# deadskull7/One-Stop-for-COVID-19-Infection-and-Lung-Segmentation-plus-Classification

Measured on AMD Instinct MI355X. Metric: CT images/sec (fwd+bwd) U-Net 512x512x1 bs16, higher is better.
Workload: dtype f32 storage / accumulate / parameters; conv products as a two-term fp16 split (3 fp16 MFMAs per multiply, ~2^-22 per product; --algo 2 = strict fp32); 1 GPU; U-Net infection seg (task1 graph T1:853-916), 512x512x1, batch 16/GPU, fp32, fwd+loss+bwd+Keras-Adam; BASELINE.json configs[1]; storage=fp32, global_batch=16, parallelism=dp1, deterministic=False, bn_fold=2

## Files before the change

include/unet_hip.h:

```cpp
#ifndef UNET_HIP_H
#define UNET_HIP_H
#include <stddef.h>
#include <stdint.h>

#ifdef __cplusplus
extern "C" {
#endif

#define UNET_ABI_VERSION 16

typedef struct unet_ctx unet_ctx;
typedef struct unet_model unet_model;
typedef uint16_t unet_bf16;
enum { UNET_DTYPE_F32 = 0, UNET_DTYPE_BF16 = 1 };

enum { UNET_OK = 0, UNET_E_ARG = -1, UNET_E_HIP = -2, UNET_E_SHAPE = -3, UNET_E_STATE = -4, UNET_E_NODEV = -5 };

enum { UNET_ALGO_AUTO = 0, UNET_ALGO_NAIVE = 1, UNET_ALGO_MFMA = 2 };

int32_t unet_abi_version(void);
int32_t unet_ctx_create(int32_t device_id, unet_ctx** out);
void unet_ctx_destroy(unet_ctx* ctx);
const char* unet_last_error(const unet_ctx* ctx);
int32_t unet_ctx_set_profiling(unet_ctx* ctx, int32_t on);
enum { UNET_OPT_RELU_BITS = 1, UNET_OPT_BN_FOLD = 2, UNET_OPT_ENC_BN_FUSED = 3, UNET_OPT_BN_CONCAT_ANALYTIC = 4, UNET_OPT_BN_FUSE_STATS = 5, UNET_OPT_DETERMINISTIC = 6,
       UNET_OPT_HEAD_FUSED = 7, UNET_OPT_SKIP_RAW = 8, UNET_OPT_POOL_SUMS_FUSED = 9, UNET_OPT_HEAD_BWD_FUSED = 10, UNET_OPT_CONV_PP = 13, UNET_OPT_ENC_TAIL_DGRAD = 14,
       UNET_OPT_WGRAD_EARLY_SPLIT = 15 };
int32_t unet_ctx_set_option(unet_ctx* ctx, int32_t option, int32_t value);
int32_t unet_ctx_get_option(unet_ctx* ctx, int32_t option);

enum { UNET_ACT_NONE = 0, UNET_ACT_RELU = 1, UNET_ACT_ELU = 2 };
enum { UNET_MASK_NONE = 0, UNET_MASK_RELU = 1, UNET_MASK_ELU = 2, UNET_MASK_ELU_DROP = 3, UNET_MASK_RELU_BITS = 9  };

size_t unet_conv3x3_w_ws_floats(int32_t cin, int32_t cout);
int32_t unet_conv3x3_pick_algo(int32_t algo, int32_t wd, int32_t cin, int32_t cout);
double unet_conv3x3_exec_ratio(int32_t algo, int32_t h, int32_t wd, int32_t cin, int32_t cout);
double unet_conv3x3_wgrad_exec_ratio(int32_t algo, int32_t h, int32_t wd, int32_t cin, int32_t cout);
int32_t unet_request_bn_stats(unet_ctx*, int32_t c);
int32_t unet_relu_bits_supported(int32_t algo, int32_t h, int32_t wd, int32_t cin, int32_t cout);
size_t unet_relu_bits_bytes(int32_t n, int32_t h, int32_t wd, int32_t c);
int32_t unet_request_relu_bits(unet_ctx*, void* bits);
int32_t unet_allow_k_slices(unet_ctx*);
int32_t unet_ctx_max_kernel_scratch_bytes(unet_ctx*);
int32_t unet_conv3x3_fwd(unet_ctx*, const float* x, const float* w, const float* bias, float* y,
                         int32_t n, int32_t h, int32_t wd, int32_t cin, int32_t cout,
                         int32_t act, float drop_rate, uint64_t drop_seed, int32_t algo, float* w_ws, void* stream);
int32_t unet_conv3x3_fwd_ld(unet_ctx*, const float* x, const float* w, const float* bias, float* y, int32_t ldy,
                            int32_t n, int32_t h, int32_t wd, int32_t cin, int32_t cout, int32_t act, int32_t algo, float* w_ws, void* stream);
int32_t unet_conv3x3_bwd_data(unet_ctx*, const float* dy, const float* w, const float* mask_src,
                              int32_t mask_mode, float mask_rate, uint64_t mask_seed,
                              float* dx, float* wt_ws, int32_t n, int32_t h, int32_t wd,
                              int32_t cin, int32_t cout, int32_t algo, void* stream);
int32_t unet_conv3x3_bnfold_supported(int32_t algo, int32_t h, int32_t wd, int32_t cin, int32_t cout);
size_t unet_conv3x3_bnfold_ws_floats(int32_t n, int32_t cin, int32_t cout);
int32_t unet_conv3x3_bnfold_fwd(unet_ctx*, const float* x, const float* bnp, const float* w, const float* bias, float* y, int32_t n, int32_t h,
                                int32_t wd, int32_t cin, int32_t cout, int32_t act, int32_t algo, float* ws, void* stream);
int32_t unet_conv3x3_bnfold_bwd_weights(unet_ctx*, const float* x, const float* bnp, const float* dy, const float* w, float* dw, float* db,
                                        double* bn_bwd_sums, void* gws, size_t gws_bytes, float* ws, int32_t n, int32_t h, int32_t wd,
                                        int32_t cin, int32_t cout, int32_t algo, void* stream);
int32_t unet_conv3x3_bnfold_bwd_data(unet_ctx*, const float* dy, const float* w, const float* bnp, const double* bn_bwd_sums, double count, const float* x,
                                     int32_t x_channels, int32_t mask_mode, float mask_rate, uint64_t mask_seed, float* dx, float* wt_ws, float* coef,
                                     int32_t n, int32_t h, int32_t wd, int32_t cin, int32_t cout, int32_t algo, void* stream);
int32_t unet_conv3x3_bnfold_bwd_data_enc_tail(unet_ctx*, const float* dy, const float* w, const float* bnp, const double* bn_bwd_sums, double count, const float* x, int32_t ldx,
                                              const float* enc_bnp, const double* enc_sums, double enc_count, const float* skip_k1, const float* dy_pooled, float rate,
                                              uint64_t seed, float* dx, float* wt_ws, float* coef, int32_t n, int32_t h, int32_t wd, int32_t c, int32_t algo, void* stream);
size_t unet_conv3x3_bwd_weights_ws_bytes(int32_t n, int32_t h, int32_t wd, int32_t cin, int32_t cout);
int32_t unet_conv3x3_bwd_weights(unet_ctx*, const float* x, const float* dy, float* dw, float* db,
                                 void* ws, size_t ws_bytes, int32_t n, int32_t h, int32_t wd,
                                 int32_t cin, int32_t cout, int32_t algo, void* stream);

int32_t unet_convT2x2_fwd(unet_ctx*, const float* x, const float* w, const float* bias, float* y,
                          int32_t ldy, int32_t n, int32_t h, int32_t wd, int32_t cin, int32_t cout,
                          int32_t algo, void* stream);
int32_t unet_convT2x2_bwd_data(unet_ctx*, const float* dy, int32_t lddy, const float* w,
                               const float* relu_src, float* dx, int32_t n, int32_t h, int32_t wd,
                               int32_t cin, int32_t cout, int32_t algo, void* stream);
size_t unet_convT2x2_bwd_weights_ws_bytes(int32_t n, int32_t h, int32_t wd, int32_t cin, int32_t cout);
int32_t unet_convT2x2_bwd_weights(unet_ctx*, const float* x, const float* dy, int32_t lddy,
                                  float* dw, float* db, void* ws, size_t ws_bytes, int32_t n,
                                  int32_t h, int32_t wd, int32_t cin, int32_t cout, int32_t algo,
                                  void* stream);

int32_t unet_bn_stats(unet_ctx*, const float* x, int32_t ldx, double* sums, int64_t pixels,
                      int32_t c, void* stream);
int32_t unet_bn_stats_concat(unet_ctx*, const float* x_up, int32_t ldx, const double* src_sums, double src_count, const float* src_gamma,
                             const float* src_beta, double* sums, int64_t pixels, int32_t c_up, int32_t c_skip, void* stream);
int32_t unet_bn_finalize_train(unet_ctx*, const double* sums, double count, const float* gamma,
                               const float* beta, float* moving_mean, float* moving_var,
                               float* bnp, int32_t c, void* stream);
int32_t unet_bn_finalize_infer(unet_ctx*, const float* gamma, const float* beta,
                               const float* moving_mean, const float* moving_var, float* bnp,
                               int32_t c, void* stream);
int32_t unet_bn_apply(unet_ctx*, const float* x, int32_t ldx, const float* bnp, float* y,
                      int32_t ldy, int64_t pixels, int32_t c, void* stream);
int32_t unet_bn_bwd_stats(unet_ctx*, const float* dy, int32_t lddy, const float* x, int32_t ldx,
                          const float* bnp, double* sums, int64_t pixels, int32_t c, void* stream);
int32_t unet_bn_bwd_param_grads(unet_ctx*, const double* sums, float* dgamma, float* dbeta,
                                int32_t c, void* stream);
int32_t unet_bn_bwd_apply(unet_ctx*, const float* dy, int32_t lddy, const float* x, int32_t ldx,
                          const float* bnp, const double* sums, double count, int32_t mask_mode,
                          float mask_rate, uint64_t mask_seed, float* dx, int32_t lddx, int64_t pixels,
                          int32_t c, void* stream);

int32_t unet_maxpool2x2_dropout_fwd(unet_ctx*, const float* x, int32_t ldx, float* y, int32_t n,
                                    int32_t h, int32_t wd, int32_t c, float rate, uint64_t seed,
                                    void* stream);
int32_t unet_maxpool2x2_dropout_bwd(unet_ctx*, const float* x, int32_t ldx, const float* dy,
                                    float* dx, int32_t lddx, int32_t n, int32_t h, int32_t wd,
                                    int32_t c, float rate, uint64_t seed, int32_t accumulate,
                                    void* stream);

int32_t unet_bn_apply_maxpool_dropout_fwd(unet_ctx*, const float* x, int32_t ldx, const float* bnp, float* y,
                                          int32_t ldy, float* pooled, int32_t n, int32_t h, int32_t wd,
                                          int32_t c, float rate, uint64_t seed, void* stream);
int32_t unet_maxpool2x2_dropout_bwd_bnstats(unet_ctx*, const float* y, int32_t ldy, const float* dy, float* dx,
                                            int32_t lddx, const float* gamma, const float* beta, double* sums,
                                            int32_t n, int32_t h, int32_t wd, int32_t c, float rate,
                                            uint64_t seed, void* stream);
int32_t unet_maxpool2x2_dropout_bwd_sums(unet_ctx*, const float* pooled, const float* dy_pooled, const float* gamma, const float* beta, double* sums,
                                         int32_t n, int32_t h, int32_t wd, int32_t c, float rate, uint64_t seed, void* stream);
int32_t unet_bn_bwd_skip_term(unet_ctx*, double* sums, const double* dec_sum_dyxhat, const float* dec_invstd, const float* dec_gamma,
                              const float* gamma, int32_t c, double frac, void* stream);
int32_t unet_bn_maxpool_bwd_apply(unet_ctx*, const float* x, int32_t ldx, const float* bnp, const double* sums, double count, const float* g_skip,
                                  int32_t ldg, const float* dy_pooled, float* dx, int32_t lddx, int32_t n, int32_t h, int32_t wd, int32_t c,
                                  float rate, uint64_t seed, void* stream);

enum { UNET_LOSS_BCE_DICE = 0, UNET_LOSS_BCE = 1, UNET_LOSS_DICE = 2, UNET_LOSS_TVERSKY = 3, UNET_LOSS_WEIGHTED_BCE_DICE = 4 };
int32_t unet_loss_weight_map(unet_ctx*, const float* y_true, float* weight, int32_t n, int32_t h, int32_t wd, void* stream);
int32_t unet_head_fwd_ex(unet_ctx*, const float* x, const float* w, const float* bias, float* p, const float* y_true, const float* weight_map, double* loss_sums,
                         int64_t pixels, int32_t cin, void* stream);
int32_t unet_head_fwd_bf16_ex(unet_ctx*, const unet_bf16* x, const float* w, const float* bias, float* p, const float* y_true, const float* weight_map,
                              double* loss_sums, int64_t pixels, int32_t cin, void* stream);

int32_t unet_head_fwd(unet_ctx*, const float* x, const float* w, const float* bias, float* p,
                      const float* y_true, double* loss_sums, int64_t pixels, int32_t cin,
                      void* stream);
int32_t unet_loss_finalize(unet_ctx*, const double* loss_sums, double count, float* loss_out,
                           void* stream);
int32_t unet_head_bwd(unet_ctx*, const float* x, const float* w, const float* p, const float* y_true,
                      const double* loss_sums, double count, float* dx, float* dw, float* db,
                      int64_t pixels, int32_t cin, int32_t relu_mask, void* stream);
int32_t unet_loss_finalize_ex(unet_ctx*, const double* loss_sums, double count, int32_t loss, float alpha, float beta, float* loss_out, void* stream);
int32_t unet_head_bwd_ex(unet_ctx*, const float* x, const float* w, const float* p, const float* y_true, const double* loss_sums, double count,
                         int32_t loss, float alpha, float beta, const float* weight_map, float* dx, float* dw, float* db, int64_t pixels, int32_t cin, int32_t relu_mask,
                         void* stream);

int32_t unet_conv3x3_bwd_data_pool_sums_supported(unet_ctx*, int32_t algo, int32_t wd, int32_t cin, int32_t cout);
int32_t unet_conv3x3_bwd_data_pool_sums(unet_ctx*, const float* dy, const float* w, const float* pooled, const float* gamma, const float* beta, float rate,
// ... 355 lines not shown
```

one-stop-for-covid-19-infection-and-lung-segmentation-plus-classification_amd/_lib.py:

```python
from __future__ import annotations

import ctypes as C
import os

_HERE = os.path.dirname(os.path.abspath(__file__))
LIB_PATH = os.environ.get("COVIDSEG_AMD_LIB") or os.path.join(_HERE, "libunet_hip.so")
ABI_VERSION = 16
COMM_HANDLE_BYTES, COMM_MAX_WORLD, COMM_MAX_DOUBLES = 64, 8, 2048

ALGO_AUTO, ALGO_NAIVE, ALGO_MFMA = 0, 1, 2
OPTIONS = {"relu_bits": 1, "bn_fold": 2, "enc_bn_fused": 3, "bn_concat_analytic": 4, "bn_fuse_stats": 5, "deterministic": 6, "head_fused": 7, "skip_raw": 8, "pool_sums_fused": 9, "head_bwd_fused": 10, "conv_pp": 13, "enc_tail_dgrad": 14, "wgrad_early_split": 15}
ARCH_UNET, ARCH_UNETPP, ARCH_CLASSIFIER = 0, 1, 2
LOSSES = {"bce_dice_loss": 0, "binary_crossentropy": 1, "dice_loss": 2, "tversky_loss": 3, "weighted_bce_dice_loss": 4}
DTYPE_F32, DTYPE_BF16 = 0, 1
ACT_NONE, ACT_RELU, ACT_ELU = 0, 1, 2
MORPH_OPS = {"dilate": 0, "erode": 1, "open": 2, "close": 3}
MORPH_MAX_ITERATIONS = 64
INTENSITY_MAX_EDGES = 63
JOINT_HIST_MAX_K, JOINT_HIST_MAX_BINS = 16, 64
SMOOTH_MAX_RADIUS = 32
PAIRS_CHUNK, PAIRS_LDS_SLOTS = 4096, 1024
PAIRS_MIN_CAPACITY, PAIRS_MAX_CAPACITY = 16, 2 ** 30
TRACK_CLS_NONE, TRACK_CLS_RESOLVED, TRACK_CLS_SHRINKAGE, TRACK_CLS_BOTH, TRACK_CLS_GROWTH, TRACK_CLS_NEW = 0, 1, 2, 3, 4, 5
TEXTURE_MAX_LEVELS, TEXTURE_MAX_DISTANCE, TEXTURE_LDS_COUNTERS = 64, 4, 8192
TEXTURE_MAX_RUN = 2 ** 15
ZONE_MAX_PARTS, ZONE_MAX_SHELLS, ZONE_MAX_BINS = 8, 4, 1024
RANK_MAX_RADIUS = 2
FILTER_MODES = {"nearest": 0, "constant": 1, "reflect": 2}
GEODESIC_MAX_STEP = 65534
MASK_NONE, MASK_RELU, MASK_ELU, MASK_ELU_DROP = 0, 1, 2, 3
PROG_FWD_TRAIN, PROG_BWD, PROG_FWD_INFER = 0, 1, 2
SYNC_BN_FWD, SYNC_LOSS, SYNC_BN_BWD, SYNC_GRAD_BUCKET = 0, 1, 2, 3

f32p = C.POINTER(C.c_float)
f64p = C.POINTER(C.c_double)
vp = C.c_void_p
i32, i64, u64, f32, f64, sz = C.c_int32, C.c_int64, C.c_uint64, C.c_float, C.c_double, C.c_size_t


class SyncPoint(C.Structure):
    _fields_ = [("after_op", i32), ("kind", i32), ("ptr", vp), ("count", i64), ("use_op", i32), ("reserved", i32)]


RENDER_MAX_TILES, RENDER_MAX_LAYERS = 64, 4


class RenderTile(C.Structure):
    _fields_ = [("axis", i32), ("index", i32), ("x0", i32), ("y0", i32), ("w", i32), ("h", i32)]


class RenderLayer(C.Structure):
    _fields_ = [("labels", vp), ("palette", vp), ("dtype", i32), ("palette_size", i32), ("fill_alpha", i32), ("outline_alpha", i32)]


class ZoneSpec(C.Structure):
    _fields_ = [("parts", i32 * 3), ("flip", i32 * 3), ("lo", (i32 * 3) * 2), ("extent", (i32 * 3) * 2), ("shells", i32), ("reserved", i32), ("r2", (f64 * 3) * 2)]


_PROTOS = {
    "unet_abi_version": (i32, []),
    "unet_ctx_create": (i32, [i32, C.POINTER(vp)]),
    "unet_ctx_destroy": (None, [vp]),
    "unet_last_error": (C.c_char_p, [vp]),
    "unet_ctx_set_profiling": (i32, [vp, i32]),
    "unet_ctx_set_option": (i32, [vp, i32, i32]),
    "unet_ctx_get_option": (i32, [vp, i32]),
    "unet_conv3x3_w_ws_floats": (sz, [i32, i32]),
    "unet_conv3x3_pick_algo": (i32, [i32, i32, i32, i32]),
    "unet_conv3x3_exec_ratio": (f64, [i32, i32, i32, i32, i32]),
    "unet_conv3x3_wgrad_exec_ratio": (f64, [i32, i32, i32, i32, i32]),
    "unet_request_bn_stats": (i32, [vp, i32]),
    "unet_relu_bits_supported": (i32, [i32, i32, i32, i32, i32]),
    "unet_relu_bits_bytes": (sz, [i32, i32, i32, i32]),
    "unet_request_relu_bits": (i32, [vp, vp]),
    "unet_allow_k_slices": (i32, [vp]),
    "unet_ctx_max_kernel_scratch_bytes": (i32, [vp]),
    "unet_conv3x3_fwd": (i32, [vp, vp, vp, vp, vp, i32, i32, i32, i32, i32, i32, f32, u64, i32, vp, vp]),
    "unet_conv3x3_fwd_ld": (i32, [vp, vp, vp, vp, vp, i32, i32, i32, i32, i32, i32, i32, i32, vp, vp]),
    "unet_conv3x3_bwd_data": (i32, [vp, vp, vp, vp, i32, f32, u64, vp, vp, i32, i32, i32, i32, i32, i32, vp]),
    "unet_conv3x3_bwd_weights_ws_bytes": (sz, [i32, i32, i32, i32, i32]),
    "unet_conv3x3_bwd_weights": (i32, [vp, vp, vp, vp, vp, vp, sz, i32, i32, i32, i32, i32, i32, vp]),
    "unet_convT2x2_fwd": (i32, [vp, vp, vp, vp, vp, i32, i32, i32, i32, i32, i32, i32, vp]),
    "unet_convT2x2_bwd_data": (i32, [vp, vp, i32, vp, vp, vp, i32, i32, i32, i32, i32, i32, vp]),
    "unet_convT2x2_bwd_weights_ws_bytes": (sz, [i32, i32, i32, i32, i32]),
    "unet_convT2x2_bwd_weights": (i32, [vp, vp, vp, i32, vp, vp, vp, sz, i32, i32, i32, i32, i32, i32, vp]),
    "unet_cast_f32_to_bf16": (i32, [vp, vp, vp, i64, vp]),
    "unet_cast_bf16_to_f32": (i32, [vp, vp, vp, i64, vp]),
    "unet_conv3x3_fwd_bf16": (i32, [vp, vp, vp, vp, vp, i32, i32, i32, i32, i32, i32, f32, u64, vp, vp]),
    "unet_conv3x3_first_fwd_bf16": (i32, [vp, vp, vp, vp, vp, i32, i32, i32, i32, i32, f32, u64, vp]),
    "unet_conv3x3_bwd_data_bf16": (i32, [vp, vp, vp, vp, i32, f32, u64, vp, vp, i32, i32, i32, i32, i32, vp]),
    "unet_conv3x3_bwd_weights_ws_bytes_bf16": (sz, [i32, i32, i32, i32, i32]),
    "unet_conv3x3_bwd_weights_bf16": (i32, [vp, vp, vp, vp, vp, vp, sz, i32, i32, i32, i32, i32, vp]),
    "unet_conv3x3_first_bwd_weights_bf16": (i32, [vp, vp, vp, vp, vp, vp, sz, i32, i32, i32, i32, vp]),
    "unet_convT2x2_fwd_bf16": (i32, [vp, vp, vp, vp, vp, i32, i32, i32, i32, i32, i32, vp, vp]),
    "unet_convT2x2_bwd_data_bf16": (i32, [vp, vp, i32, vp, vp, vp, i32, i32, i32, i32, i32, vp, vp]),
    "unet_convT2x2_bwd_weights_ws_bytes_bf16": (sz, [i32, i32, i32, i32, i32]),
    "unet_convT2x2_bwd_weights_bf16": (i32, [vp, vp, vp, i32, vp, vp, vp, sz, i32, i32, i32, i32, i32, vp]),
    "unet_bn_stats": (i32, [vp, vp, i32, vp, i64, i32, vp]),
    "unet_bn_stats_bf16": (i32, [vp, vp, i32, vp, i64, i32, vp]),
    "unet_conv3x3_bnfold_supported": (i32, [i32, i32, i32, i32, i32]),
    "unet_conv3x3_bnfold_ws_floats": (sz, [i32, i32, i32]),
    "unet_conv3x3_bnfold_fwd": (i32, [vp, vp, vp, vp, vp, vp, i32, i32, i32, i32, i32, i32, i32, vp, vp]),
    "unet_conv3x3_bnfold_bwd_weights": (i32, [vp, vp, vp, vp, vp, vp, vp, vp, vp, sz, vp, i32, i32, i32, i32, i32, i32, vp]),
    "unet_conv3x3_bnfold_bwd_data": (i32, [vp, vp, vp, vp, vp, f64, vp, i32, i32, f32, u64, vp, vp, vp, i32, i32, i32, i32, i32, i32, vp]),
    "unet_conv3x3_bnfold_bwd_data_enc_tail": (i32, [vp, vp, vp, vp, vp, f64, vp, i32, vp, vp, f64, vp, vp, f32, u64, vp, vp, vp, i32, i32, i32, i32, i32, vp]),
    "unet_bn_stats_concat": (i32, [vp, vp, i32, vp, f64, vp, vp, vp, i64, i32, i32, vp]),
    "unet_bn_stats_concat_bf16": (i32, [vp, vp, i32, vp, f64, vp, vp, vp, i64, i32, i32, vp]),
    "unet_bn_finalize_train": (i32, [vp, vp, f64, vp, vp, vp, vp, vp, i32, vp]),
    "unet_bn_finalize_infer": (i32, [vp, vp, vp, vp, vp, vp, i32, vp]),
    "unet_bn_apply": (i32, [vp, vp, i32, vp, vp, i32, i64, i32, vp]),
    "unet_bn_apply_bf16": (i32, [vp, vp, i32, vp, vp, i32, i64, i32, vp]),
    "unet_bn_bwd_stats": (i32, [vp, vp, i32, vp, i32, vp, vp, i64, i32, vp]),
    "unet_bn_bwd_stats_bf16": (i32, [vp, vp, i32, vp, i32, vp, vp, i64, i32, vp]),
    "unet_bn_bwd_param_grads": (i32, [vp, vp, vp, vp, i32, vp]),
    "unet_bn_bwd_apply": (i32, [vp, vp, i32, vp, i32, vp, vp, f64, i32, f32, u64, vp, i32, i64, i32, vp]),
    "unet_bn_bwd_apply_bf16": (i32, [vp, vp, i32, vp, i32, vp, vp, f64, i32, f32, u64, vp, i32, i64, i32, vp]),
    "unet_maxpool2x2_dropout_fwd": (i32, [vp, vp, i32, vp, i32, i32, i32, i32, f32, u64, vp]),
    "unet_maxpool2x2_dropout_fwd_bf16": (i32, [vp, vp, i32, vp, i32, i32, i32, i32, f32, u64, vp]),
    "unet_maxpool2x2_dropout_bwd": (i32, [vp, vp, i32, vp, vp, i32, i32, i32, i32, i32, f32, u64, i32, vp]),
    "unet_maxpool2x2_dropout_bwd_bf16": (i32, [vp, vp, i32, vp, vp, i32, i32, i32, i32, i32, f32, u64, i32, vp]),
    "unet_bn_apply_maxpool_dropout_fwd": (i32, [vp, vp, i32, vp, vp, i32, vp, i32, i32, i32, i32, f32, u64, vp]),
    "unet_bn_apply_maxpool_dropout_fwd_bf16": (i32, [vp, vp, i32, vp, vp, i32, vp, i32, i32, i32, i32, f32, u64, vp]),
    "unet_maxpool2x2_dropout_bwd_bnstats": (i32, [vp, vp, i32, vp, vp, i32, vp, vp, vp, i32, i32, i32, i32, f32, u64, vp]),
    "unet_maxpool2x2_dropout_bwd_sums": (i32, [vp, vp, vp, vp, vp, vp, i32, i32, i32, i32, f32, u64, vp]),
    "unet_maxpool2x2_dropout_bwd_sums_bf16": (i32, [vp, vp, vp, vp, vp, vp, i32, i32, i32, i32, f32, u64, vp]),
    "unet_bn_maxpool_bwd_apply_bf16": (i32, [vp, vp, i32, vp, vp, f64, vp, i32, vp, vp, i32, i32, i32, i32, i32, f32, u64, vp]),
    "unet_bn_bwd_skip_term": (i32, [vp, vp, vp, vp, vp, vp, i32, f64, vp]),
    "unet_bn_maxpool_bwd_apply": (i32, [vp, vp, i32, vp, vp, f64, vp, i32, vp, vp, i32, i32, i32, i32, i32, f32, u64, vp]),
    "unet_maxpool2x2_dropout_bwd_bnstats_bf16": (i32, [vp, vp, i32, vp, vp, i32, vp, vp, vp, i32, i32, i32, i32, f32, u64, vp]),
    "unet_head_fwd": (i32, [vp, vp, vp, vp, vp, vp, vp, i64, i32, vp]),
    "unet_head_fwd_bf16": (i32, [vp, vp, vp, vp, vp, vp, vp, i64, i32, vp]),
    "unet_loss_finalize": (i32, [vp, vp, f64, vp, vp]),
    "unet_head_bwd": (i32, [vp, vp, vp, vp, vp, vp, f64, vp, vp, vp, i64, i32, i32, vp]),
    "unet_head_bwd_bf16": (i32, [vp, vp, vp, vp, vp, vp, f64, vp, vp, vp, i64, i32, i32, vp]),
    "unet_loss_finalize_ex": (i32, [vp, vp, f64, i32, f32, f32, vp, vp]),
    "unet_head_bwd_ex": (i32, [vp, vp, vp, vp, vp, vp, f64, i32, f32, f32, vp, vp, vp, vp, i64, i32, i32, vp]),
    "unet_head_bwd_bf16_ex": (i32, [vp, vp, vp, vp, vp, vp, f64, i32, f32, f32, vp, vp, vp, vp, i64, i32, i32, vp]),
    "unet_head_fwd_ex": (i32, [vp, vp, vp, vp, vp, vp, vp, vp, i64, i32, vp]),
    "unet_head_fwd_bf16_ex": (i32, [vp, vp, vp, vp, vp, vp, vp, vp, i64, i32, vp]),
    "unet_loss_weight_map": (i32, [vp, vp, vp, i32, i32, i32, vp]),
    "unet_conv3x3_head_fwd_ex": (i32, [vp, vp, vp, vp, vp, vp, vp, vp, vp, vp, vp, vp, i32, i32, i32, i32, vp, vp]),
    "unet_adam_keras": (i32, [vp, vp, vp, vp, vp, i64, f32, f32, f32, f32, f32, vp]),
    "unet_seg_metrics_sweep": (i32, [vp, vp, vp, vp, i32, vp, i64, vp]),
    "unet_gather_samples": (i32, [vp, vp, vp, vp, i64, i64, vp]),
    "unet_augment_samples": (i32, [vp, vp, vp, vp, vp, vp, vp, i64, i32, i32, i32, vp]),
    "unet_feat_col_mean": (i32, [vp, vp, i64, i64, i64, vp, vp]),
    "unet_feat_gemm_nt_workspace": (sz, [i64, i64, i64, i32]),
    "unet_feat_gemm_nt": (i32, [vp, vp, i64, vp, vp, i64, vp, i64, i64, i64, i32, vp, i64, i32, vp, sz, vp]),
    "unet_feat_gemm_tn_workspace": (sz, [i64, i64, i64]),
    "unet_feat_gemm_tn": (i32, [vp, vp, i64, vp, i64, vp, i64, i64, i64, vp, i64, i32, vp, sz, vp]),
    "unet_kmeans_step": (i32, [vp, vp, i64, i64, i64, vp, i32, vp, vp, vp, vp, vp, vp]),
    "unet_cluster_route_workspace": (sz, [i64, i64, i32]),
    "unet_cluster_route": (i32, [vp, vp, i32, i64, i32, i32, i32, i64, vp, vp, i32, vp, i32, vp, vp, vp, vp, sz, vp]),
    "unet_conv3x3_head_supported": (i32, [vp, i32, i32, i32, i32]),
    "unet_conv3x3_head_fwd": (i32, [vp, vp, vp, vp, vp, vp, vp, vp, vp, vp, vp, i32, i32, i32, i32, vp, vp]),
    "unet_conv3x3_bwd_data_pool_sums_supported": (i32, [vp, i32, i32, i32, i32]),
    "unet_conv3x3_bwd_data_pool_sums": (i32, [vp, vp, vp, vp, vp, vp, f32, vp, vp, vp, i32, i32, i32, i32, i32, vp]),
    "unet_head_dy": (i32, [vp, vp, vp, vp, f64, vp, vp, vp, vp, vp, vp, vp, i32, i32, i32, vp]),
    "unet_head_bwd_stream_supported": (i32, [vp, i32, i32, i32]),
    "unet_head_dzm": (i32, [vp, vp, vp, vp, f64, vp, vp, vp, vp, vp, i32, i32, i32, vp]),
    "unet_head_dy_ex": (i32, [vp, vp, vp, vp, f64, vp, i32, f32, f32, vp, vp, vp, vp, vp, vp, vp, i32, i32, i32, vp]),
    "unet_head_dzm_ex": (i32, [vp, vp, vp, vp, f64, vp, i32, f32, f32, vp, vp, vp, vp, vp, i32, i32, i32, vp]),
    "unet_conv3x3_bwd_data_dzm": (i32, [vp, vp, vp, vp, vp, vp, vp, i32, i32, i32, i32, vp]),
    "unet_conv3x3_bwd_weights_dzm": (i32, [vp, vp, vp, vp, vp, vp, vp, sz, i32, i32, i32, i32, vp]),
    "unet_zero": (i32, [vp, vp, sz, vp]),
    "unet_comm_create": (i32, [vp, i32, i32, vp, vp]),
    "unet_comm_connect": (i32, [vp, vp]),
    "unet_comm_set_timeout_ms": (i32, [vp, i32]),
    "unet_comm_allreduce_f64": (i32, [vp, vp, i32, vp]),
    "unet_comm_status": (i32, [vp, vp, vp]),
    "unet_comm_destroy": (None, [vp]),
    "unet_copy_slice": (i32, [vp, vp, i32, vp, i32, i64, i32, vp]),
    "unet_copy_slice_bf16": (i32, [vp, vp, i32, vp, i32, i64, i32, vp]),
    "unet_accum_slices": (i32, [vp, C.POINTER(vp), C.POINTER(i32), i32, vp, i32, i64, i32, i32, vp]),
    "unet_accum_slices_bf16": (i32, [vp, C.POINTER(vp), C.POINTER(i32), i32, vp, i32, i64, i32, i32, vp]),
    "unet_dense_ws_bytes": (sz, [i32, i32, i32]),
    "unet_dense_fwd": (i32, [vp, vp, vp, vp, vp, i32, i32, i32, i32, f32, u64, vp, sz, vp]),
    "unet_dense_fwd_bf16": (i32, [vp, vp, vp, vp, vp, i32, i32, i32, i32, f32, u64, vp, sz, vp]),
    "unet_dense_bwd": (i32, [vp, vp, vp, vp, vp, vp, i32, i32, i32, vp]),
    "unet_dense_bwd_bf16": (i32, [vp, vp, vp, vp, vp, vp, i32, i32, i32, vp]),
    "unet_cls_head_fwd": (i32, [vp, vp, vp, vp, vp, vp, f32, f32, vp, i32, i32, vp]),
    "unet_cls_loss_finalize": (i32, [vp, vp, f64, vp, vp]),
    "unet_cls_head_bwd": (i32, [vp, vp, vp, vp, vp, f32, f32, f64, f32, vp, vp, vp, vp, i32, i32, vp]),
    "unet_pre_minmax_ws_bytes": (sz, [i32]),
    "unet_pre_minmax_to_u8": (i32, [vp, vp, vp, i32, i64, vp, sz, vp]),
    "unet_pre_unit_to_u8": (i32, [vp, vp, vp, i64, vp]),
    "unet_pre_u8_to_unit": (i32, [vp, vp, vp, i64, vp]),
    "unet_pre_clahe_ws_bytes": (sz, [i32, i32, i32]),
    "unet_pre_clahe_u8": (i32, [vp, vp, vp, i32, i32, i32, f32, i32, i32, vp, sz, vp]),
    "unet_pre_resize_u8": (i32, [vp, vp, i32, i32, i32, vp, vp, i32, i32, i32, i32, i32, vp]),
    "unet_pre_contours_u8": (i32, [vp, vp, i32, i32, i32, i32, vp, vp, vp, i32]),
    "unet_vol_slices_ws_bytes": (sz, [i32, i32]),
    "unet_vol_slices_f64": (i32, [vp, vp, i32, i32, i32, i32, i32, f64, f64, i32, i32, i32, vp, vp, vp, vp, vp, vp, sz, vp]),
    "unet_vol_paste_back": (i32, [vp, vp, i32, i32, vp, vp, i32, vp]),
    "unet_vol_unslice": (i32, [vp, vp, i32, f32, i32, i32, i32, i32, i32, vp, vp, vp]),
    "unet_vol_label_ws_bytes": (sz, [i32, i32, i32]),
    "unet_vol_label": (i32, [vp, vp, i32, i32, i32, i32, vp, vp, vp, sz, vp]),
    "unet_vol_component_stats": (i32, [vp, vp, i32, i32, i32, i32, vp, vp]),
    "unet_vol_filter_components": (i32, [vp, vp, vp, i32, i32, i32, i32, i32, i32, vp, vp, vp]),
    "unet_vol_confusion": (i32, [vp, vp, vp, i32, i32, i32, vp, vp]),
    "unet_vol_surface": (i32, [vp, vp, i32, i32, i32, i32, vp, vp, vp]),
    "unet_vol_edt_ws_bytes": (sz, [i32, i32, i32]),
    "unet_vol_edt_sq": (i32, [vp, vp, i32, i32, i32, i32, vp, vp, vp, sz, vp]),
    "unet_vol_sqrt_f64": (i32, [vp, vp, i64, vp]),
    "unet_vol_surface_distances": (i32, [vp, vp, vp, i32, i32, i32, vp, vp, i64, vp, sz, vp]),
    "unet_vol_lesion_overlap": (i32, [vp, vp, i32, vp, i32, i32, i32, i32, vp, vp, vp]),
    "unet_vol_label_planar": (i32, [vp, vp, i32, i32, i32, i32, vp, vp, vp, sz, vp]),
    "unet_vol_morph_ws_bytes": (sz, [i32, i32, i32]),
    "unet_vol_morph": (i32, [vp, vp, i32, i32, i32, i32, i32, i32, i32, i32, vp, vp, vp, sz, vp]),
    "unet_vol_ball": (i32, [vp, vp, i32, i32, i32, f64, i32, vp, vp, vp]),
    "unet_vol_fill_holes_ws_bytes": (sz, [i32, i32, i32]),
    "unet_vol_fill_holes": (i32, [vp, vp, i32, i32, i32, i32, i32, vp, vp, vp, sz, vp]),
    "unet_vol_dihedral": (i32, [vp, vp, i32, i32, i32, vp, vp]),
    "unet_vol_canvas_axpy": (i32, [vp, vp, f32, vp, i64, i32, vp]),
    "unet_vol_canvas_div": (i32, [vp, vp, f32, i64, vp]),
    "unet_vol_unslice_prob": (i32, [vp, vp, i32, i32, i32, i32, i32, i32, vp, vp]),
    "unet_vol_vote_pack": (i32, [vp, vp, i32, i32, vp, i64, vp]),
    "unet_vol_vote_reduce": (i32, [vp, vp, i32, i32, i32, i32, i32, vp, vp, vp, vp, vp, vp, vp]),
    "unet_vol_intensity_bands": (i32, [vp, vp, i32, i32, i32, i32, i32, f64, f64, vp, vp, i32, vp, vp, i32, vp, vp, vp, vp]),
    "unet_vol_intensity_gather": (i32, [vp, vp, i32, i32, i32, i32, i32, f64, f64, vp, vp, i32, vp, vp, vp, i64, vp, vp]),
    "unet_vol_group_moments_ws_bytes": (sz, [i64, i32]),
    "unet_vol_group_moments": (i32, [vp, vp, vp, i32, vp, vp, sz, vp]),
    "unet_vol_side_assign": (i32, [vp, vp, vp, vp, i32, i32, i32, i32, i32, vp, vp, vp]),
    "unet_vol_side_table": (i32, [vp, vp, vp, vp, i32, i32, i32, i32, vp, vp, vp, vp]),
    "unet_vol_project": (i32, [vp, vp, i32, i32, i32, i32, i32, f64, f64, i32, i32, i32, i32, vp, vp, vp, i32, vp, vp]),
    "unet_vol_render": (i32, [vp, vp, i32, i32, i32, i32, i32, f64, f64, vp, f64, f64, vp, i32, i32, i32, vp, i32, vp, i32, vp, i32, i32, vp]),
    "unet_vol_resample_nearest": (i32, [vp, vp, i32, i32, i32, i32, vp, i32, u64, vp, i32, i32, i32, vp]),
    "unet_vol_resample_linear": (i32, [vp, vp, i32, i32, i32, i32, i32, f64, f64, vp, i32, f64, vp, i32, i32, i32, i32, vp]),
    "unet_vol_joint_hist": (i32, [vp, vp, i32, i32, i32, i32, i32, f64, f64, vp, vp, i32, i32, i32, i32, i32, f64, f64, vp, i32, i32, f64, f64, f64, f64, vp, vp]),
    "unet_vol_smooth_axis": (i32, [vp, vp, i32, i32, i32, i32, i32, i32, vp, vp, vp]),
    "unet_vol_demons_step": (i32, [vp, vp, i32, i32, i32, i32, i32, f64, f64, vp, vp, i32, i32, i32, i32, i32, f64, f64, vp, vp, vp, f64, vp, vp, vp]),
    "unet_vol_warp_field": (i32, [vp, vp, i32, i32, i32, i32, i32, f64, f64, vp, vp, vp, i32, i32, i32, vp, i32, i32, f64, u64, vp, i32, i32, i32, i32, vp]),
    "unet_vol_jacobian": (i32, [vp, vp, i32, i32, i32, vp, vp, vp, vp]),
    "unet_vol_mesh_ws_bytes": (sz, [i32, i32, i32, i32]),
    "unet_vol_mesh_count": (i32, [vp, vp, i32, i32, i32, i32, i32, i32, f64, f64, f64, i32, i32, f64, vp, sz, vp, vp]),
    "unet_vol_mesh_emit": (i32, [vp, vp, i32, i32, i32, i32, i32, i32, f64, f64, f64, i32, i32, f64, vp, vp, sz, vp, i64, vp, vp, i64, vp]),
    "unet_vol_mesh_measure": (i32, [vp, vp, i64, vp, i64, vp, vp, vp]),
    "unet_vol_label_pairs": (i32, [vp, vp, i32, vp, i32, i32, i32, i32, vp, vp, i64, vp, vp]),
# ... 120 lines not shown
```

one-stop-for-covid-19-infection-and-lung-segmentation-plus-classification_amd/csrc/common.h:

```cpp
#pragma once
#include <hip/hip_runtime.h>
#include <stdint.h>
#include <stdio.h>
#include <set>
#include <string>

#include "../../include/unet_hip.h"

constexpr int UNET_BN_SLOTS = 64, UNET_BN_SLOTS_DET = 1024, UNET_BN_SLOT_DOUBLES = 2048;
struct unet_loss_sel { int32_t kind = UNET_LOSS_BCE_DICE; float alpha = 0.5f, beta = 0.5f; };
inline bool unet_loss_sel_ok(const unet_loss_sel& ls, const float* wm = nullptr, bool need_map = true) {
  if (ls.kind < UNET_LOSS_BCE_DICE || ls.kind > UNET_LOSS_WEIGHTED_BCE_DICE) return false;
  if (ls.kind == UNET_LOSS_TVERSKY && !(ls.alpha > 0.0f && ls.beta > 0.0f && ls.alpha < 1e30f && ls.beta < 1e30f)) return false;
  return !need_map || (ls.kind == UNET_LOSS_WEIGHTED_BCE_DICE) == (wm != nullptr);
}
constexpr int UNET_HEAD_SUMS = 100;
struct unet_ctx {
  int device = 0;
  int num_cu = 256;
  int profiling = 0;
  int opt_relu_bits = 1;
  int opt_bn_fold = 2;
  int opt_enc_bn_fused = 1;
  int opt_bn_concat_analytic = 1;
  int opt_bn_fuse_stats = 1;
  int opt_pool_sums_fused = 1;
  int opt_skip_raw = 1;
  int opt_head_fused = 1;
  int opt_head_bwd_fused = 1;
  int opt_enc_tail_dgrad = 1;
  int opt_wgrad_early_split = 0;
  int opt_conv_pp = 1;
  int opt_deterministic = 0;
  double* bn_slots = nullptr;
  int bn_nslots() const { return opt_deterministic ? UNET_BN_SLOTS_DET : UNET_BN_SLOTS; }
  void* convt_img = nullptr;
  size_t convt_img_bytes = 0;
  int k_slices_ok = 0;
  void* splitk_ws = nullptr;
  size_t splitk_ws_bytes = 0;
  int stats_req_c = 0;
  const void* stats_in_slots = nullptr;
  int stats_in_slots_c = 0;
  bool stats_in_slots_xs = false;
  unsigned long long* signs_req = nullptr;
  const void* signs_done = nullptr;
  std::set<const void*> big_lds_kernels;
  std::set<const void*> noted_kernels;
  int max_scratch_bytes = 0;
  std::string err;
};

#define UNET_FAIL(ctx, code, ...)                         \
  do {                                                    \
    char _b[512];                                         \
    snprintf(_b, sizeof(_b), __VA_ARGS__);                \
    if (ctx) (ctx)->err = _b;                             \
    return (code);                                        \
  } while (0)

#define UNET_CHECK_LAUNCH(ctx, what)                                              \
  do {                                                                            \
    hipError_t _e = hipGetLastError();                                            \
    if (_e != hipSuccess) UNET_FAIL(ctx, UNET_E_HIP, "%s: %s", what, hipGetErrorString(_e)); \
  } while (0)

#define UNET_HIP(ctx, expr)                                                       \
  do {                                                                            \
    hipError_t _e = (expr);                                                       \
    if (_e != hipSuccess) UNET_FAIL(ctx, UNET_E_HIP, "%s: %s", #expr, hipGetErrorString(_e)); \
  } while (0)

static inline int32_t unet_big_lds(unet_ctx* ctx, const void* kernel, size_t bytes, const char* what) {
  if (ctx->big_lds_kernels.count(kernel)) return UNET_OK;
  if (hipFuncSetAttribute(kernel, hipFuncAttributeMaxDynamicSharedMemorySize, (int)bytes) != hipSuccess) UNET_FAIL(ctx, UNET_E_HIP, "%s: cannot reserve %zu bytes of LDS", what, bytes);
  ctx->big_lds_kernels.insert(kernel);
  return UNET_OK;
}
static inline void unet_note_kernel(unet_ctx* ctx, const void* kernel) {
  if (ctx->noted_kernels.count(kernel)) return;
  ctx->noted_kernels.insert(kernel);
  hipFuncAttributes at;
  if (hipFuncGetAttributes(&at, kernel) == hipSuccess && (int)at.localSizeBytes > ctx->max_scratch_bytes) ctx->max_scratch_bytes = (int)at.localSizeBytes;
}
#define UNET_BIG_LDS(ctx, kern, bytes, what) do { int32_t _r = unet_big_lds(ctx, reinterpret_cast<const void*>(kern), bytes, what); if (_r) return _r; } while (0)

static inline hipStream_t as_stream(void* s) { return reinterpret_cast<hipStream_t>(s); }
static inline int64_t cdiv64(int64_t a, int64_t b) { return (a + b - 1) / b; }

__device__ __forceinline__ float wave_sum(float v) {
#pragma unroll
  for (int o = 32; o > 0; o >>= 1) v += __shfl_xor(v, o, 64);
  return v;
}

constexpr int UNET_XW = 4;
__device__ __forceinline__ void xsum_add(double* row, int idx, float t) {
  unsigned long long* acc = reinterpret_cast<unsigned long long*>(row) + (size_t)UNET_XW * idx;
  const int eb = (int)((__float_as_uint(t) >> 23) & 0xFF);
  if (eb == 0) return;
  const int e = eb - 127;
  if (e >= 60) { atomicMax(reinterpret_cast<long long*>(acc + 3), 1LL << 62); return; }
  if (e >= 39) {
    atomicAdd(acc + 3, (unsigned long long)__double2ll_rd((double)t * (1.0 / 65536.0)));
    return;
  }
  const int w = min(max((e - 23 + 80) >> 5, 0), 2);
  const double sc = __longlong_as_double((long long)(1023 + 80 - 32 * w) << 52);
  const long long q = __double2ll_rd((double)t * sc);
  atomicAdd(acc + w, (unsigned long long)(q & 0xFFFFFFFFll));
  atomicAdd(acc + w + 1, (unsigned long long)(q >> 32));
}
__device__ __forceinline__ double xsum_take(double* slots, int idx, int nslots) {
// ... 68 lines not shown
typedef float unet_f32x16 __attribute__((ext_vector_type(16)));
__device__ __forceinline__ unsigned pack_bf16x2(float lo, float hi) {
  return __builtin_bit_cast(unsigned, __builtin_convertvector((unet_f32x2){lo, hi}, unet_bf16x2));
}
__device__ __forceinline__ float bf16_lo(unsigned u) { return __uint_as_float(u << 16); }
__device__ __forceinline__ float bf16_hi(unsigned u) { return __uint_as_float(u & 0xFFFF0000u); }
__device__ __forceinline__ float4 ld4(const float* p) { return *reinterpret_cast<const float4*>(p); }
__device__ __forceinline__ void st4(float* p, float4 v) { *reinterpret_cast<float4*>(p) = v; }
__device__ __forceinline__ float4 ld4(const unet_bf16* p) {
  const uint2 u = *reinterpret_cast<const uint2*>(p);
  return make_float4(bf16_lo(u.x), bf16_hi(u.x), bf16_lo(u.y), bf16_hi(u.y));
}
__device__ __forceinline__ void st4(unet_bf16* p, float4 v) { *reinterpret_cast<uint2*>(p) = make_uint2(pack_bf16x2(v.x, v.y), pack_bf16x2(v.z, v.w)); }
__device__ __forceinline__ float ld1(const float* p) { return *p; }
__device__ __forceinline__ float ld1(const unet_bf16* p) { return __uint_as_float((unsigned)*p << 16); }
__device__ __forceinline__ void st1(float* p, float v) { *p = v; }
__device__ __forceinline__ void st1(unet_bf16* p, float v) { *p = (unet_bf16)(pack_bf16x2(v, 0.f) & 0xFFFFu); }

__device__ __forceinline__ uint4 philox4x32(uint64_t ctr, uint64_t seed) {
  uint32_t c0 = (uint32_t)ctr, c1 = (uint32_t)(ctr >> 32), c2 = 0x243F6A88u, c3 = 0x85A308D3u;
  uint32_t k0 = (uint32_t)seed, k1 = (uint32_t)(seed >> 32);
#pragma unroll
  for (int r = 0; r < 10; ++r) {
    uint32_t hi0 = __umulhi(0xD2511F53u, c0), lo0 = 0xD2511F53u * c0;
    uint32_t hi1 = __umulhi(0xCD9E8D57u, c2), lo1 = 0xCD9E8D57u * c2;
    uint32_t n0 = hi1 ^ c1 ^ k0, n1 = lo1, n2 = hi0 ^ c3 ^ k1, n3 = lo0;
    c0 = n0; c1 = n1; c2 = n2; c3 = n3;
    k0 += 0x9E3779B9u; k1 += 0xBB67AE85u;
  }
  return make_uint4(c0, c1, c2, c3);
}
__device__ __forceinline__ float u32_to_unit(uint32_t u) { return (float)(u >> 8) * (1.0f / 16777216.0f); }

__device__ __forceinline__ float4 keep_scale(long long quad_idx, float rate, uint64_t seed) {
  uint4 r = philox4x32((uint64_t)quad_idx, seed);
  float s = 1.0f / (1.0f - rate);
  return make_float4(u32_to_unit(r.x) >= rate ? s : 0.f, u32_to_unit(r.y) >= rate ? s : 0.f,
                     u32_to_unit(r.z) >= rate ? s : 0.f, u32_to_unit(r.w) >= rate ? s : 0.f);
}

__device__ __forceinline__ int argmax4(float a, float b, float c, float d) {
  int k = 0; float m = a;
  if (b > m) { m = b; k = 1; }
  if (c > m) { m = c; k = 2; }
  if (d > m) { m = d; k = 3; }
  return k;
}

enum { ACT_NONE = 0, ACT_RELU = 1, ACT_ELU = 2 };
__device__ __forceinline__ float apply_act(float v, int act) {
  if (act == ACT_RELU) return fmaxf(v, 0.0f);
  if (act == ACT_ELU) return v > 0.0f ? v : expm1f(v);
  return v;
}
enum { MASK_NONE = 0, MASK_RELU = 1, MASK_ELU = 2, MASK_ELU_DROP = 3 };
enum { MASK_BIAS_TAB = 4 };
enum { MASK_BN_BWD = 5 };
enum { MASK_BN_BWD_ELU = 6, MASK_BN_BWD_ELU_DROP = 7 };
enum { MASK_BN_BWD_RELU = 8 };
enum { MASK_RELU_BITS = 9 };
enum { MASK_POOL_SUMS = 10 };
int32_t k_bn_bwd_coef(unet_ctx*, const float* bnp, const double* sums, double count, float* coef, int c, hipStream_t s);
__device__ __forceinline__ float mask_factor(float m, int mode, float ks , float rate) {
  if (mode == MASK_RELU) return m > 0.0f ? 1.0f : 0.0f;
  if (mode == MASK_ELU) return m > 0.0f ? 1.0f : m + 1.0f;
  if (mode == MASK_ELU_DROP) { const float a = m * (1.0f - rate); return ks * (a > 0.0f ? 1.0f : a + 1.0f); }
  return 1.0f;
}

size_t bn_fold_scratch_floats(int cin, int cout);
int32_t k_bn_fold_prepare(unet_ctx*, const float* w, const float* bias, const float* scale, const float* shift, int cin, int cout, float* scratch, hipStream_t s, bool want_scaled = true);
size_t wgrad_bn_fold_scratch_floats(int n, int cout);
bool wgrad_bn_fold_supported(int cout);
int32_t k_wgrad_bn_fold_fix(unet_ctx*, const float* dy, int n, int h, int wd, int cin, int cout, const float* scale, const float* shift, float* dw, const float* db, float* scratch,
                            hipStream_t s, const float* w = nullptr, const float* mean = nullptr, const float* istd = nullptr, double* bn_bwd_sums = nullptr,
                            const float* pre_s = nullptr, const float* pre_t = nullptr,
                            float* dgamma = nullptr, float* dbeta = nullptr);
int32_t k_wgrad_bn_fold_fix_bf16(unet_ctx*, const unet_bf16* dy, int n, int h, int wd, int cin, int cout, const float* scale, const float* shift, float* dw, const float* db,
                                 float* scratch, hipStream_t s, const float* w = nullptr, const float* mean = nullptr, const float* istd = nullptr, double* bn_bwd_sums = nullptr);
constexpr int UNET_PREP_MAX = 36;
bool h2_conv3x3_selected(int algo, int K, int M);
bool pp_conv3x3_selected(const unet_ctx* ctx, int K, int M, int n, int h, int wd, const float* mask, int mask_mode, int act, float rate, int ldy);
int32_t k_conv3x3_pp_fwd(unet_ctx*, const float* x, const void* wimg, const float* bias, const float* mask, int mask_mode, float* y, int ldy, int n, int h, int wd, int K, int M,
                         int act, hipStream_t s, bool vdy = false);
size_t h2_wimg_bytes(int K, int M);
int32_t k_h2_weights(unet_ctx*, const float* w, void* img, int cin, int cout, int flip, hipStream_t s, const float* cs = nullptr);
int32_t k_h2_weights_multi(unet_ctx*, const float* const* w, void* const* img, const int* cin, const int* cout, const int* flip, int count, hipStream_t s);
int32_t k_h2_weights_bound(unet_ctx*, const float* w, const float* cs, void* img, int cin, int cout, hipStream_t s);
int32_t k_h2_prep_multi(unet_ctx*, const float* const* w, const float* const* cs, void* const* img, const int* cin, const int* cout, const int* kind, int count, hipStream_t s);
size_t h2_convT_img_bytes(int cin, int cout);
int32_t k_conv3x3_h2_fwd(unet_ctx*, const float* x, const void* wimg, const float* bias, const float* mask, int mask_mode, float* y, int n, int h, int wd, int K, int M,
                         int act, float rate, uint64_t seed, hipStream_t s, int mask_climit = 1 << 30, int ldy = 0);
int32_t k_slot_fold(unet_ctx*, double* sums, int count, hipStream_t s, bool xs = false);
int32_t k_enc_tail_finish(unet_ctx*, double* sums, const double* dec_sum_dyxhat, const float* dec_invstd, const float* dec_gamma, const float* gamma, float* dgamma, float* dbeta, int c,
                          double frac, hipStream_t s);
bool h2_enc_tail_dgrad_selected(const unet_ctx* ctx, int algo, int n, int h, int wd, int C, bool force);
int32_t k_conv3x3_h2_dgrad_bn_bwd_up(unet_ctx*, const float* dy, const void* wimg, const float* coef, const float* x, float* dx, int n, int h, int wd, int C, hipStream_t s);
int32_t k_conv3x3_h2_dgrad_enc_tail(unet_ctx*, const float* dy, const void* wimg, const float* coef, const float* x, int ldx, const float* enc_bnp, const double* enc_sums, double count,
                                    const float* skip_k1, const float* dy_pooled, float* dx, int n, int h, int wd, int C, float rate, uint64_t seed, hipStream_t s);
bool h2_pool_sums_selected(const unet_ctx* ctx, int algo, int wd, int K, int M);
int32_t k_conv3x3_h2_dgrad_pool_sums(unet_ctx*, const float* dy, const void* wimg, const float* pooled, const float* gamma, const float* beta, float rate, float* dx, double* sums,
                                     int n, int h, int wd, int K, int M, hipStream_t s);
int32_t k_bn_finalize_compose(unet_ctx*, int training, const double* sums, double count, const float* gamma, const float* beta, float* mm, float* mv, float* bnp, int c,
                              const float* enc_bnp, float* comp, hipStream_t s);
int32_t k_loss_finalize(unet_ctx*, const double* loss_sums, double count, float* loss_out, float* loss_out2, hipStream_t s, unet_loss_sel ls = {});
int32_t k_cls_loss_finalize(unet_ctx*, const double* sums, double count, float* out, float* out2, hipStream_t s);
int32_t k_bn_compose(unet_ctx*, const float* bnp_dec, const float* bnp_enc, float* comp, int c, hipStream_t s);
struct h2_head_args { const float* w = nullptr; const float* b = nullptr; float* p = nullptr; const float* t = nullptr; double* slots = nullptr; float aux = 0.0f; const float* wm = nullptr; double inv_count = 0.0; };
bool h2_conv3x3_head_selected(const unet_ctx* ctx, int algo, int wd, int K, int M);
int32_t k_conv3x3_h2_head_fwd(unet_ctx*, const float* x, const void* wimg, const float* bias, float* y, const float* wh, const float* bh, float* p, const float* t,
                              int n, int h, int wd, int K, hipStream_t s, const float* wm = nullptr);
int32_t k_head_fold(unet_ctx*, double* loss_sums, double* head_sums, hipStream_t s, bool weighted = false);
int32_t k_loss_weight_map(unet_ctx*, const float* y_true, float* weight, int n, int h, int wd, hipStream_t s);
int32_t k_head_dy(unet_ctx*, const float* p, const float* t, const double* loss_sums, double count, const double* head_sums, const float* w, const unsigned long long* bits,
                  const float* y, float* dy, float* dw, float* db, int n, int h, int wd, hipStream_t s, unet_loss_sel ls = {}, const float* wm = nullptr);
int32_t k_bn_maxpool_bwd_apply_k1(unet_ctx*, const float* x, int ldx, const float* bnp, const double* sums, double count, const float* g_skip, int ldg, const float* skip_k1,
                                  const float* dy_pooled, float* dx, int lddx, int n, int h, int wd, int c, float rate, uint64_t seed, hipStream_t s);
bool h2_convT_selected(const unet_ctx* ctx, int algo, int cin, int cout);
int32_t k_convT_h2_fwd(unet_ctx*, const float* x, const float* w, const float* bias, float* y, int ldy, int n, int h, int wd, int cin, int cout, hipStream_t s, const void* prepared = nullptr);
int32_t k_convT_h2_dgrad(unet_ctx*, const float* dy, int lddy, const float* w, const float* mask, float* dx, int n, int h, int wd, int cin, int cout, hipStream_t s, int mask_bits = 0,
                         const void* prepared = nullptr);
bool h2_wgrad_selected(int algo, int cin, int cout);
bool h2_wgrad_c16_selected(int algo, int wd, int cin, int cout);
size_t h2_wgrad_c16_ws_bytes(int n, int h, int wd);
int32_t k_wgrad_c16_gather(unet_ctx*, const float* G, float* dw, float* db, hipStream_t s);
int32_t k_conv3x3_h2_wgrad_c16(unet_ctx*, const float* x, const float* dy, float* dw, float* db, void* ws, size_t ws_bytes, int n, int h, int wd, hipStream_t s);
size_t h2_wgrad_ws_bytes(int n, int h, int wd, int cin, int cout);
int32_t k_conv3x3_h2_wgrad(unet_ctx*, const float* x, const float* dy, float* dw, float* db, void* ws, size_t ws_bytes, int n, int h, int wd, int cin, int cout, hipStream_t s);
int32_t k_head_dzm(unet_ctx*, const float* p, const float* t, const double* loss_sums, double count, const double* head_sums, const unsigned long long* bits, void* dzm, float* dw,
                   float* db, int n, int h, int wd, hipStream_t s, unet_loss_sel ls = {}, const float* wm = nullptr);
bool h2_head_bwd_selected(const unet_ctx* ctx, int algo, int wd, int cin);
int32_t k_conv3x3_h2_dgrad_dzm(unet_ctx*, const void* dzm, const void* wimg, const float* mask, int mask_mode, float* dx, int n, int h, int wd, int M, hipStream_t s);
int32_t k_conv3x3_h2_wgrad_dzm(unet_ctx*, const float* x, const void* dzm, const float* w_head, float* dw, float* db, void* ws, size_t ws_bytes, int n, int h, int wd, int cin,
                               hipStream_t s);
int32_t k_conv3x3_naive_fwd(unet_ctx*, const float* x, const float* w, const float* bias, const float* mask, int mask_mode,
                            float* y, int n, int h, int wd, int cin, int cout, int act, float rate, uint64_t seed, hipStream_t s);
bool c1_relu_bits_supported(int wd, int cout);
int32_t k_conv3x3_c1_fwd_bits(unet_ctx*, const float* x, const float* w, const float* bias, float* y, unsigned long long* signs, int n, int h, int wd, int cout, hipStream_t s);
int32_t k_conv3x3_c1_fwd(unet_ctx*, const float* x, const float* w, const float* bias, float* y, int n, int h,
                         int wd, int cout, int act, float rate, uint64_t seed, hipStream_t s);
size_t c1_wgrad_ws_bytes(int cout);
int32_t k_conv3x3_c1_wgrad(unet_ctx*, const float* x, const float* dy, float* dw, float* db, void* ws, size_t ws_bytes, int n, int h,
                           int wd, int cout, hipStream_t s);
int32_t k_flip_transpose_w3x3(unet_ctx*, const float* w, float* wt, int cin, int cout, hipStream_t s);
int32_t k_conv3x3_naive_wgrad(unet_ctx*, const float* x, const float* dy, float* dw, float* db, int n, int h,
                              int wd, int cin, int cout, hipStream_t s);
int32_t k_convT_naive_fwd(unet_ctx*, const float* x, const float* w, const float* bias, float* y, int ldy, int n,
                          int h, int wd, int cin, int cout, hipStream_t s);
int32_t k_convT_naive_dgrad(unet_ctx*, const float* dy, int lddy, const float* w, const float* mask, float* dx,
                            int n, int h, int wd, int cin, int cout, hipStream_t s);
int32_t k_convT_naive_wgrad(unet_ctx*, const float* x, const float* dy, int lddy, float* dw, float* db, int n,
                            int h, int wd, int cin, int cout, hipStream_t s);
bool mfma_conv3x3_supported(int cin, int cout);
int32_t k_conv3x3_mfma_fwd(unet_ctx*, const float* x, const float* w, const float* bias, const float* mask, int mask_mode,
                           float* y, int n, int h, int wd, int cin, int cout, int act, float rate, uint64_t seed, hipStream_t s);
bool mfma_wgrad_supported(int ca, int cb);
bool mfma_convT_supported(int cin, int cout);
int32_t k_convT_mfma_fwd(unet_ctx*, const float* x, const float* w, const float* bias, float* y, int ldy, int n, int h, int wd,
                         int cin, int cout, hipStream_t s);
int32_t k_convT_mfma_dgrad(unet_ctx*, const float* dy, int lddy, const float* w, const float* mask, float* dx, int n, int h, int wd,
                           int cin, int cout, hipStream_t s);
size_t mfma_convT_wgrad_ws_bytes(int n, int h, int wd, int cin, int cout);
bool h2_convT_wgrad_selected(int algo, int cin, int cout);
size_t h2_convT_wgrad_ws_bytes(int n, int h, int wd, int cin, int cout);
int32_t k_convT_h2_wgrad(unet_ctx*, const float* x, const float* dy, int lddy, float* dw, float* db, void* ws, size_t ws_bytes, int n, int h, int wd, int cin, int cout,
                         hipStream_t s);
int32_t k_convT_mfma_wgrad(unet_ctx*, const float* x, const float* dy, int lddy, float* dw, float* db, void* ws, size_t ws_bytes, int n,
// ... 32 lines not shown
```

one-stop-for-covid-19-infection-and-lung-segmentation-plus-classification_amd/csrc/kernels_conv_naive.hip:

```cpp
#include "common.h"

namespace {
constexpr int TPB = 256;

__global__ __launch_bounds__(TPB) void conv3x3_naive_kernel(const float* __restrict__ x, const float* __restrict__ w,
                                                            const float* __restrict__ bias, const float* __restrict__ mask, int mask_mode,
                                                            float* __restrict__ y, int N, int H, int W, int Cin, int Cout, int act,
                                                            float rate, unsigned long long seed) {
  const long long total = (long long)N * H * W * Cout;
  for (long long idx = (long long)blockIdx.x * TPB + threadIdx.x; idx < total; idx += (long long)gridDim.x * TPB) {
    int co = (int)(idx % Cout); long long pix = idx / Cout;
    int j = (int)(pix % W); long long t = pix / W; int i = (int)(t % H); long long n = t / H;
    float acc = bias ? bias[co] : 0.0f;
    for (int a = 0; a < 3; ++a) {
      int ii = i + a - 1; if (ii < 0 || ii >= H) continue;
      for (int b = 0; b < 3; ++b) {
        int jj = j + b - 1; if (jj < 0 || jj >= W) continue;
        const float* xp = x + ((n * H + ii) * W + jj) * (long long)Cin;
        const float* wp = w + (long long)((a * 3 + b) * Cin) * Cout + co;
        for (int ci = 0; ci < Cin; ++ci) acc = fmaf(xp[ci], wp[(long long)ci * Cout], acc);
      }
    }
    acc = apply_act(acc, act);
    float ks = 1.0f;
// ... 344 lines not shown
  long long threads = (long long)n * h * wd * (cout / 4);
  if ((wd & 3) == 0) {
    hipLaunchKernelGGL(conv3x3_c1x4_kernel<T>, dim3(grid_for(threads / 4, 4096)), dim3(TPB), 0, s, x, w, bias, y, n, h, wd, cout, act, rate, (unsigned long long)seed);
    UNET_CHECK_LAUNCH(ctx, "conv3x3_c1x4_fwd"); return UNET_OK;
  }
  hipLaunchKernelGGL(conv3x3_c1_kernel<T>, dim3(grid_for(threads / 2 + 1, 2048)), dim3(TPB), 0, s, x, w, bias, y, n, h, wd, cout, act, rate,
                     (unsigned long long)seed);
  UNET_CHECK_LAUNCH(ctx, "conv3x3_c1_fwd"); return UNET_OK;
}
int32_t k_conv3x3_c1_fwd(unet_ctx* ctx, const float* x, const float* w, const float* bias, float* y, int n, int h, int wd, int cout, int act, float rate,
                         uint64_t seed, hipStream_t s) { return c1_fwd_impl(ctx, x, w, bias, y, n, h, wd, cout, act, rate, seed, s); }
bool c1_relu_bits_supported(int wd, int cout) { return cout == 32 && wd >= 8 && (wd & 7) == 0; }
int32_t k_conv3x3_c1_fwd_bits(unet_ctx* ctx, const float* x, const float* w, const float* bias, float* y, unsigned long long* signs, int n, int h, int wd, int cout, hipStream_t s) {
  if (!c1_relu_bits_supported(wd, cout) || !signs || (long long)n * h * wd >= (1LL << 31)) UNET_FAIL(ctx, UNET_E_SHAPE, "conv3x3_c1 + sign bits: cout=%d W=%d unsupported", cout, wd);
  const long long items = (long long)n * ((h + 3) / 4) * (wd / 8);
  hipLaunchKernelGGL(conv3x3_c1_bits_kernel, dim3(grid_for(items * 64, 4096)), dim3(TPB), 0, s, x, w, bias, y, signs, n, h, wd);
  UNET_CHECK_LAUNCH(ctx, "conv3x3_c1_bits_fwd"); return UNET_OK;
}
int32_t k_conv3x3_c1_fwd_bf16(unet_ctx* ctx, const float* x, const float* w, const float* bias, unet_bf16* y, int n, int h, int wd, int cout, int act,
                              float rate, uint64_t seed, hipStream_t s) { return c1_fwd_impl(ctx, x, w, bias, y, n, h, wd, cout, act, rate, seed, s); }

int32_t k_flip_transpose_w3x3(unet_ctx* ctx, const float* w, float* wt, int cin, int cout, hipStream_t s) {
  hipLaunchKernelGGL(flip_transpose_kernel, dim3(grid_for(9LL * cin * cout, 2048)), dim3(TPB), 0, s, w, wt, cin, cout);
  UNET_CHECK_LAUNCH(ctx, "flip_transpose"); return UNET_OK;
}

int32_t k_conv3x3_naive_wgrad(unet_ctx* ctx, const float* x, const float* dy, float* dw, float* db, int n, int h, int wd,
                              int cin, int cout, hipStream_t s) {
  UNET_HIP(ctx, hipMemsetAsync(dw, 0, sizeof(float) * 9 * cin * cout, s));
  UNET_HIP(ctx, hipMemsetAsync(db, 0, sizeof(float) * cout, s));
  long long outs = (long long)(9 * cin + 1) * cout, pixels = (long long)n * h * wd;
  int gx = (int)cdiv64(outs, TPB);
  long long want = (1 << 18) / (outs < 1 ? 1 : outs) + 1;
  int gy = (int)std::min<long long>(std::max<long long>(want, 1), std::max<long long>(pixels / 64, 1));
  hipLaunchKernelGGL(conv3x3_naive_wgrad_kernel, dim3(gx, gy), dim3(TPB), 0, s, x, dy, dw, db, n, h, wd, cin, cout);
  UNET_CHECK_LAUNCH(ctx, "conv3x3_naive_wgrad"); return UNET_OK;
}

int32_t k_convT_naive_fwd(unet_ctx* ctx, const float* x, const float* w, const float* bias, float* y, int ldy, int n, int h,
                          int wd, int cin, int cout, hipStream_t s) {
  long long total = (long long)n * 4 * h * wd * cout;
  hipLaunchKernelGGL(convT_naive_fwd_kernel, dim3(grid_for(total, 1 << 20)), dim3(TPB), 0, s, x, w, bias, y, ldy, n, h, wd, cin, cout);
  UNET_CHECK_LAUNCH(ctx, "convT_naive_fwd"); return UNET_OK;
}

int32_t k_convT_naive_dgrad(unet_ctx* ctx, const float* dy, int lddy, const float* w, const float* mask, float* dx, int n,
                            int h, int wd, int cin, int cout, hipStream_t s) {
  long long total = (long long)n * h * wd * cin;
  dim3 g(grid_for(total, 1 << 20)), b(TPB);
  if (mask) hipLaunchKernelGGL(convT_naive_dgrad_kernel<true>, g, b, 0, s, dy, lddy, w, mask, dx, n, h, wd, cin, cout);
  else hipLaunchKernelGGL(convT_naive_dgrad_kernel<false>, g, b, 0, s, dy, lddy, w, mask, dx, n, h, wd, cin, cout);
  UNET_CHECK_LAUNCH(ctx, "convT_naive_dgrad"); return UNET_OK;
}

int32_t k_convT_naive_wgrad(unet_ctx* ctx, const float* x, const float* dy, int lddy, float* dw, float* db, int n, int h,
                            int wd, int cin, int cout, hipStream_t s) {
  UNET_HIP(ctx, hipMemsetAsync(dw, 0, sizeof(float) * 4 * cin * cout, s));
  UNET_HIP(ctx, hipMemsetAsync(db, 0, sizeof(float) * cout, s));
  long long outs = 4LL * cout * (cin + 1), pixels = (long long)n * h * wd;
  int gx = (int)cdiv64(outs, TPB);
  long long want = (1 << 18) / outs + 1;
  int gy = (int)std::min<long long>(std::max<long long>(want, 1), std::max<long long>(pixels / 64, 1));
  hipLaunchKernelGGL(convT_naive_wgrad_kernel, dim3(gx, gy), dim3(TPB), 0, s, x, dy, lddy, dw, db, n, h, wd, cin, cout);
  UNET_CHECK_LAUNCH(ctx, "convT_naive_wgrad"); return UNET_OK;
}

size_t c1_wgrad_ws_bytes(int cout) { return (size_t)(C1_BLOCKS + 32) * 10 * cout * sizeof(float); }

template <typename T>
static int32_t c1_wgrad_impl(unet_ctx* ctx, const float* x, const T* dy, float* dw, float* db, void* ws, size_t ws_bytes, int n, int h,
                           int wd, int cout, hipStream_t s) {
  if ((cout & 3) || TPB % (cout / 4) || (cout / 4) > 64 || (long long)n * h * wd >= (1LL << 31)) UNET_FAIL(ctx, UNET_E_SHAPE, "conv3x3_c1_wgrad: cout=%d unsupported", cout);
  if (!ws || ws_bytes < c1_wgrad_ws_bytes(cout)) UNET_FAIL(ctx, UNET_E_ARG, "conv3x3_c1_wgrad: workspace too small");
  long long groups = ((long long)n * h * wd * (cout / 4) + TPB - 1) / TPB;
  int blocks = (int)std::min<long long>(C1_BLOCKS, std::max<long long>(groups, 1));
  if ((wd & 3) == 0) hipLaunchKernelGGL((conv3x3_c1_wgrad_kernel<T, true>), dim3(blocks), dim3(TPB), 0, s, x, dy, static_cast<float*>(ws), n, h, wd, cout);
  else hipLaunchKernelGGL((conv3x3_c1_wgrad_kernel<T, false>), dim3(blocks), dim3(TPB), 0, s, x, dy, static_cast<float*>(ws), n, h, wd, cout);
  float* part = static_cast<float*>(ws); float* part2 = part + (size_t)C1_BLOCKS * 10 * cout;
  const int ngroups = (blocks + 31) / 32;
  hipLaunchKernelGGL(reduce_c1_kernel, dim3((10 * cout + 127) / 128, ngroups), dim3(128), 0, s, part, part2, nullptr, blocks, 32, cout, 0);
  hipLaunchKernelGGL(reduce_c1_kernel, dim3((10 * cout + 127) / 128, 1), dim3(128), 0, s, part2, dw, db, ngroups, ngroups, cout, 1);
  UNET_CHECK_LAUNCH(ctx, "conv3x3_c1_wgrad"); return UNET_OK;
}
int32_t k_conv3x3_c1_wgrad(unet_ctx* ctx, const float* x, const float* dy, float* dw, float* db, void* ws, size_t ws_bytes, int n, int h, int wd, int cout,
                           hipStream_t s) { return c1_wgrad_impl(ctx, x, dy, dw, db, ws, ws_bytes, n, h, wd, cout, s); }
int32_t k_conv3x3_c1_wgrad_bf16(unet_ctx* ctx, const float* x, const unet_bf16* dy, float* dw, float* db, void* ws, size_t ws_bytes, int n, int h, int wd,
                                int cout, hipStream_t s) { return c1_wgrad_impl(ctx, x, dy, dw, db, ws, ws_bytes, n, h, wd, cout, s); }
```

one-stop-for-covid-19-infection-and-lung-segmentation-plus-classification_amd/csrc/kernels_conv_pp.hip:

```cpp
#include <type_traits>

#include "common.h"

#ifndef PP_TRACE
#define PP_TRACE 0
#endif
#ifndef PP_MID
#define PP_MID 2
#endif
#ifndef PP_STORE_AUX
#define PP_STORE_AUX 2
#endif
#ifndef PP_EXP
#define PP_EXP 0
#endif
#if PP_TRACE
__device__ unsigned long long pp_trace[256 * 2 * 40 * 12];
#define PP_STAMP(i) do { if (lane == 0 && wave == 0 && it < 40 && blockIdx.x < 256) pp_trace[((blockIdx.x * 2 + half) * 40 + it) * 12 + (i)] = __builtin_readcyclecounter(); } while (0)
extern "C" int32_t unet_debug_pp_trace(unsigned long long* host, int n) { return hipMemcpyFromSymbol(host, HIP_SYMBOL(pp_trace), (size_t)n * 8) == hipSuccess ? 0 : 1; }
#else
#define PP_STAMP(i) do { } while (0)
#endif

namespace {

typedef _Float16 f16x8 __attribute__((ext_vector_type(8)));
typedef unet_f32x16 f32x16;
constexpr int PP_HEADER = 256;

__device__ __forceinline__ float pp_pow2f(int e) { return __uint_as_float((unsigned)(e + 127) << 23); }
__device__ __forceinline__ f16x8 pp_frag(const char* p) { return *reinterpret_cast<const f16x8*>(p); }
__device__ __forceinline__ int pp_cell(int p, int c) { return p * 128 + ((c ^ (p & 7)) << 4); }

template <int KC, bool BITS, bool VDY>
__global__ __launch_bounds__(512, 2) void conv_pp_kernel(const float* __restrict__ x, const unet_bf16* __restrict__ wimg_hdr, const float* __restrict__ bias,
                                                         const float* __restrict__ mask, float* __restrict__ y, int ldy, int N, int H, int W, int act, int mask_mode,
                                                         int tiles_x, int tiles_y, int total_tiles, double* __restrict__ stats, int stats_c,
                                                         unsigned long long* __restrict__ signs, int xs) {
  constexpr int RW = 2, TH = 8, PWD = 34, NPIX = (TH + 2) * PWD, K = 16 * KC, M = 32;
  constexpr int HS = NPIX * 16;
  constexpr int PLANE = 2 * HS, CHUNK = 2 * PLANE + 32;
  constexpr int IN_HALF = KC * CHUNK;
  constexpr int W_BYTES = 9 * 2048, W_ALL = KC * W_BYTES;
  constexpr int PPC = 4 * KC, PPIECES = NPIX * PPC, PL = (PPIECES + 255) / 256;
  static_assert(256 % PPC == 0, "a thread's pieces are the same 16 bytes of 256 / PPC pixels apart");
  extern __shared__ __attribute__((aligned(16))) char smem[];
  const int tid = threadIdx.x & 255, lane = threadIdx.x & 63, l31 = lane & 31, hi = lane >> 5;
  const int wave8 = __builtin_amdgcn_readfirstlane(threadIdx.x >> 6);
  const int half = wave8 >> 2, wave = wave8 & 3;
  char* const s_w = smem;
  char* const s_in = smem + W_ALL + half * IN_HALF;
  char* const s_out = smem + W_ALL + 2 * IN_HALF + wave * 4096;
  float* const s_amax = reinterpret_cast<float*>(smem + W_ALL + 2 * IN_HALF + 4 * 4096) + half * 4;
  float* const s_bias = reinterpret_cast<float*>(smem + W_ALL + 2 * IN_HALF + 4 * 4096) + 8;
  float* const s_stat = s_bias + 32;
  float* const s_tab = s_stat + 8 * 2 * 32;

  const int per = gridDim.x >> 3, xcd = blockIdx.x & 7, j = blockIdx.x >> 3;
  const int tpx = (total_tiles + 7) >> 3;
  const int t_beg = xcd * tpx, t_end = min(t_beg + tpx, total_tiles);
  const int slots = 2 * per, iters = (tpx + slots - 1) / slots;
  const int t0 = t_beg + j * 2 + half;

  const int pc = tid % PPC, pix0 = tid / PPC;
  const int dst0 = (pc >> 2) * CHUNK + ((pc & 3) >> 1) * HS + pix0 * 16 + (pc & 1) * 8;
  int rel[PL];
#pragma unroll
  for (int k = 0; k < PL; ++k) {
    const int pix = pix0 + k * (256 / PPC), r = pix / PWD, col = pix - r * PWD;
    rel[k] = pix < NPIX ? (VDY ? (r * W + col) * 8 : ((r * W + col) * K + pc * 4) * 4) : UNET_OOB;
  }
  constexpr int XPP = VDY ? 2 : K;
  const long long lead = (long long)(W + 1) * XPP;
  const __amdgpu_buffer_rsrc_t rs_x = make_rsrc(x - lead, ((long long)N * H * W * XPP + lead) * 4);
  const __amdgpu_buffer_rsrc_t rs_y = make_rsrc(y, (((long long)N * H * W - 1) * ldy + M) * 4);
  const int st_lane = ((lane >> 3) * ldy + (lane & 7) * 4) * 4;

  unet_u32x4 pregA[PL];
  struct pos { int n, y0, x0; };
  auto tile_pos = [&](int t) __attribute__((always_inline)) {
    pos p; const int tx = t % tiles_x; const int t2 = t / tiles_x;
    const int ty = t2 % tiles_y; p.n = t2 / tiles_y; p.x0 = tx * 32; p.y0 = ty * TH;
    return p;
  };
  const int d_x = (slots % tiles_x) * 32, d_y = ((slots / tiles_x) % tiles_y) * TH, d_n = slots / (tiles_x * tiles_y);
  auto advance = [&](pos p) __attribute__((always_inline)) {
    p.x0 += d_x; if (p.x0 >= tiles_x * 32) { p.x0 -= tiles_x * 32; p.y0 += TH; }
    p.y0 += d_y; if (p.y0 >= tiles_y * TH) { p.y0 -= tiles_y * TH; p.n += 1; }
    p.n += d_n;
    return p;
  };
  auto issue_loads = [&](pos p, unet_u32x4 (&preg)[PL]) __attribute__((always_inline)) {
    const int soff = (((p.n * H + p.y0) * W + p.x0) * XPP) * 4;
    int off[PL];
    if (p.y0 > 0 && p.y0 + TH < H && p.x0 > 0 && p.x0 + 32 < W) {
#pragma unroll
      for (int k = 0; k < PL; ++k) off[k] = rel[k];
    } else {
#pragma unroll
      for (int k = 0; k < PL; ++k) {
        const int pix = pix0 + k * (256 / PPC), r = pix / PWD, col = pix - r * PWD;
        const bool ok = (unsigned)(p.y0 - 1 + r) < (unsigned)H && (unsigned)(p.x0 - 1 + col) < (unsigned)W;
        off[k] = ok ? rel[k] : UNET_OOB;
      }
    }
#pragma unroll
    for (int k = 0; k < PL; ++k) {
      asm volatile("" : "+v"(off[k]));
      if (VDY) { const unet_u32x2 v = __builtin_amdgcn_raw_buffer_load_b64(rs_x, off[k], soff, 0); preg[k][0] = v[0]; preg[k][1] = v[1]; }
      else preg[k] = __builtin_amdgcn_raw_buffer_load_b128(rs_x, off[k], soff, 0);
    }
  };

  {
    const __amdgpu_buffer_rsrc_t rs_w = __builtin_amdgcn_make_buffer_rsrc(const_cast<unet_bf16*>(wimg_hdr), 0, PP_HEADER + W_ALL, 0x00020000);
    constexpr int WP = W_ALL / 16;
#pragma unroll
    for (int k = 0; k < (WP + 511) / 512; ++k) {
      const int idx = (int)threadIdx.x + k * 512;
      const unet_u32x4 v = __builtin_amdgcn_raw_buffer_load_b128(rs_w, idx < WP ? PP_HEADER + idx * 16 : UNET_OOB, 0, 0);
      if (idx < WP) *reinterpret_cast<unet_u32x4*>(s_w + idx * 16) = v;
    }
    if (threadIdx.x < 32) s_bias[threadIdx.x] = bias ? bias[threadIdx.x] : 0.f;
    if (!BITS && mask_mode == MASK_BIAS_TAB) s_tab[threadIdx.x] = mask[threadIdx.x];
  }
  const float w_unscale = *reinterpret_cast<const float*>(wimg_hdr);
  pos p_prev = {0, 0, 0}, p_cur = tile_pos(t0), p_next = advance(p_cur);
  if (t0 < t_end) issue_loads(p_cur, pregA);
  __syncthreads();
  if (half) { __builtin_amdgcn_s_barrier(); __builtin_amdgcn_s_barrier(); }

  f32x16 acc[RW];
#pragma unroll
  for (int r = 0; r < RW; ++r)
#pragma unroll
    for (int i = 0; i < 16; ++i) acc[r][i] = 0.f;
  float vprev[RW][16];
  float4 st1 = make_float4(0.f, 0.f, 0.f, 0.f), st2 = st1;
  int e_prev = 0, e_cur = 0;
  constexpr bool bits_mask = BITS;
  const bool tab_mask = !BITS && mask_mode == MASK_BIAS_TAB;
  unsigned mpre[BITS ? RW : 1][4];
  const __amdgpu_buffer_rsrc_t rs_m = make_rsrc(mask, BITS ? (long long)N * H * (W >> 3) * 32 : 0);
  float4 t4s[4];
  int sg_lo = 0, sg_hi = 0;

  auto eslice = [&](const int sl) __attribute__((always_inline)) {
    const int pn = p_prev.n, py0 = p_prev.y0, px0 = p_prev.x0;
    const int r = sl < 9 ? 0 : 1, q = sl - r * 9;
    const int py = py0 + wave * RW + r;
    if (py >= H) return;
    if (q == 0) {
#pragma unroll
      for (int qq = 0; qq < 4; ++qq)
        *reinterpret_cast<float4*>(s_out + pp_cell(l31, hi * 4 + qq)) = make_float4(vprev[r][qq * 4], vprev[r][qq * 4 + 1], vprev[r][qq * 4 + 2], vprev[r][qq * 4 + 3]);
    } else if (q == 1) {
#pragma unroll
      for (int jj = 0; jj < 4; ++jj) t4s[jj] = *reinterpret_cast<const float4*>(s_out + pp_cell(jj * 8 + (lane >> 3), lane & 7));
    }
    if (q >= 2 && (q & 1) == 0) {
      const int jj = (q - 2) >> 1;
      const int pxj = px0 + jj * 8 + (lane >> 3);
      const float4 t4 = t4s[jj];
      if (signs) {
        const unsigned long long b[4] = {__builtin_amdgcn_ballot_w64(t4.x > 0.f), __builtin_amdgcn_ballot_w64(t4.y > 0.f), __builtin_amdgcn_ballot_w64(t4.z > 0.f), __builtin_amdgcn_ballot_w64(t4.w > 0.f)};
#pragma unroll
        for (int k = 0; k < 4; ++k) {
          unet_writelane(sg_lo, (unsigned)b[k], jj * 4 + k);
          unet_writelane(sg_hi, (unsigned)(b[k] >> 32), jj * 4 + k);
        }
        if (jj == 3) {
          const int cells = min(4, (W - px0) >> 3);
          if (lane < 4 * cells)
            signs[(((long long)pn * H + py) * (W >> 3) + (px0 >> 3)) * 4 + lane] = ((unsigned long long)(unsigned)sg_hi << 32) | (unsigned)sg_lo;
        }
      }
      const bool ok = pxj < W;
      const int row_off = (((pn * H + py) * W + px0 + jj * 8) * ldy) * 4;
      __builtin_amdgcn_raw_buffer_store_b128(__builtin_bit_cast(unet_u32x4, t4), rs_y, ok ? st_lane : UNET_OOB, row_off, PP_STORE_AUX);
      if (stats) {
        const float kf = ok ? 1.f : 0.f;
        st1.x = fmaf(kf, t4.x, st1.x); st1.y = fmaf(kf, t4.y, st1.y); st1.z = fmaf(kf, t4.z, st1.z); st1.w = fmaf(kf, t4.w, st1.w);
        const float ux = kf * t4.x, uy = kf * t4.y, uz = kf * t4.z, uw = kf * t4.w;
        st2.x = fmaf(ux, t4.x, st2.x); st2.y = fmaf(uy, t4.y, st2.y); st2.z = fmaf(uz, t4.z, st2.z); st2.w = fmaf(uw, t4.w, st2.w);
      }
    }
  };

  auto mphase = [&](auto HC_, auto HP_, const int it) __attribute__((always_inline)) {
    constexpr bool HC = decltype(HC_)::value, HP = decltype(HP_)::value;
    f16x8 px[2][RW + 2], wf[2][2];
    auto ld_row = [&](int ch, int kx, int rr) __attribute__((always_inline)) {
#pragma unroll
      for (int p = 0; p < 2; ++p) px[p][rr] = pp_frag(s_in + ch * CHUNK + p * PLANE + hi * HS + ((wave * RW + rr) * PWD + l31 + kx) * 16);
    };
    auto ld_w = [&](int s_) __attribute__((always_inline)) {
      const int ch = s_ / 9, kx = (s_ / 3) % 3, ky = s_ % 3;
#pragma unroll
      for (int p = 0; p < 2; ++p) wf[s_ & 1][p] = pp_frag(s_w + ch * W_BYTES + (((ky * 3 + kx) * 2 + p) * 2 + hi) * 512 + l31 * 16);
    };
    if (HC) {
#pragma unroll
      for (int r = 0; r < RW; ++r)
#pragma unroll
        for (int i = 0; i < 16; ++i) acc[r][i] = 0.f;
      ld_row(0, 0, 0); ld_row(0, 0, 1); ld_w(0);
    }
#pragma unroll
    for (int s_ = 0; s_ < 9 * KC; ++s_) {
      if (HC) {
        const int ky = s_ % 3;
        if (s_ + 1 < 9 * KC) {
          const int s1 = s_ + 1, ch1 = s1 / 9, kx1 = (s1 / 3) % 3, ky1 = s1 % 3;
          ld_w(s1);
          if (ky1 == 0) { ld_row(ch1, kx1, 0); ld_row(ch1, kx1, 1); }
          else ld_row(ch1, kx1, ky1 + 1);
        }
#pragma unroll
        for (int pr = 0; pr < 3; ++pr) {
          constexpr int PW[3] = {0, 1, 0}, PX[3] = {1, 0, 0};
#pragma unroll
          for (int r = 0; r < RW; ++r) acc[r] = __builtin_amdgcn_mfma_f32_32x32x16_f16(wf[s_ & 1][PW[pr]], px[PX[pr]][r + ky], acc[r], 0, 0, 0);
        }
      }
      if (HP) eslice(s_ * 18 / (9 * KC));
      __builtin_amdgcn_sched_barrier(0);
      if (s_ == PP_MID) {
        PP_STAMP(7);
        __builtin_amdgcn_s_barrier();
        PP_STAMP(8);
        __builtin_amdgcn_sched_barrier(0);
      }
    }
  };

  auto body = [&](const int it, unet_u32x4 (&preg)[PL]) __attribute__((always_inline)) {
    const int t_cur = t0 + it * slots, t_next = t_cur + slots, t_prev = t_cur - slots;
    const bool have_cur = it < iters && t_cur < t_end, have_next = it + 1 < iters && t_next < t_end, have_prev = it >= 1 && t_prev < t_end;
    auto output_values = [&]() __attribute__((always_inline)) {
    {
        const int py0 = p_prev.y0, px0 = p_prev.x0;
        const float unscale = pp_pow2f(-e_prev) * w_unscale;
        const int px_ = px0 + l31;
        const bool border = tab_mask && (py0 == 0 || py0 + TH >= H || px0 == 0 || px0 + 32 >= W);
        float bv[16];
#pragma unroll
        for (int q = 0; q < 4; ++q) {
          const float4 b4 = *reinterpret_cast<const float4*>(s_bias + hi * 16 + q * 4);
          bv[q * 4] = b4.x; bv[q * 4 + 1] = b4.y; bv[q * 4 + 2] = b4.z; bv[q * 4 + 3] = b4.w;
        }
#pragma unroll
        for (int r = 0; r < RW; ++r) {
          const int py = py0 + wave * RW + r;
          if (border && (py == 0 || py == H - 1 || px_ == 0 || px_ == W - 1)) {
            const int cls = (((py == 0) | ((py == H - 1) << 1)) << 2) | ((px_ == 0) | ((px_ == W - 1) << 1));
            const float* tb = s_tab + cls * M + hi * 16;
#pragma unroll
            for (int q = 0; q < 4; ++q) {
              const float4 b4 = *reinterpret_cast<const float4*>(tb + q * 4);
              vprev[r][q * 4] = fmaf(acc[r][q * 4], unscale, b4.x); vprev[r][q * 4 + 1] = fmaf(acc[r][q * 4 + 1], unscale, b4.y);
              vprev[r][q * 4 + 2] = fmaf(acc[r][q * 4 + 2], unscale, b4.z); vprev[r][q * 4 + 3] = fmaf(acc[r][q * 4 + 3], unscale, b4.w);
            }
          } else {
#pragma unroll
            for (int i = 0; i < 16; ++i) vprev[r][i] = fmaf(acc[r][i], unscale, bv[i]);
          }
          if (act == ACT_RELU) {
#pragma unroll
            for (int i = 0; i < 16; ++i) vprev[r][i] = fmaxf(vprev[r][i], 0.f);
          }
          if (bits_mask) {
            const unsigned sh = (l31 & 3) * 8 + hi * 4;
#pragma unroll
            for (int qq = 0; qq < 4; ++qq)
#pragma unroll
              for (int k = 0; k < 4; ++k) vprev[r][qq * 4 + k] = __uint_as_float(__float_as_uint(vprev[r][qq * 4 + k]) & (unsigned)__builtin_amdgcn_sbfe((int)mpre[BITS ? r : 0][k], sh + qq, 1u));
          }
        }
      }
    };
    PP_STAMP(0);
    if (have_cur) {
      float mx = 0.f;
#pragma unroll
      for (int k = 0; k < PL; ++k) {
        if (VDY) { mx = fmaxf(mx, preg[k][1] ? fabsf(__uint_as_float(preg[k][0])) : 0.f); continue; }
        asm("v_max3_f32 %0, |%1|, |%2|, %0" : "+v"(mx) : "v"(preg[k][0]), "v"(preg[k][1]));
        asm("v_max3_f32 %0, |%1|, |%2|, %0" : "+v"(mx) : "v"(preg[k][2]), "v"(preg[k][3]));
      }
      mx = wave_max_nonneg(mx);
      if (lane == 0) s_amax[wave] = mx;
    }
    asm volatile("s_waitcnt lgkmcnt(0)" ::: "memory");
    PP_STAMP(1);
    __builtin_amdgcn_s_barrier();
    PP_STAMP(2);
    if (BITS && have_prev) output_values();
    if (have_cur) {
      const float4 m4 = *reinterpret_cast<const float4*>(s_amax);
      const float mx = fmaxf(fmaxf(m4.x, m4.y), fmaxf(m4.z, m4.w));
      const int eb = __builtin_amdgcn_readfirstlane((int)((__float_as_uint(mx) >> 23) & 0xFF));
      e_cur = min(138 - eb, 120);
      const float sc = pp_pow2f(e_cur);
#pragma unroll
      for (int k = 0; k < PL; ++k) {
        if (pix0 + k * (256 / PPC) < NPIX) {
          unsigned h0, m0, h1, m1;
          if (VDY) {
            unsigned hh, mm;
            split2_scaled(__uint_as_float(preg[k][0]), __uint_as_float(preg[k][0]), sc, hh, mm);
            const unsigned nib = preg[k][1] >> (pc * 4);
            const unsigned k01 = h2_pair_mask(nib, 0), k23 = h2_pair_mask(nib, 2);
            h0 = hh & k01; h1 = hh & k23; m0 = mm & k01; m1 = mm & k23;
          } else {
          split2_scaled(__uint_as_float(preg[k][0]), __uint_as_float(preg[k][1]), sc, h0, m0);
          split2_scaled(__uint_as_float(preg[k][2]), __uint_as_float(preg[k][3]), sc, h1, m1);
          }
          *reinterpret_cast<uint2*>(s_in + dst0 + k * (256 / PPC) * 16) = make_uint2(h0, h1);
          *reinterpret_cast<uint2*>(s_in + dst0 + k * (256 / PPC) * 16 + PLANE) = make_uint2(m0, m1);
        }
      }
    }
    PP_STAMP(3);
    if (bits_mask && have_cur) {
#pragma unroll
      for (int r = 0; r < RW; ++r) {
        const int py = p_cur.y0 + wave * RW + r;
        const bool ok = py < H && p_cur.x0 + (l31 & ~7) < W;
        const int mo = ok ? (((p_cur.n * H + py) * (W >> 3) + (p_cur.x0 >> 3) + (l31 >> 3)) * 32 + ((l31 >> 2) & 1) * 4) : UNET_OOB;
#pragma unroll
        for (int k = 0; k < 4; ++k) mpre[BITS ? r : 0][k] = __builtin_amdgcn_raw_buffer_load_b32(rs_m, mo, k * 8, 0);
      }
    }
    __builtin_amdgcn_sched_barrier(0);
    if (have_next && (PP_EXP & 2) == 0) issue_loads(p_next, preg);
    __builtin_amdgcn_sched_barrier(0);
    PP_STAMP(4);
    if (!BITS && have_prev) output_values();
    asm volatile("s_waitcnt lgkmcnt(0)" ::: "memory");
    PP_STAMP(5);
    __builtin_amdgcn_s_barrier();
    PP_STAMP(6);
    __builtin_amdgcn_sched_barrier(0);
    if (have_cur && have_prev) mphase(std::true_type{}, std::true_type{}, it);
    else if (have_cur) mphase(std::true_type{}, std::false_type{}, it);
    else if (have_prev) mphase(std::false_type{}, std::true_type{}, it);
    else { PP_STAMP(7); __builtin_amdgcn_s_barrier(); PP_STAMP(8); }
    asm volatile("s_waitcnt lgkmcnt(0)" ::: "memory");
    __builtin_amdgcn_sched_barrier(0);
    PP_STAMP(9);
    __builtin_amdgcn_s_barrier();
    PP_STAMP(10);
    e_prev = e_cur; p_prev = p_cur; p_cur = p_next; p_next = advance(p_next);
  };
  for (int it = 0; it <= iters; ++it) body(it, pregA);
  if (!half) { __builtin_amdgcn_s_barrier(); __builtin_amdgcn_s_barrier(); }

  if (stats) {
    float sv[8] = {st1.x, st1.y, st1.z, st1.w, st2.x, st2.y, st2.z, st2.w};
#pragma unroll
    for (int i = 0; i < 8; ++i) { sv[i] += __shfl_xor(sv[i], 8); sv[i] += __shfl_xor(sv[i], 16); sv[i] += __shfl_xor(sv[i], 32); }
    if (lane < 8) {
#pragma unroll
      for (int i = 0; i < 4; ++i) { s_stat[(wave8 * 2 + 0) * 32 + lane * 4 + i] = sv[i]; s_stat[(wave8 * 2 + 1) * 32 + lane * 4 + i] = sv[4 + i]; }
    }
    __syncthreads();
    if (threadIdx.x < 64) {
      const int kind = threadIdx.x >> 5, c32 = threadIdx.x & 31;
      float t = 0.f;
#pragma unroll
      for (int wv = 0; wv < 8; ++wv) t += s_stat[(wv * 2 + kind) * 32 + c32];
      double* const row = stats + (size_t)(blockIdx.x % UNET_BN_SLOTS) * UNET_BN_SLOT_DOUBLES;
      if (xs) xsum_add(row, (kind ? stats_c : 0) + c32, t); else atomicAdd(row + (kind ? stats_c : 0) + c32, (double)t);
    }
  }
}

}

bool pp_conv3x3_selected(const unet_ctx* ctx, int K, int M, int n, int h, int wd, const float* mask, int mask_mode, int act, float rate, int ldy) {
  if (!ctx || !ctx->opt_conv_pp) return false;
  if (K != 32 || M != 32 || rate != 0.0f || (act != ACT_NONE && act != ACT_RELU)) return false;
  if (mask && mask_mode != MASK_BIAS_TAB && mask_mode != MASK_RELU_BITS) return false;
  if (mask && mask_mode == MASK_RELU_BITS && (wd & 7)) return false;
  if (ldy < M || (ldy & 3)) return false;
  const long long tiles = (long long)((wd + 31) / 32) * ((h + 7) / 8) * n;
  if (tiles < 4LL * 2 * ctx->num_cu && ctx->opt_conv_pp < 2) return false;
  if ((long long)n * h * wd * K * 4 + (long long)(wd + 1) * K * 4 >= (1LL << 31)) return false;
  if ((long long)n * h * wd * ldy * 4 >= (1LL << 31)) return false;
  return true;
}

int32_t k_conv3x3_pp_fwd(unet_ctx* ctx, const float* x, const void* wimg, const float* bias, const float* mask, int mask_mode, float* y, int ldy, int n, int h, int wd, int K, int M,
                         int act, hipStream_t s, bool vdy) {
  if (K != 32 || M != 32) UNET_FAIL(ctx, UNET_E_SHAPE, "conv pp: K=%d M=%d", K, M);
  constexpr int KC = 2;
  ctx->k_slices_ok = 0;
  if (!mask) mask_mode = MASK_NONE;
  const int tiles_x = (wd + 31) / 32, tiles_y = (h + 7) / 8;
  const long long total = (long long)tiles_x * tiles_y * n;
  double* stats = nullptr; int stats_c = 0;
  if (ctx->stats_req_c > 0) {
    const int c = ctx->stats_req_c; ctx->stats_req_c = 0;
    const int xw = ctx->opt_deterministic ? UNET_XW : 1;
    if ((mask_mode == MASK_NONE || mask_mode == MASK_BIAS_TAB) && 2 * c * xw <= UNET_BN_SLOT_DOUBLES && c == M && ctx->bn_slots) {
      stats = ctx->bn_slots; stats_c = c; ctx->stats_in_slots = y; ctx->stats_in_slots_c = c; ctx->stats_in_slots_xs = ctx->opt_deterministic != 0;
    }
  }
  unsigned long long* signs = nullptr;
  if (ctx->signs_req) {
    unsigned long long* q = ctx->signs_req; ctx->signs_req = nullptr;
    if (act == ACT_RELU && (mask_mode == MASK_NONE || mask_mode == MASK_BIAS_TAB) && !(wd & 7)) { signs = q; ctx->signs_done = q; }
  }
  constexpr int NPIX = 340, CHUNK = 4 * NPIX * 16 + 32;
  constexpr size_t smem = (size_t)KC * 9 * 2048 + 2 * (size_t)KC * CHUNK + 4 * 4096 + 32 + 128 + 8 * 2 * 32 * 4 + 16 * 32 * 4;
  if (vdy && (stats || signs || bias || act != ACT_NONE || mask_mode == MASK_BIAS_TAB)) UNET_FAIL(ctx, UNET_E_ARG, "conv pp behind the head's {dz, mask} stream: a plain data-gradient launch only");
  auto kern = vdy ? (mask_mode == MASK_RELU_BITS ? conv_pp_kernel<KC, true, true> : conv_pp_kernel<KC, false, true>)
                  : (mask_mode == MASK_RELU_BITS ? conv_pp_kernel<KC, true, false> : conv_pp_kernel<KC, false, false>);
  UNET_BIG_LDS(ctx, kern, smem, "conv_pp");
  unet_note_kernel(ctx, reinterpret_cast<const void*>(kern));
  const unsigned grid = (unsigned)(ctx->num_cu & ~7);
  hipLaunchKernelGGL(kern, dim3(grid), dim3(512), smem, s, x, static_cast<const unet_bf16*>(wimg), bias, mask, y, ldy, n, h, wd, act, mask_mode, tiles_x, tiles_y, (int)total, stats,
                     stats_c, signs, ctx->opt_deterministic ? 1 : 0);
  UNET_CHECK_LAUNCH(ctx, "conv_pp");
  return UNET_OK;
}
```

one-stop-for-covid-19-infection-and-lung-segmentation-plus-classification_amd/csrc/model.hip:

```cpp
#include <algorithm>
#include <functional>
#include <map>
#include <set>
#include <string>
#include <vector>

#include "common.h"

extern "C" {

int32_t unet_abi_version(void) { return UNET_ABI_VERSION; }

int32_t unet_ctx_create(int32_t device_id, unet_ctx** out) {
  if (!out) return UNET_E_ARG;
  *out = nullptr;
  int ndev = 0;
  if (hipGetDeviceCount(&ndev) != hipSuccess || ndev <= 0 || device_id < 0 || device_id >= ndev) return UNET_E_NODEV;
  hipDeviceProp_t prop;
  if (hipGetDeviceProperties(&prop, device_id) != hipSuccess) return UNET_E_NODEV;
  if (std::string(prop.gcnArchName).rfind("gfx950", 0) != 0) return UNET_E_NODEV;
  unet_ctx* c = new unet_ctx();
  c->device = device_id;
  c->num_cu = prop.multiProcessorCount;
  const size_t sb = sizeof(double) * UNET_BN_SLOTS_DET * UNET_BN_SLOT_DOUBLES;
  int prev = 0;
  (void)hipGetDevice(&prev);
  if (hipSetDevice(device_id) != hipSuccess || hipMalloc(reinterpret_cast<void**>(&c->bn_slots), sb) != hipSuccess ||
      hipMemset(c->bn_slots, 0, sb) != hipSuccess) { (void)hipSetDevice(prev); delete c; return UNET_E_HIP; }
  c->convt_img_bytes = (size_t)8 << 20;
  if (hipMalloc(&c->convt_img, c->convt_img_bytes) != hipSuccess) { c->convt_img = nullptr; c->convt_img_bytes = 0; }
  c->splitk_ws_bytes = (size_t)32 << 20;
  if (hipMalloc(&c->splitk_ws, c->splitk_ws_bytes) != hipSuccess) { c->splitk_ws = nullptr; c->splitk_ws_bytes = 0; }
  (void)hipSetDevice(prev);
  *out = c;
  return UNET_OK;
}

void unet_ctx_destroy(unet_ctx* ctx) {
  if (ctx && ctx->bn_slots) (void)hipFree(ctx->bn_slots);
  if (ctx && ctx->convt_img) (void)hipFree(ctx->convt_img);
  if (ctx && ctx->splitk_ws) (void)hipFree(ctx->splitk_ws);
  delete ctx;
}
const char* unet_last_error(const unet_ctx* ctx) { return ctx ? ctx->err.c_str() : "null ctx"; }
int32_t unet_ctx_set_profiling(unet_ctx* ctx, int32_t on) { if (!ctx) return UNET_E_ARG; ctx->profiling = on; return UNET_OK; }

static int* ctx_option(unet_ctx* ctx, int32_t option) {
  switch (option) {
    case UNET_OPT_RELU_BITS: return &ctx->opt_relu_bits;
    case UNET_OPT_BN_FOLD: return &ctx->opt_bn_fold;
    case UNET_OPT_ENC_BN_FUSED: return &ctx->opt_enc_bn_fused;
    case UNET_OPT_BN_CONCAT_ANALYTIC: return &ctx->opt_bn_concat_analytic;
    case UNET_OPT_BN_FUSE_STATS: return &ctx->opt_bn_fuse_stats;
    case UNET_OPT_DETERMINISTIC: return &ctx->opt_deterministic;
    case UNET_OPT_HEAD_FUSED: return &ctx->opt_head_fused;
    case UNET_OPT_SKIP_RAW: return &ctx->opt_skip_raw;
    case UNET_OPT_POOL_SUMS_FUSED: return &ctx->opt_pool_sums_fused;
    case UNET_OPT_HEAD_BWD_FUSED: return &ctx->opt_head_bwd_fused;
    case UNET_OPT_CONV_PP: return &ctx->opt_conv_pp;
    case UNET_OPT_ENC_TAIL_DGRAD: return &ctx->opt_enc_tail_dgrad;
    case UNET_OPT_WGRAD_EARLY_SPLIT: return &ctx->opt_wgrad_early_split;
    default: return nullptr;
  }
}
int32_t unet_ctx_set_option(unet_ctx* ctx, int32_t option, int32_t value) {
  if (!ctx) return UNET_E_ARG;
  int* p = ctx_option(ctx, option);
  const int hi = option == UNET_OPT_BN_FOLD ? 3 : (option == UNET_OPT_CONV_PP || option == UNET_OPT_ENC_TAIL_DGRAD) ? 2 : 1;
  if (!p || value < 0 || value > hi) UNET_FAIL(ctx, UNET_E_ARG, "ctx_set_option: option %d value %d", option, value);
  *p = value;
  return UNET_OK;
}
int32_t unet_ctx_get_option(unet_ctx* ctx, int32_t option) {
  if (!ctx) return UNET_E_ARG;
  const int* p = ctx_option(ctx, option);
  if (!p) UNET_FAIL(ctx, UNET_E_ARG, "ctx_get_option: unknown option %d", option);
  return *p;
}

}

static bool use_mfma(int algo, int cin, int cout) {
  if (algo == UNET_ALGO_NAIVE) return false;
  return mfma_conv3x3_supported(cin, cout);
}
static bool use_h2(int algo, int cin, int cout, const void* uws) { return uws && h2_conv3x3_selected(algo, cin, cout); }

static int32_t conv3x3_fwd_dispatch(unet_ctx* ctx, const float* x, const float* w, const float* bias, const float* mask, int mask_mode,
                                    float* y, int n, int h, int wd, int cin, int cout, int act, float rate, uint64_t seed, int algo,
                                    hipStream_t s, float* uws = nullptr, int flip = 0, const float* prepared = nullptr, int ldy = 0) {
  if (ldy && ldy != cout && !(use_h2(algo, cin, cout, uws) && prepared)) UNET_FAIL(ctx, UNET_E_STATE, "conv3x3: a strided output (ldy %d) exists on the h2 kernels with a prepared image only", ldy);
  if (use_h2(algo, cin, cout, uws)) {
    if (prepared) return k_conv3x3_h2_fwd(ctx, x, prepared, bias, mask, mask_mode, y, n, h, wd, cin, cout, act, rate, seed, s, 1 << 30, ldy);
    int32_t r = flip ? k_h2_weights(ctx, w, uws, cout, cin, 1, s) : k_h2_weights(ctx, w, uws, cin, cout, 0, s);
    if (r) return r;
    return k_conv3x3_h2_fwd(ctx, x, uws, bias, mask, mask_mode, y, n, h, wd, cin, cout, act, rate, seed, s);
  }
  if (mask_mode >= MASK_BIAS_TAB) UNET_FAIL(ctx, UNET_E_STATE, "conv3x3: the folded-BatchNorm / bit-mask epilogues exist on the h2 kernels only (cin=%d cout=%d algo=%d)", cin, cout, algo);
  if (flip) {
    if (!uws) UNET_FAIL(ctx, UNET_E_ARG, "conv3x3 data gradient: needs the weight scratch");
    int32_t r = k_flip_transpose_w3x3(ctx, w, uws, cout, cin, s);
    if (r) return r;
    w = uws;
  }
  if (use_mfma(algo, cin, cout)) return k_conv3x3_mfma_fwd(ctx, x, w, bias, mask, mask_mode, y, n, h, wd, cin, cout, act, rate, seed, s);
  if (cin == 1 && !mask && algo != UNET_ALGO_NAIVE && (cout % 4) == 0 && 256 % (cout / 4) == 0) {
    if (ctx->signs_req && act == ACT_RELU && rate == 0.0f && c1_relu_bits_supported(wd, cout)) {
      unsigned long long* q = ctx->signs_req; ctx->signs_req = nullptr;
      int32_t r = k_conv3x3_c1_fwd_bits(ctx, x, w, bias, y, q, n, h, wd, cout, s);
      if (!r) ctx->signs_done = q;
      return r;
    }
    return k_conv3x3_c1_fwd(ctx, x, w, bias, y, n, h, wd, cout, act, rate, seed, s);
  }
  return k_conv3x3_naive_fwd(ctx, x, w, bias, mask, mask_mode, y, n, h, wd, cin, cout, act, rate, seed, s);
}

static int32_t conv3x3_wgrad_dispatch(unet_ctx* ctx, const float* x, const float* dy, float* dw, float* db, void* ws,
                                      size_t ws_bytes, int n, int h, int wd, int cin, int cout, int algo, hipStream_t s) {
  if (algo != UNET_ALGO_NAIVE && mfma_wgrad_supported(cin, cout) && ws && ws_bytes >= mfma_wgrad_ws_bytes(n, h, wd, cin, cout)) {
    if (h2_wgrad_c16_selected(algo, wd, cin, cout) && ws_bytes >= h2_wgrad_c16_ws_bytes(n, h, wd))
      return k_conv3x3_h2_wgrad_c16(ctx, x, dy, dw, db, ws, ws_bytes, n, h, wd, s);
    if (h2_wgrad_selected(algo, cin, cout) && ws_bytes >= h2_wgrad_ws_bytes(n, h, wd, cin, cout))
      return k_conv3x3_h2_wgrad(ctx, x, dy, dw, db, ws, ws_bytes, n, h, wd, cin, cout, s);
    return k_conv3x3_mfma_wgrad(ctx, x, dy, dw, db, ws, ws_bytes, n, h, wd, cin, cout, s);
  }
  if (cin == 1 && algo != UNET_ALGO_NAIVE && (cout % 4) == 0 && 256 % (cout / 4) == 0 && cout <= 256 && ws && ws_bytes >= c1_wgrad_ws_bytes(cout))
    return k_conv3x3_c1_wgrad(ctx, x, dy, dw, db, ws, ws_bytes, n, h, wd, cout, s);
  return k_conv3x3_naive_wgrad(ctx, x, dy, dw, db, n, h, wd, cin, cout, s);
}

extern "C" {

int32_t unet_request_bn_stats(unet_ctx* ctx, int32_t c) {
  if (!ctx || c < 0) UNET_FAIL(ctx, UNET_E_ARG, "request_bn_stats: bad args");
  ctx->stats_req_c = ctx->opt_bn_fuse_stats ? c : 0;
  return UNET_OK;
}

int32_t unet_relu_bits_supported(int32_t algo, int32_t h, int32_t wd, int32_t cin, int32_t cout) {
  if (cin < 1 || cout < 1 || (cout & 31) || (wd & 7) || h < 1) return 0;
  if (cin == 1) return algo == UNET_ALGO_AUTO && c1_relu_bits_supported(wd, cout) ? 1 : 0;
  return h2_conv3x3_selected(algo, cin, cout) ? 1 : 0;
}
// ... 50 lines not shown
  ctx->signs_req = nullptr;
  if (!r && armed && ctx->signs_done != armed) UNET_FAIL(ctx, UNET_E_SHAPE, "conv3x3_head_fwd: armed with unet_request_relu_bits but the launch did not write them");
  if (!r && y_true) r = k_head_fold(ctx, loss_sums, head_sums, as_stream(stream), weight_map != nullptr);
  return r;
}
int32_t unet_conv3x3_head_fwd(unet_ctx* ctx, const float* x, const float* w, const float* bias, float* y, const float* w_head, const float* b_head, float* p, const float* y_true,
                              double* loss_sums, double* head_sums, int32_t n, int32_t h, int32_t wd, int32_t cin, float* w_ws, void* stream) {
  return unet_conv3x3_head_fwd_ex(ctx, x, w, bias, y, w_head, b_head, p, y_true, nullptr, loss_sums, head_sums, n, h, wd, cin, w_ws, stream);
}
int32_t unet_head_bwd_stream_supported(unet_ctx* ctx, int32_t algo, int32_t wd, int32_t cin) {
  return ctx && cin == 32 && h2_head_bwd_selected(ctx, algo, wd, cin) && h2_wgrad_selected(algo, cin, 32) ? 1 : 0;
}
int32_t unet_head_dzm(unet_ctx* ctx, const float* p, const float* y_true, const double* loss_sums, double count, const double* head_sums, const void* relu_bits, void* dzm,
                      float* dw_head, float* db_head, int32_t n, int32_t h, int32_t wd, void* stream) {
  if (!ctx) return UNET_E_ARG;
  return k_head_dzm(ctx, p, y_true, loss_sums, count, head_sums, static_cast<const unsigned long long*>(relu_bits), dzm, dw_head, db_head, n, h, wd, as_stream(stream));
}
int32_t unet_head_dzm_ex(unet_ctx* ctx, const float* p, const float* y_true, const double* loss_sums, double count, const double* head_sums, int32_t loss, float alpha,
                         float beta, const float* weight_map, const void* relu_bits, void* dzm, float* dw_head, float* db_head, int32_t n, int32_t h, int32_t wd, void* stream) {
  if (!ctx) return UNET_E_ARG;
  return k_head_dzm(ctx, p, y_true, loss_sums, count, head_sums, static_cast<const unsigned long long*>(relu_bits), dzm, dw_head, db_head, n, h, wd, as_stream(stream),
                    unet_loss_sel{loss, alpha, beta}, weight_map);
}
int32_t unet_conv3x3_bwd_data_dzm(unet_ctx* ctx, const void* dzm, const float* w, const float* w_head, const void* relu_bits_in, float* dx, float* wt_ws, int32_t n, int32_t h,
                                  int32_t wd, int32_t cin, void* stream) {
  if (!ctx || !dzm || !w || !w_head || !dx || !wt_ws || n < 1 || h < 1 || wd < 1) UNET_FAIL(ctx, UNET_E_ARG, "conv3x3_bwd_data_dzm: bad args");
  if (!unet_head_bwd_stream_supported(ctx, UNET_ALGO_AUTO, wd, cin)) UNET_FAIL(ctx, UNET_E_SHAPE, "conv3x3_bwd_data_dzm: not supported here (unet_head_bwd_stream_supported)");
  int32_t r = k_h2_weights(ctx, w, wt_ws, cin, 32, 1, as_stream(stream), w_head);
  if (!r) r = k_conv3x3_h2_dgrad_dzm(ctx, dzm, wt_ws, static_cast<const float*>(relu_bits_in), relu_bits_in ? MASK_RELU_BITS : MASK_NONE, dx, n, h, wd, cin, as_stream(stream));
  ctx->k_slices_ok = 0;
  return r;
}
int32_t unet_conv3x3_bwd_weights_dzm(unet_ctx* ctx, const float* x, const void* dzm, const float* w_head, float* dw, float* db, void* ws, size_t ws_bytes, int32_t n, int32_t h,
                                     int32_t wd, int32_t cin, void* stream) {
  if (!ctx || !x || !dzm || !w_head || !dw || !db || n < 1 || h < 1 || wd < 1) UNET_FAIL(ctx, UNET_E_ARG, "conv3x3_bwd_weights_dzm: bad args");
  if (!unet_head_bwd_stream_supported(ctx, UNET_ALGO_AUTO, wd, cin)) UNET_FAIL(ctx, UNET_E_SHAPE, "conv3x3_bwd_weights_dzm: not supported here (unet_head_bwd_stream_supported)");
  return k_conv3x3_h2_wgrad_dzm(ctx, x, dzm, w_head, dw, db, ws, ws_bytes, n, h, wd, cin, as_stream(stream));
}
int32_t unet_head_dy(unet_ctx* ctx, const float* p, const float* y_true, const double* loss_sums, double count, const double* head_sums, const float* w_head, const void* relu_bits,
                     const float* y, float* dy, float* dw_head, float* db_head, int32_t n, int32_t h, int32_t wd, void* stream) {
  if (!ctx) return UNET_E_ARG;
  return k_head_dy(ctx, p, y_true, loss_sums, count, head_sums, w_head, static_cast<const unsigned long long*>(relu_bits), y, dy, dw_head, db_head, n, h, wd, as_stream(stream));
}
int32_t unet_head_dy_ex(unet_ctx* ctx, const float* p, const float* y_true, const double* loss_sums, double count, const double* head_sums, int32_t loss, float alpha,
                        float beta, const float* weight_map, const float* w_head, const void* relu_bits, const float* y, float* dy, float* dw_head, float* db_head,
                        int32_t n, int32_t h, int32_t wd, void* stream) {
  if (!ctx) return UNET_E_ARG;
  return k_head_dy(ctx, p, y_true, loss_sums, count, head_sums, w_head, static_cast<const unsigned long long*>(relu_bits), y, dy, dw_head, db_head, n, h, wd, as_stream(stream),
                   unet_loss_sel{loss, alpha, beta}, weight_map);
}

int32_t unet_conv3x3_pick_algo(int32_t algo, int32_t wd, int32_t cin, int32_t cout) {
  (void)wd;
  if (h2_conv3x3_selected(algo, cin, cout)) return UNET_ALGO_AUTO;
  if (algo != UNET_ALGO_NAIVE && mfma_conv3x3_supported(cin, cout)) return UNET_ALGO_MFMA;
  return UNET_ALGO_NAIVE;
}

double unet_conv3x3_exec_ratio(int32_t algo, int32_t h, int32_t wd, int32_t cin, int32_t cout) {
  (void)h; (void)wd;
  return h2_conv3x3_selected(algo, cin, cout) ? 3.0 * 157.3 / 2500.0 : 1.0;
}

double unet_conv3x3_wgrad_exec_ratio(int32_t algo, int32_t h, int32_t wd, int32_t cin, int32_t cout) {
  (void)h; (void)wd;
  if (algo == UNET_ALGO_NAIVE || !mfma_wgrad_supported(cin, cout)) return 1.0;
  return h2_wgrad_selected(algo, cin, cout) ? 3.0 * 157.3 / 2500.0 : 1.0;
}

size_t unet_conv3x3_w_ws_floats(int32_t cin, int32_t cout) { return cin > 0 && cout > 0 ? (size_t)16 * std::max(cin, 32) * std::max(cout, 32) + 64 : 0; }

int32_t unet_conv3x3_bwd_data(unet_ctx* ctx, const float* dy, const float* w, const float* mask_src, int32_t mask_mode, float mask_rate,
                              uint64_t mask_seed, float* dx, float* wt_ws, int32_t n, int32_t h, int32_t wd, int32_t cin, int32_t cout,
                              int32_t algo, void* stream) {
  if (!ctx || !dy || !w || !dx || !wt_ws || n < 1 || h < 1 || wd < 1 || cin < 1 || cout < 1 || mask_mode < 0 || (mask_mode > 3 && mask_mode != MASK_RELU_BITS) ||
      (mask_mode != MASK_NONE && !mask_src) || mask_rate < 0 || mask_rate >= 1)
    UNET_FAIL(ctx, UNET_E_ARG, "conv3x3_bwd_data: bad args");
  if (mask_mode == MASK_RELU_BITS && !unet_relu_bits_supported(algo, h, wd, cout, cin))
    UNET_FAIL(ctx, UNET_E_SHAPE, "conv3x3_bwd_data: no bit-mask form for h=%d w=%d cin=%d cout=%d algo=%d (unet_relu_bits_supported(algo, h, w, cout, cin))", h, wd, cin, cout, algo);
  const int32_t r = conv3x3_fwd_dispatch(ctx, dy, w, nullptr, mask_src, mask_mode, dx, n, h, wd, cout, cin, ACT_NONE, mask_rate, mask_seed, algo,
                                         as_stream(stream), wt_ws, 1);
  ctx->k_slices_ok = 0;
  return r;
}

int32_t unet_conv3x3_bwd_data_pool_sums_supported(unet_ctx* ctx, int32_t algo, int32_t wd, int32_t cin, int32_t cout) { return ctx && h2_pool_sums_selected(ctx, algo, wd, cout, cin) ? 1 : 0; }
int32_t unet_conv3x3_bwd_data_pool_sums(unet_ctx* ctx, const float* dy, const float* w, const float* pooled, const float* gamma, const float* beta, float rate, float* dx, double* sums,
                                        float* wt_ws, int32_t n, int32_t h, int32_t wd, int32_t cin, int32_t cout, void* stream) {
  if (!ctx || !dy || !w || !pooled || !gamma || !beta || !dx || !sums || !wt_ws || n < 1 || h < 1 || wd < 1) UNET_FAIL(ctx, UNET_E_ARG, "conv3x3_bwd_data_pool_sums: bad args");
  if (!h2_pool_sums_selected(ctx, UNET_ALGO_AUTO, wd, cout, cin)) UNET_FAIL(ctx, UNET_E_SHAPE, "conv3x3_bwd_data_pool_sums: not supported here (unet_conv3x3_bwd_data_pool_sums_supported)");
  int32_t r = k_h2_weights(ctx, w, wt_ws, cin, cout, 1, as_stream(stream));
  if (r) return r;
  return k_conv3x3_h2_dgrad_pool_sums(ctx, dy, wt_ws, pooled, gamma, beta, rate, dx, sums, n, h, wd, cout, cin, as_stream(stream));
}

int32_t unet_conv3x3_bnfold_supported(int32_t algo, int32_t h, int32_t wd, int32_t cin, int32_t cout) {
  return (h >= 1 && wd >= 1 && cin >= 1 && cout >= 1 && h2_conv3x3_selected(algo, cin, cout) && (cout % 16) == 0 && wgrad_bn_fold_supported(cout)) ? 1 : 0;
}
size_t unet_conv3x3_bnfold_ws_floats(int32_t n, int32_t cin, int32_t cout) {
  if (n < 1 || cin < 1 || cout < 1) return 0;
  return bn_fold_scratch_floats(cin, cout) + unet_conv3x3_w_ws_floats(cin, cout) + wgrad_bn_fold_scratch_floats(n, cout);
}
int32_t unet_conv3x3_bnfold_fwd(unet_ctx* ctx, const float* x, const float* bnp, const float* w, const float* bias, float* y, int32_t n, int32_t h, int32_t wd,
                                int32_t cin, int32_t cout, int32_t act, int32_t algo, float* ws, void* stream) {
  if (!ctx || !x || !bnp || !w || !y || !ws || n < 1 || act < 0 || act > ACT_RELU) UNET_FAIL(ctx, UNET_E_ARG, "conv3x3_bnfold_fwd: bad args");
  if (!unet_conv3x3_bnfold_supported(algo, h, wd, cin, cout)) UNET_FAIL(ctx, UNET_E_SHAPE, "conv3x3_bnfold_fwd: no folded form for h=%d w=%d cin=%d cout=%d (unet_conv3x3_bnfold_supported)", h, wd, cin, cout);
  hipStream_t s = as_stream(stream);
  float* u = ws + bn_fold_scratch_floats(cin, cout);
  int32_t r = k_bn_fold_prepare(ctx, w, bias, bnp, bnp + cin, cin, cout, ws, s, false);
  if (r) return r;
  r = k_h2_weights(ctx, w, u, cin, cout, 0, s, bnp);
  if (r) return r;
  const float* tab = ws + (size_t)9 * cin * cout;
  r = k_conv3x3_h2_fwd(ctx, x, u, tab, tab, MASK_BIAS_TAB, y, n, h, wd, cin, cout, act, 0.0f, 0, s);
  ctx->k_slices_ok = 0;
  return r;
}
int32_t unet_conv3x3_bnfold_bwd_weights(unet_ctx* ctx, const float* x, const float* bnp, const float* dy, const float* w, float* dw, float* db, double* bn_bwd_sums, void* gws,
                                        size_t gws_bytes, float* ws, int32_t n, int32_t h, int32_t wd, int32_t cin, int32_t cout, int32_t algo, void* stream) {
  if (!ctx || !x || !bnp || !dy || !dw || !db || !ws || n < 1 || h < 1 || wd < 1 || cin < 1) UNET_FAIL(ctx, UNET_E_ARG, "conv3x3_bnfold_bwd_weights: bad args");
  if (!wgrad_bn_fold_supported(cout)) UNET_FAIL(ctx, UNET_E_SHAPE, "conv3x3_bnfold_bwd_weights: cout=%d (needs a divisor of 256)", cout);
  hipStream_t s = as_stream(stream);
  int32_t r = conv3x3_wgrad_dispatch(ctx, x, dy, dw, db, gws, gws_bytes, n, h, wd, cin, cout, algo, s);
  if (r) return r;
  if (bn_bwd_sums && !w) UNET_FAIL(ctx, UNET_E_ARG, "conv3x3_bnfold_bwd_weights: bn_bwd_sums needs the kernel w");
  return k_wgrad_bn_fold_fix(ctx, dy, n, h, wd, cin, cout, bnp, bnp + cin, dw, db, ws + bn_fold_scratch_floats(cin, cout) + unet_conv3x3_w_ws_floats(cin, cout), s,
                             bn_bwd_sums ? w : nullptr, bn_bwd_sums ? bnp + 2 * cin : nullptr, bn_bwd_sums ? bnp + 3 * cin : nullptr, bn_bwd_sums);
}
int32_t unet_conv3x3_bnfold_bwd_data(unet_ctx* ctx, const float* dy, const float* w, const float* bnp, const double* bn_bwd_sums, double count, const float* x, int32_t x_channels,
                                     int32_t mask_mode, float mask_rate, uint64_t mask_seed, float* dx, float* wt_ws, float* coef, int32_t n, int32_t h, int32_t wd, int32_t cin,
                                     int32_t cout, int32_t algo, void* stream) {
  if (!ctx || !dy || !w || !bnp || !bn_bwd_sums || !x || !dx || !wt_ws || !coef || n < 1 || !(count >= 1) || mask_mode < MASK_NONE || mask_mode > MASK_ELU_DROP || !(mask_rate >= 0) ||
      mask_rate >= 1)
    UNET_FAIL(ctx, UNET_E_ARG, "conv3x3_bnfold_bwd_data: bad args");
  if (!unet_conv3x3_bnfold_supported(algo, h, wd, cin, cout))
    UNET_FAIL(ctx, UNET_E_SHAPE, "conv3x3_bnfold_bwd_data: no folded form for h=%d w=%d cin=%d cout=%d (unet_conv3x3_bnfold_supported)", h, wd, cin, cout);
  if (x_channels != cin && (x_channels < 32 || x_channels > cin || (x_channels % 32) || mask_mode != MASK_NONE))
    UNET_FAIL(ctx, UNET_E_ARG, "conv3x3_bnfold_bwd_data: x_channels %d (cin = %d, or a multiple of 32 below it with UNET_MASK_NONE)", x_channels, cin);
  static const int modes[4] = {MASK_BN_BWD, MASK_BN_BWD_RELU, MASK_BN_BWD_ELU, MASK_BN_BWD_ELU_DROP};
  hipStream_t s = as_stream(stream);
  int32_t r = k_bn_bwd_coef(ctx, bnp, bn_bwd_sums, count, coef, cin, s);
  if (!r) r = k_h2_weights(ctx, w, wt_ws, cin, cout, 1, s);
  const bool drop = mask_mode == MASK_ELU_DROP;
  if (!r) r = k_conv3x3_h2_fwd(ctx, dy, wt_ws, coef, x, modes[mask_mode], dx, n, h, wd, cout, cin, ACT_NONE, drop ? mask_rate : 0.0f, drop ? mask_seed : 0, s, x_channels < cin ? x_channels : 1 << 30);
  ctx->k_slices_ok = 0;
  return r;
}
int32_t unet_conv3x3_bnfold_bwd_data_enc_tail(unet_ctx* ctx, const float* dy, const float* w, const float* bnp, const double* bn_bwd_sums, double count, const float* x, int32_t ldx,
                                              const float* enc_bnp, const double* enc_sums, double enc_count, const float* skip_k1, const float* dy_pooled, float rate, uint64_t seed,
                                              float* dx, float* wt_ws, float* coef, int32_t n, int32_t h, int32_t wd, int32_t c, int32_t algo, void* stream) {
  if (!ctx || !dy || !w || !bnp || !bn_bwd_sums || !x || !enc_bnp || !enc_sums || !dy_pooled || !dx || !wt_ws || !coef || n < 1 || !(count >= 1) || !(enc_count >= 1) || !(rate >= 0) || rate >= 1)
    UNET_FAIL(ctx, UNET_E_ARG, "conv3x3_bnfold_bwd_data_enc_tail: bad args");
  if (c < 32 || (c % 32) || (h & 1) || (wd & 1) || !unet_conv3x3_bnfold_supported(algo, h, wd, 2 * c, c) || !h2_enc_tail_dgrad_selected(ctx, algo, n, h, wd, c, true))
    UNET_FAIL(ctx, UNET_E_SHAPE, "conv3x3_bnfold_bwd_data_enc_tail: h=%d w=%d c=%d (even h and w, c a multiple of 32, unet_conv3x3_bnfold_supported(2 c -> c))", h, wd, c);
  hipStream_t s = as_stream(stream);
  int32_t r = k_bn_bwd_coef(ctx, bnp, bn_bwd_sums, count, coef, 2 * c, s);
  if (!r) r = k_h2_weights(ctx, w, wt_ws, 2 * c, c, 1, s);
  if (!r) r = k_conv3x3_h2_dgrad_enc_tail(ctx, dy, wt_ws, coef, x, ldx, enc_bnp, enc_sums, enc_count, skip_k1, dy_pooled, dx, n, h, wd, c, rate, seed, s);
  return r;
}

size_t unet_conv3x3_bwd_weights_ws_bytes(int32_t n, int32_t h, int32_t wd, int32_t cin, int32_t cout) {
  if (cin == 1 && (cout % 4) == 0 && 256 % (cout / 4) == 0 && cout <= 256) return c1_wgrad_ws_bytes(cout);
  return mfma_wgrad_supported(cin, cout) ? mfma_wgrad_ws_bytes(n, h, wd, cin, cout) : 0;
}

// ... 61 lines not shown
  return k_conv3x3_bf16_wgrad(ctx, x, dy, dw, db, ws, ws_bytes, n, h, wd, cin, cout, as_stream(stream));
}
int32_t unet_conv3x3_first_bwd_weights_bf16(unet_ctx* ctx, const float* x, const unet_bf16* dy, float* dw, float* db, void* ws, size_t ws_bytes, int32_t n,
                                            int32_t h, int32_t wd, int32_t cout, void* stream) {
  if (!ctx || !x || !dy || !dw || !db || n < 1 || h < 1 || wd < 1) UNET_FAIL(ctx, UNET_E_ARG, "conv3x3_first_bwd_weights_bf16: bad args");
  return k_conv3x3_c1_wgrad_bf16(ctx, x, dy, dw, db, ws, ws_bytes, n, h, wd, cout, as_stream(stream));
}
int32_t unet_convT2x2_fwd_bf16(unet_ctx* ctx, const unet_bf16* x, const float* w, const float* bias, unet_bf16* y, int32_t ldy, int32_t n, int32_t h,
                               int32_t wd, int32_t cin, int32_t cout, void* w_ws, void* stream) {
  if (!ctx || !x || !w || !y || !w_ws || ldy < cout || (ldy & 7) || n < 1 || h < 1 || wd < 1) UNET_FAIL(ctx, UNET_E_ARG, "convT_fwd_bf16: bad args");
  return k_convT_bf16_fwd(ctx, x, w, bias, y, ldy, n, h, wd, cin, cout, static_cast<unet_bf16*>(w_ws), as_stream(stream));
}
int32_t unet_convT2x2_bwd_data_bf16(unet_ctx* ctx, const unet_bf16* dy, int32_t lddy, const float* w, const unet_bf16* relu_src, unet_bf16* dx, int32_t n,
                                    int32_t h, int32_t wd, int32_t cin, int32_t cout, void* w_ws, void* stream) {
  if (!ctx || !dy || !w || !dx || !w_ws || lddy < cout || (lddy & 7)) UNET_FAIL(ctx, UNET_E_ARG, "convT_bwd_data_bf16: bad args");
  return k_convT_bf16_dgrad(ctx, dy, lddy, w, relu_src, dx, n, h, wd, cin, cout, static_cast<unet_bf16*>(w_ws), as_stream(stream));
}
size_t unet_convT2x2_bwd_weights_ws_bytes_bf16(int32_t n, int32_t h, int32_t wd, int32_t cin, int32_t cout) { return bf16_convT_wgrad_ws_bytes(n, h, wd, cin, cout); }
int32_t unet_convT2x2_bwd_weights_bf16(unet_ctx* ctx, const unet_bf16* x, const unet_bf16* dy, int32_t lddy, float* dw, float* db, void* ws, size_t ws_bytes,
                                       int32_t n, int32_t h, int32_t wd, int32_t cin, int32_t cout, void* stream) {
  if (!ctx || !x || !dy || !dw || !db || lddy < cout || (lddy & 7)) UNET_FAIL(ctx, UNET_E_ARG, "convT_bwd_weights_bf16: bad args");
  return k_convT_bf16_wgrad(ctx, x, dy, lddy, dw, db, ws, ws_bytes, n, h, wd, cin, cout, as_stream(stream));
}

}

namespace {

struct Layer { std::string name; int kind; int cin, cout; };
struct TInfo { int is_state; int64_t off, count; };
struct Buf { size_t off = 0; int ld = 0, n = 0, h = 0, w = 0, c = 0; size_t chan_off = 0; int f32 = 0; };

struct TPtr {
  void* p;
  operator const float*() const { return static_cast<const float*>(p); }
  operator float*() const { return static_cast<float*>(p); }
  operator const unet_bf16*() const { return static_cast<const unet_bf16*>(p); }
  operator unet_bf16*() const { return static_cast<unet_bf16*>(p); }
};

struct Op {
  std::string name;
  std::function<int32_t(hipStream_t)> run;
  double flops = 0, bytes = 0, ms = 0;
  int64_t calls = 0;
};

}

struct unet_model {
  unet_ctx* ctx = nullptr;
  int arch = 0, in_ch = 1, N = 0, H = 0, W = 0, world = 1, algo = 0;
  int dt = UNET_DTYPE_F32;
  std::vector<Layer> layers;
  std::map<std::string, TInfo> tinfo;
  int64_t n_params = 0, n_state = 0;
  float *params = nullptr, *grads = nullptr, *adam_m = nullptr, *adam_v = nullptr, *state = nullptr;
  char* ws = nullptr; size_t ws_bytes = 0;
  const float *x = nullptr, *yt = nullptr; float* pout = nullptr; float* loss_out2 = nullptr;
  float drop_rate = 0.0f; uint64_t drop_seed = 0;
  float cw0 = 1.0f, cw1 = 1.0f;
  unet_loss_sel loss;
  size_t off_wmap = 0;
  bool weighted() const { return loss.kind == UNET_LOSS_WEIGHTED_BCE_DICE; }
  const float* wmap() const { return weighted() ? reinterpret_cast<const float*>(ws) + off_wmap : nullptr; }
  size_t off_dense_ws = 0, dense_ws_bytes = 0;
  std::map<std::string, Buf> act, grad;
  size_t ws_floats_infer = 0, ws_floats_train = 0;
  size_t off_bn_sums = 0, bn_sums_doubles = 0;
  size_t off_bn_bsums = 0;
  std::map<std::string, size_t> bn_sum_off, bn_bsum_off, bnp_off;
  size_t off_loss_sums = 0, off_loss_out = 0, off_wt = 0, off_wgrad_ws = 0; size_t wgrad_ws_bytes = 0;
  size_t off_first_tmp = 0;
  bool skip_raw = false; std::map<std::string, size_t> bn_comp_off; size_t off_tap_tmp = 0;
  std::set<std::string> pool_sums_fused;
  bool c9b_virtual = false;
  bool head_bwd_fused = false;
  size_t off_head_sums = 0; bool head_fused = false;
  std::map<std::string, size_t> sign_off;
  std::map<std::string, size_t> wprep_f, wprep_b;
  std::map<std::string, size_t> fold_off, fold_g_off, fold_c_off;
  std::map<std::string, std::pair<std::string, int>> folded_bn;
  std::map<std::string, size_t> skip_k1_off;
  std::set<std::string> enc_tail_dgrad;
  std::vector<Op> prog[3];
  std::vector<unet_sync_point> sync[3];
  struct SyncRef { int after_op, kind; bool in_ws; size_t off_bytes; int64_t count; int use_op = -1; };
  std::vector<SyncRef> syncref[3];

  float* wsf(size_t off) const { return reinterpret_cast<float*>(ws) + off; }
  double* wsd(size_t off_floats) const { return reinterpret_cast<double*>(reinterpret_cast<float*>(ws) + off_floats); }
  float* P(const std::string& n) const { auto& t = tinfo.at(n); return (t.is_state ? state : params) + t.off; }
  float* G(const std::string& n) const { auto& t = tinfo.at(n); return grads + t.off; }
  const float* A(const std::string& n) const { auto& b = act.at(n); return wsf(b.off + b.chan_off); }
  float* Aw(const std::string& n) const { auto& b = act.at(n); return wsf(b.off + b.chan_off); }
  float* D(const std::string& n) const { auto& b = grad.at(n); return wsf(b.off + b.chan_off); }
  int elem_bytes(const Buf& b) const { return (dt && !b.f32) ? 2 : 4; }
  void* bufptr(const Buf& b) const { return ws + b.off * 4 + b.chan_off * elem_bytes(b); }
  void* Av(const std::string& n) const { return bufptr(act.at(n)); }
  void* Dv(const std::string& n) const { return bufptr(grad.at(n)); }
  TPtr At(const std::string& n) const { return {Av(n)}; }
  TPtr Dt(const std::string& n) const { return {Dv(n)}; }
};

namespace {

const int ENC[4] = {32, 64, 128, 256};

void assign_param_offsets(unet_model* m) {
  int64_t po = 0, so = 0;
  for (auto& l : m->layers) {
    if (l.kind == 2) {
      m->tinfo[l.name + "/gamma"] = {0, po, l.cout}; po += l.cout;
      m->tinfo[l.name + "/beta"] = {0, po, l.cout}; po += l.cout;
      m->tinfo[l.name + "/mean"] = {1, so, l.cout}; so += l.cout;
      m->tinfo[l.name + "/var"] = {1, so, l.cout}; so += l.cout;
    } else {
      int64_t kn = (l.kind == 0 ? 9 : l.kind == 1 ? 4 : 1) * (int64_t)l.cin * l.cout;
      m->tinfo[l.name + "/kernel"] = {0, po, kn}; po += kn;
      m->tinfo[l.name + "/bias"] = {0, po, l.cout}; po += l.cout;
    }
  }
  m->n_params = po; m->n_state = so;
}

void build_layers(unet_model* m) {
  auto& L = m->layers;
  int cprev = m->in_ch;
  for (int k = 1; k <= 4; ++k) {
    int c = ENC[k - 1];
    L.push_back({"c" + std::to_string(k) + "a", 0, cprev, c});
    L.push_back({"c" + std::to_string(k) + "b", 0, c, c});
    L.push_back({"bn" + std::to_string(k), 2, c, c});
    cprev = c;
  }
  L.push_back({"c5a", 0, 256, 512});
  L.push_back({"c5b", 0, 512, 512});
  cprev = 512;
  const int dec[4] = {256, 128, 64, 32};
  for (int k = 6; k <= 9; ++k) {
    int c = dec[k - 6];
    L.push_back({"u" + std::to_string(k), 1, cprev, c});
    L.push_back({"bn" + std::to_string(k), 2, 2 * c, 2 * c});
    L.push_back({"c" + std::to_string(k) + "a", 0, 2 * c, c});
    L.push_back({"c" + std::to_string(k) + "b", 0, c, c});
    cprev = c;
  }
  L.push_back({"out", 3, 32, 1});
  assign_param_offsets(m);
}

struct Carver {
  size_t cur = 0; int dt = 0;
  size_t take(size_t floats) { size_t o = cur; cur += (floats + 63) & ~size_t(63); return o; }
};

Buf mk(Carver& cv, int n, int h, int w, int c) { Buf b; const size_t el = (size_t)n * h * w * c; b.off = cv.take(cv.dt ? (el + 1) / 2 : el); b.ld = c; b.n = n; b.h = h; b.w = w; b.c = c; return b; }
Buf slice(const Buf& b, int c0, int c) { Buf s = b; s.chan_off = c0; s.c = c; return s; }

void plan_scratch(unet_model* m, Carver& cv) {
  size_t nd = 0;
  for (auto& l : m->layers) if (l.kind == 2) { m->bn_sum_off[l.name] = nd; nd += 2 * (size_t)l.cout; }
  m->bn_sums_doubles = nd;
  m->off_bn_sums = cv.take((nd + 5 + UNET_HEAD_SUMS) * 2);
  m->off_loss_sums = m->off_bn_sums + nd * 2;
  m->off_head_sums = m->off_loss_sums + 5 * 2;
// ... 285 lines not shown
}
void emit_bn_apply(unet_model* m, Ops& F, const std::string& name, const std::string& in, const std::string& out, int c) {
  unet_ctx* ctx = m->ctx; const int dt = m->dt; const double eb = dt ? 2.0 : 4.0;
  const Buf ib = m->act.at(in), ob = m->act.at(out);
  const int64_t pixels = (int64_t)ib.n * ib.h * ib.w;
  const size_t bo = m->bnp_off.at(name);
  ADD_OP(F, "bn_apply:" + name, 0, 2 * eb * pixels * c, {
    return TWIN(dt, unet_bn_apply, unet_bn_apply_bf16, ctx, m->At(in), ib.ld, m->wsf(bo), m->At(out), ob.ld, pixels, c, s);
  });
}
void emit_bn_fwd(unet_model* m, Ops& F, Syncs& SY, const std::string& name, const std::string& in, const std::string& out, int c, const std::string& pool, bool training) {
  if (training) { emit_bn_stats(m, F, name, in, c); emit_bn_stats_sync(m, F, SY, name, c); }
  emit_bn_finalize(m, F, name, in, c, training);
  if (pool.empty()) { if (!m->folded_bn.count(name)) emit_bn_apply(m, F, name, in, out, c); return; }
  unet_ctx* ctx = m->ctx; const int dt = m->dt; const double eb = dt ? 2.0 : 4.0;
  const Buf ib = m->act.at(in), ob = m->act.at(out);
  const int64_t pixels = (int64_t)ib.n * ib.h * ib.w;
  const size_t bo = m->bnp_off.at(name);
  ADD_OP(F, "bn_apply_pool:" + pool, 0, eb * 2.25 * pixels * c, {
    return TWIN(dt, unet_bn_apply_maxpool_dropout_fwd, unet_bn_apply_maxpool_dropout_fwd_bf16, ctx, m->At(in), ib.ld, m->wsf(bo), m->At(out), ob.ld, m->At(pool), ib.n, ib.h, ib.w, c, 0.0f, 0, s);
  });
}

void emit_conv_fwd(unet_model* m, Ops& F, const std::string& name, const std::string& in, int cin, int cout, int act, float rate, uint64_t salt, bool training) {
  unet_ctx* ctx = m->ctx; const int dt = m->dt, algo = m->algo; const double eb = dt ? 2.0 : 4.0;
  const Buf ob = m->act.at(name);
  const double px = (double)ob.n * ob.h * ob.w;
  ADD_OP(F, "conv3x3_fwd:" + name, 2.0 * 9 * cin * cout * px, eb * px * (cin + cout) + 4.0 * 9.0 * cin * cout, {
    const float r = (training && m->drop_rate > 0.0f) ? rate : 0.0f;
    if (dt) {
      if (in.empty()) return first_conv_fwd_bf16(ctx, m, name, ob, cout, act, r, m->drop_seed + salt, s);
      return k_conv3x3_bf16_fwd(ctx, m->At(in), m->P(name + "/kernel"), m->P(name + "/bias"), nullptr, MASK_NONE, m->At(name), ob.n, ob.h, ob.w, cin, cout, act, r, m->drop_seed + salt,
                                WBF(static_cast<void*>(m->wsf(m->off_wt))), 0, s);
    }
    return conv3x3_fwd_dispatch(ctx, in.empty() ? m->x : m->A(in), m->P(name + "/kernel"), m->P(name + "/bias"), nullptr, MASK_NONE, m->Aw(name), ob.n, ob.h, ob.w, cin, cout, act, r,
                                m->drop_seed + salt, algo, s, m->wsf(m->off_wt), 0);
  });
}
void emit_conv_fwd_folded(unet_model* m, Ops& F, const std::string& cn, const std::string& xn, const std::string& bnn, int c, int act, float rate, uint64_t salt, bool training) {
  unet_ctx* ctx = m->ctx; const int dt = m->dt; const double eb = dt ? 2.0 : 4.0;
  const Buf ob = m->act.at(cn);
  const double px = (double)ob.n * ob.h * ob.w;
  const size_t fo = m->fold_off.at(cn), bo = m->bnp_off.at(bnn);
  ADD_OP(F, "bn_fold_prepare:" + cn, 2.0 * 9 * c * c * 2, 4.0 * 9 * c * c * 4, {
    return k_bn_fold_prepare(ctx, m->P(cn + "/kernel"), m->P(cn + "/bias"), m->wsf(bo), m->wsf(bo) + c, c, c, m->wsf(fo), s, dt != 0);
  });
  ADD_OP(F, "conv3x3_fwd:" + cn, 2.0 * 9 * c * c * px, eb * px * 2 * c + 4.0 * 9.0 * c * c, {
    const float r = (training && m->drop_rate > 0.0f) ? rate : 0.0f;
    const float* tab = m->wsf(fo) + (size_t)9 * c * c;
    if (dt) return k_conv3x3_bf16_fwd(ctx, m->At(xn), m->wsf(fo), tab, reinterpret_cast<const unet_bf16*>(tab), MASK_BIAS_TAB, m->At(cn), ob.n, ob.h, ob.w, c, c, act, r, m->drop_seed + salt,
                                      WBF(static_cast<void*>(m->wsf(m->off_wt))), 0, s);
    int32_t e = k_h2_weights(ctx, m->P(cn + "/kernel"), m->wsf(m->off_wt), c, c, 0, s, m->wsf(bo));
    if (e) return e;
    return k_conv3x3_h2_fwd(ctx, m->A(xn), m->wsf(m->off_wt), tab, tab, MASK_BIAS_TAB, m->Aw(cn), ob.n, ob.h, ob.w, c, c, act, r, m->drop_seed + salt, s);
  });
}

void emit_bn_bwd(unet_model* m, Ops& BW, Syncs& SY, const std::string& name, const std::string& dyname, const std::string& xname, const std::string& dxname, int c, int mask_mode, float rate,
                 uint64_t salt, bool stats_done) {
  unet_ctx* ctx = m->ctx; const int dt = m->dt; const double eb = dt ? 2.0 : 4.0, gcount = (double)m->world;
  const Buf gb = m->grad.at(dyname), xb = m->act.at(xname), db = m->grad.at(dxname);
  const int64_t pixels = (int64_t)xb.n * xb.h * xb.w;
  const size_t so = m->bn_bsum_off.at(name), bo = m->bnp_off.at(name);
  if (stats_done) ADD_OP(BW, "bn_bwd_param_grads:" + name, 0, 0, {
    return unet_bn_bwd_param_grads(ctx, m->wsd(m->off_bn_bsums) + so, m->G(name + "/gamma"), m->G(name + "/beta"), c, s);
  });
  else ADD_OP(BW, "bn_bwd_stats:" + name, 0, 2 * eb * pixels * c, {
    int32_t r = TWIN(dt, unet_bn_bwd_stats, unet_bn_bwd_stats_bf16, ctx, m->Dt(dyname), gb.ld, m->At(xname), xb.ld, m->wsf(bo), m->wsd(m->off_bn_bsums) + so, pixels, c, s);
    if (r) return r;
    return unet_bn_bwd_param_grads(ctx, m->wsd(m->off_bn_bsums) + so, m->G(name + "/gamma"), m->G(name + "/beta"), c, s);
  });
  SY.push_back({(int)BW.size() - 1, 2, true, m->off_bn_bsums * 4 + so * 8, 2 * (int64_t)c});
  ADD_OP(BW, "bn_bwd_apply:" + name, 0, 3 * eb * pixels * c, {
    const bool drop = m->drop_rate > 0.0f && rate > 0.0f;
    return TWIN(dt, unet_bn_bwd_apply, unet_bn_bwd_apply_bf16, ctx, m->Dt(dyname), gb.ld, m->At(xname), xb.ld, m->wsf(bo), m->wsd(m->off_bn_bsums) + so, (double)pixels * gcount,
                (mask_mode == MASK_ELU_DROP && !drop) ? MASK_ELU : mask_mode, drop ? rate : 0.0f, m->drop_seed + salt, m->Dt(dxname), db.ld, pixels, c, s);
  });
}

void emit_conv_wgrad(unet_model* m, Ops& BW, const std::string& name, const std::string& in, int cin, int cout) {
  unet_ctx* ctx = m->ctx; const int dt = m->dt, algo = m->algo; const double eb = dt ? 2.0 : 4.0;
  const Buf ob = m->act.at(name);
  const double px = (double)ob.n * ob.h * ob.w;
  ADD_OP(BW, "conv3x3_wgrad:" + name, 2.0 * 9 * cin * cout * px, eb * px * (cin + cout) + 4.0 * 9.0 * cin * cout, {
    if (dt) {
      if (in.empty()) return first_conv_wgrad_bf16(ctx, m, name, ob, cout, s);
      return k_conv3x3_bf16_wgrad(ctx, m->At(in), m->Dt(name), m->G(name + "/kernel"), m->G(name + "/bias"), m->wsf(m->off_wgrad_ws), m->wgrad_ws_bytes, ob.n, ob.h, ob.w, cin, cout, s);
    }
    return conv3x3_wgrad_dispatch(ctx, in.empty() ? m->x : m->A(in), m->D(name), m->G(name + "/kernel"), m->G(name + "/bias"), m->wsf(m->off_wgrad_ws), m->wgrad_ws_bytes, ob.n, ob.h, ob.w, cin,
                                  cout, algo, s);
  });
}
void emit_conv_bwd(unet_model* m, Ops& BW, const std::string& name, const std::string& in, int cin, int cout, bool want_dx, int mask_mode, float rate, uint64_t salt) {
  emit_conv_wgrad(m, BW, name, in, cin, cout);
  if (!want_dx) return;
  unet_ctx* ctx = m->ctx; const int dt = m->dt, algo = m->algo; const double eb = dt ? 2.0 : 4.0;
  const Buf ob = m->act.at(name);
  const double px = (double)ob.n * ob.h * ob.w;
  ADD_OP(BW, "conv3x3_dgrad:" + name, 2.0 * 9 * cin * cout * px, eb * px * (cout + cin + (mask_mode ? cin : 0)) + 4.0 * 9.0 * cin * cout, {
    const bool drop = m->drop_rate > 0.0f && rate > 0.0f;
    const int mm = (mask_mode == MASK_ELU_DROP && !drop) ? MASK_ELU : mask_mode;
    if (dt) return k_conv3x3_bf16_fwd(ctx, m->Dt(name), m->P(name + "/kernel"), nullptr, mm ? CBF(m->Av(in)) : nullptr, mm, m->Dt(in), ob.n, ob.h, ob.w, cout, cin, ACT_NONE, drop ? rate : 0.0f,
                                      m->drop_seed + salt, WBF(static_cast<void*>(m->wsf(m->off_wt))), 1, s);
    return unet_conv3x3_bwd_data(ctx, m->D(name), m->P(name + "/kernel"), mm ? m->A(in) : nullptr, mm, drop ? rate : 0.0f, m->drop_seed + salt, m->D(in), m->wsf(m->off_wt), ob.n, ob.h, ob.w, cin, cout,
                                 algo, s);
  });
}
void emit_conv_bwd_folded(unet_model* m, Ops& BW, Syncs& SY, const std::string& cn, const std::string& xn, const std::string& bnn, int c, int mask_mode, float rate, uint64_t salt) {
  unet_ctx* ctx = m->ctx; const int dt = m->dt; const double eb = dt ? 2.0 : 4.0, gcount = (double)m->world;
  const Buf ob = m->act.at(cn);
  const double px = (double)ob.n * ob.h * ob.w;
  const size_t go = m->fold_g_off.at(cn), co = m->fold_c_off.at(cn), bo = m->bnp_off.at(bnn), so = m->bn_bsum_off.at(bnn);
  emit_conv_wgrad(m, BW, cn, xn, c, c);
  ADD_OP(BW, "wgrad_bn_fold_fix:" + cn, 2.0 * 9 * c * c, 8.0 * 9 * c * c, {
    int32_t r = dt ? k_wgrad_bn_fold_fix_bf16(ctx, m->Dt(cn), ob.n, ob.h, ob.w, c, c, m->wsf(bo), m->wsf(bo) + c, m->G(cn + "/kernel"), m->G(cn + "/bias"), m->wsf(go), s, m->P(cn + "/kernel"),
                                              m->wsf(bo) + 2 * c, m->wsf(bo) + 3 * c, m->wsd(m->off_bn_bsums) + so)
                   : k_wgrad_bn_fold_fix(ctx, m->D(cn), ob.n, ob.h, ob.w, c, c, m->wsf(bo), m->wsf(bo) + c, m->G(cn + "/kernel"), m->G(cn + "/bias"), m->wsf(go), s, m->P(cn + "/kernel"),
                                         m->wsf(bo) + 2 * c, m->wsf(bo) + 3 * c, m->wsd(m->off_bn_bsums) + so);
    if (r) return r;
    return unet_bn_bwd_param_grads(ctx, m->wsd(m->off_bn_bsums) + so, m->G(bnn + "/gamma"), m->G(bnn + "/beta"), c, s);
  });
  SY.push_back({(int)BW.size() - 1, 2, true, m->off_bn_bsums * 4 + so * 8, 2 * (int64_t)c});
  ADD_OP(BW, "conv3x3_dgrad_bn_bwd:" + cn, 2.0 * 9 * c * c * px, eb * px * 3 * c + 4.0 * 9.0 * c * c, {
    const bool drop = m->drop_rate > 0.0f && rate > 0.0f;
    const int mm = (mask_mode == MASK_BN_BWD_ELU_DROP && !drop) ? MASK_BN_BWD_ELU : mask_mode;
    int32_t r = k_bn_bwd_coef(ctx, m->wsf(bo), m->wsd(m->off_bn_bsums) + so, px * gcount, m->wsf(co), c, s);
    if (r) return r;
    if (dt) return k_conv3x3_bf16_fwd(ctx, m->Dt(cn), m->P(cn + "/kernel"), m->wsf(co), m->At(xn), mm, m->Dt(xn), ob.n, ob.h, ob.w, c, c, ACT_NONE, drop ? rate : 0.0f, m->drop_seed + salt,
                                      WBF(static_cast<void*>(m->wsf(m->off_wt))), 1, s);
    r = k_h2_weights(ctx, m->P(cn + "/kernel"), m->wsf(m->off_wt), c, c, 1, s);
    if (r) return r;
    return k_conv3x3_h2_fwd(ctx, m->D(cn), m->wsf(m->off_wt), m->wsf(co), m->A(xn), mm, m->D(xn), ob.n, ob.h, ob.w, c, c, ACT_NONE, drop ? rate : 0.0f, m->drop_seed + salt, s);
  });
}

void build_programs(unet_model* m) {
  unet_ctx* ctx = m->ctx;
  const int algo = m->algo;
  const double gcount = (double)m->world;
  const int dt = m->dt;
  const double eb = dt ? 2.0 : 4.0;
  auto& FT = m->prog[UNET_PROG_FWD_TRAIN];
  auto& FI = m->prog[UNET_PROG_FWD_INFER];
  auto& BW = m->prog[UNET_PROG_BWD];
  struct PrepItem { std::string name; int cin, cout, h, w; };
  std::vector<PrepItem> prep_items;
  for (auto& l : m->layers) if (l.kind == 0 && l.cin > 1) { const Buf& ob = m->act.at(l.name); prep_items.push_back({l.name, l.cin, l.cout, ob.h, ob.w}); }
  auto prep_weights_bf16 = [=](int flip, hipStream_t s) -> int32_t {
    unet_wimg_prep_list L; L.n = 0; int ci[UNET_PREP_MAX], co[UNET_PREP_MAX];
    for (auto& it : prep_items) {
      if (!flip && m->fold_off.count(it.name)) continue;
      if (L.n >= UNET_PREP_MAX) UNET_FAIL(ctx, UNET_E_STATE, "weight images (bf16): too many layers for one batch");
      L.item[L.n] = unet_wimg_prep{m->P(it.name + "/kernel"), static_cast<unet_bf16*>(static_cast<void*>(m->wsf((flip ? m->wprep_b : m->wprep_f).at(it.name)))), 0, 0, 0, 0, 0, 0, flip, 0};
      ci[L.n] = flip ? it.cout : it.cin; co[L.n] = flip ? it.cin : it.cout; ++L.n;
    }
    return k_wimg_multi(ctx, &L, ci, co, s);
  };
  std::vector<PrepItem> convt_items;
  for (auto& l : m->layers) if (l.kind == 1 && m->wprep_f.count(l.name)) convt_items.push_back({l.name, l.cin, l.cout, 0, 0});
  auto prep_weights = [=](int flip, hipStream_t s) -> int32_t {
    const float* ws_[UNET_PREP_MAX]; const float* cs_[UNET_PREP_MAX]; void* is_[UNET_PREP_MAX]; int ci_[UNET_PREP_MAX], co_[UNET_PREP_MAX], kd_[UNET_PREP_MAX], nx = 0;
    for (int k = 0; k < UNET_PREP_MAX; ++k) cs_[k] = nullptr;
    for (auto& it : prep_items) {
      const int K = flip ? it.cout : it.cin, M = flip ? it.cin : it.cout;
      if (flip && it.name == "c1a") continue;
      const bool folded = !flip && m->fold_off.count(it.name) != 0;
// ... 161 lines not shown
    const Buf hb = m->act.at("c9b");
    const int64_t hp = (int64_t)hb.n * hb.h * hb.w;
    if (!dt) ADD_OP(BW, "weight_images:bwd", 0, 0, { return prep_weights(1, s); });
    else ADD_OP(BW, "weight_images:bwd", 0, 0, { return prep_weights_bf16(1, s); });
    m->head_bwd_fused = m->head_fused && ctx->opt_head_bwd_fused && m->arch == UNET_ARCH_UNET && m->sign_off.count("c9b") && m->wprep_b.count("c9b") && h2_head_bwd_selected(ctx, algo, hb.w, 32) &&
                        h2_wgrad_selected(algo, 32, 32);
    if (m->head_bwd_fused) ADD_OP(BW, "head_dzm", 8.0 * hp, hp * (8.0 + 4.0 + 8.0), {
      if (!m->yt || !m->pout) UNET_FAIL(ctx, UNET_E_STATE, "head_dzm: io not set");
      return k_head_dzm(ctx, m->pout, m->yt, m->wsd(m->off_loss_sums), (double)hp * gcount, m->wsd(m->off_head_sums), reinterpret_cast<const unsigned long long*>(m->wsf(m->sign_off.at("c9b"))),
                        m->D("c9b"), m->G("out/kernel"), m->G("out/bias"), hb.n, hb.h, hb.w, s, m->loss, m->wmap());
    });
    else
    if (m->head_fused) ADD_OP(BW, "head_dy", 2.0 * 32 * hp, hp * (4.0 * 32 + 8.0 + 4.0), {
      if (!m->yt || !m->pout) UNET_FAIL(ctx, UNET_E_STATE, "head_dy: io not set");
      const auto so = m->sign_off.find("c9b");
      return k_head_dy(ctx, m->pout, m->yt, m->wsd(m->off_loss_sums), (double)hp * gcount, m->wsd(m->off_head_sums), m->P("out/kernel"),
                       so == m->sign_off.end() ? nullptr : reinterpret_cast<const unsigned long long*>(m->wsf(so->second)), m->A("c9b"), m->D("c9b"),
                       m->G("out/kernel"), m->G("out/bias"), hb.n, hb.h, hb.w, s, m->loss, m->wmap());
    });
    else
    emit_head_bwd(m, BW, "c9b", 1);
    std::vector<Op> DEF;
    auto flush_def = [&]() { for (auto& o : DEF) BW.push_back(std::move(o)); DEF.clear(); };
    auto conv_bwd = [&](const std::string& name, const std::string& in, int cin, int cout, bool want_dx, bool mask_in, const std::string& xraw = "", bool defer_wgrad = false) {
      const Buf ob = m->act.at(name);
      const double px = (double)ob.n * ob.h * ob.w;
      const std::string xsrc = xraw.empty() ? in : xraw;
      auto& WV = (defer_wgrad && xraw.empty()) ? DEF : BW;
      const bool hstream = name == "c9b" && m->head_bwd_fused;
      if (hstream) ADD_OP(WV, "conv3x3_wgrad:" + name, 2.0 * 9 * cin * cout * px, eb * px * cin + 8.0 * px + 4.0 * 9.0 * cin * cout, {
        return k_conv3x3_h2_wgrad_dzm(ctx, m->A(xsrc), m->D(name), m->P("out/kernel"), m->G(name + "/kernel"), m->G(name + "/bias"), m->wsf(m->off_wgrad_ws), m->wgrad_ws_bytes, ob.n, ob.h, ob.w, cin, s);
      });
      else emit_conv_wgrad(m, WV, name, xsrc, cin, cout);
      if (!xraw.empty()) {
        const size_t go = m->fold_g_off.at(name), bo = m->bnp_off.at(in);
        const bool pg = !dt && m->fold_c_off.count(name) != 0;
        ADD_OP(BW, "wgrad_bn_fold_fix:" + name, 2.0 * 9 * cin * cout, 8.0 * 9 * cin * cout, {
          if (dt) return k_wgrad_bn_fold_fix_bf16(ctx, CBF(m->Dv(name)), ob.n, ob.h, ob.w, cin, cout, m->wsf(bo), m->wsf(bo) + cin, m->G(name + "/kernel"), m->G(name + "/bias"), m->wsf(go), s,
                                                  m->P(name + "/kernel"), m->wsf(bo) + 2 * cin, m->wsf(bo) + 3 * cin, m->wsd(m->off_bn_bsums) + m->bn_bsum_off.at(in));
          if (m->skip_raw) {
            const float* comp = m->wsf(m->bn_comp_off.at(in));
            return k_wgrad_bn_fold_fix(ctx, m->D(name), ob.n, ob.h, ob.w, cin, cout, comp, comp + cin, m->G(name + "/kernel"), m->G(name + "/bias"), m->wsf(go), s,
                                       m->P(name + "/kernel"), m->wsf(bo) + 2 * cin, m->wsf(bo) + 3 * cin, m->wsd(m->off_bn_bsums) + m->bn_bsum_off.at(in), comp + 2 * cin, comp + 3 * cin,
                                       pg ? m->G(in + "/gamma") : nullptr, pg ? m->G(in + "/beta") : nullptr);
          }
          return k_wgrad_bn_fold_fix(ctx, m->D(name), ob.n, ob.h, ob.w, cin, cout, m->wsf(bo), m->wsf(bo) + cin, m->G(name + "/kernel"), m->G(name + "/bias"), m->wsf(go), s,
                                     m->P(name + "/kernel"), m->wsf(bo) + 2 * cin, m->wsf(bo) + 3 * cin, m->wsd(m->off_bn_bsums) + m->bn_bsum_off.at(in), nullptr, nullptr,
                                     pg ? m->G(in + "/gamma") : nullptr, pg ? m->G(in + "/beta") : nullptr);
        });
      }
      if (!xraw.empty() && m->fold_c_off.count(name)) {
        const std::string bnn = in;
        const size_t so = m->bn_bsum_off.at(bnn), bo = m->bnp_off.at(bnn), co = m->fold_c_off.at(name);
        ADD_OP(BW, "bn_bwd_param_grads:" + bnn, 0, 0, {
          if (!dt) return UNET_OK;
          return unet_bn_bwd_param_grads(ctx, m->wsd(m->off_bn_bsums) + so, m->G(bnn + "/gamma"), m->G(bnn + "/beta"), cin, s);
        });
        SY.push_back({(int)BW.size() - 1, 2, true, m->off_bn_bsums * 4 + so * 8, 2 * (int64_t)cin});
        const size_t syi = SY.size() - 1;
        flush_def();
        SY[syi].use_op = (int)BW.size();
        const bool half = !dt && name.size() == 3 && m->enc_tail_dgrad.count("bn" + std::to_string(10 - (name[1] - '0'))) != 0;
        ADD_OP(BW, "conv3x3_dgrad_bn_bwd:" + name, (half ? 0.5 : 1.0) * 2.0 * 9 * cin * cout * px, half ? eb * px * (cout + cin) + 4.0 * 9.0 * (cin / 2) * cout : eb * px * (cout + 2 * cin) + 4.0 * 9.0 * cin * cout, {
          int32_t r = k_bn_bwd_coef(ctx, m->wsf(bo), m->wsd(m->off_bn_bsums) + so, px * gcount, m->wsf(co), cin, s);
          if (r) return r;
          if (half) return k_conv3x3_h2_dgrad_bn_bwd_up(ctx, m->D(name), m->wsf(m->wprep_b.at(name)), m->wsf(co), m->A(xraw), m->D(xraw), ob.n, ob.h, ob.w, cout, s);
          if (dt) return k_conv3x3_bf16_fwd(ctx, CBF(m->Dv(name)), m->P(name + "/kernel"), m->wsf(co), CBF(m->Av(xraw)), MASK_BN_BWD, WBF(m->Dv(xraw)), ob.n, ob.h, ob.w, cout, cin, ACT_NONE, 0.0f, 0,
                                            WBF(static_cast<void*>(m->wsf(m->off_wt))), 1, s, CBF(static_cast<void*>(m->wsf(m->wprep_b.at(name)))));
          const int climit = m->skip_k1_off.count("bn" + std::to_string(10 - (name[1] - '0'))) ? cin / 2 : (1 << 30);
          return k_conv3x3_h2_fwd(ctx, m->D(name), m->wsf(m->wprep_b.at(name)), m->wsf(co), m->A(xraw), MASK_BN_BWD, m->D(xraw), ob.n, ob.h, ob.w, cout, cin, ACT_NONE, 0.0f, 0, s, climit);
        });
        return;
      }
      if (want_dx && !dt && !mask_in && in.size() == 2 && in[0] == 'p' && ctx->opt_enc_bn_fused && m->wprep_b.count(name) && h2_pool_sums_selected(ctx, algo, ob.w, cout, cin)) {
        const std::string bnn = "bn" + in.substr(1);
        m->pool_sums_fused.insert(in);
        ADD_OP(BW, "conv3x3_dgrad_pool_sums:" + name, 2.0 * 9 * cin * cout * px, eb * px * (cout + 2 * cin) + 4.0 * 9.0 * cin * cout, {
          return k_conv3x3_h2_dgrad_pool_sums(ctx, m->D(name), m->wsf(m->wprep_b.at(name)), m->A(in), m->P(bnn + "/gamma"), m->P(bnn + "/beta"), m->drop_rate, m->D(in),
                                              nullptr, ob.n, ob.h, ob.w, cout, cin, s);
        });
      } else
      if (want_dx) {
        const bool bits = mask_in && m->sign_off.count(in) != 0;
        ADD_OP(BW, "conv3x3_dgrad:" + name, 2.0 * 9 * cin * cout * px, (hstream ? 8.0 * px + eb * px * (cin + (mask_in ? (bits ? cin / 32.0 : cin) : 0)) : eb * px * (cout + cin + (mask_in ? (bits ? cin / 32.0 : cin) : 0))) + 4.0 * 9.0 * cin * cout, {
          if (dt) return k_conv3x3_bf16_fwd(ctx, CBF(m->Dv(name)), m->P(name + "/kernel"), nullptr, mask_in ? CBF(m->Av(in)) : nullptr, mask_in ? MASK_RELU : MASK_NONE, WBF(m->Dv(in)), ob.n, ob.h,
                                            ob.w, cout, cin, ACT_NONE, 0.0f, 0, WBF(static_cast<void*>(m->wsf(m->off_wt))), 1, s, CBF(static_cast<void*>(m->wsf(m->wprep_b.at(name)))));
          const auto pb = m->wprep_b.find(name);
          const auto so = mask_in ? m->sign_off.find(in) : m->sign_off.end();
          if (name == "c9b" && m->head_bwd_fused)
            return k_conv3x3_h2_dgrad_dzm(ctx, m->D(name), m->wsf(pb->second), so != m->sign_off.end() ? m->wsf(so->second) : mask_in ? m->A(in) : nullptr,
                                          so != m->sign_off.end() ? MASK_RELU_BITS : mask_in ? MASK_RELU : MASK_NONE, m->D(in), ob.n, ob.h, ob.w, cin, s);
          if (so != m->sign_off.end())
            return conv3x3_fwd_dispatch(ctx, m->D(name), m->P(name + "/kernel"), nullptr, m->wsf(so->second), MASK_RELU_BITS, m->D(in), ob.n, ob.h,
                                        ob.w, cout, cin, ACT_NONE, 0.0f, 0, algo, s, m->wsf(m->off_wt), 1, pb == m->wprep_b.end() ? nullptr : m->wsf(pb->second));
          return conv3x3_fwd_dispatch(ctx, m->D(name), m->P(name + "/kernel"), nullptr, mask_in ? m->A(in) : nullptr, mask_in ? MASK_RELU : MASK_NONE, m->D(in), ob.n, ob.h,
                                      ob.w, cout, cin, ACT_NONE, 0.0f, 0, algo, s, m->wsf(m->off_wt), 1, pb == m->wprep_b.end() ? nullptr : m->wsf(pb->second));
        });
      }
    };
    auto bucket = [&](const std::string& first, const std::string& last_tensor) { emit_bucket(m, BW, SY, first, last_tensor); };
    if (!dt && m->skip_raw && ctx->opt_enc_bn_fused && ctx->opt_enc_tail_dgrad)
      for (int k = 1; k <= 4; ++k) {
        const std::string bnn = "bn" + std::to_string(k), dca = "c" + std::to_string(10 - k) + "a", cb = "c" + std::to_string(k) + "b";
        const Buf xb = m->act.at(bnn), cg = m->grad.at(cb);
        if (m->fold_c_off.count(dca) && m->skip_k1_off.count(bnn) && m->wprep_b.count(dca) && cg.ld == xb.c && m->act.at(dca).c == xb.c &&
            h2_enc_tail_dgrad_selected(ctx, algo, xb.n, xb.h, xb.w, xb.c, ctx->opt_enc_tail_dgrad == 2))
          m->enc_tail_dgrad.insert(bnn);
      }
    bool enc_split = false;
    const int dec[4] = {256, 128, 64, 32};
    for (int k = 9; k >= 6; --k) {
      int c = dec[k - 6]; std::string ks = std::to_string(k);
      std::string prev = (k == 6) ? "c5b" : "c" + std::to_string(k - 1) + "b";
      int cprev = (k == 6) ? 512 : dec[k - 7];
      conv_bwd("c" + ks + "b", "c" + ks + "a", c, c, true, true, "", m->fold_c_off.count("c" + ks + "a") != 0);
      conv_bwd("c" + ks + "a", "bn" + ks, 2 * c, c, true, false, m->fold_off.count("c" + ks + "a") ? "cat" + ks : "");
      flush_def();
      if (!m->fold_c_off.count("c" + ks + "a")) emit_bn_bwd(m, BW, SY, "bn" + ks, "bn" + ks, "cat" + ks, "cat" + ks, 2 * c, MASK_NONE, 0.0f, 0, m->fold_off.count("c" + ks + "a") != 0);
      const Buf ib = m->act.at(prev), ug = m->grad.at("u" + ks);
      const std::string un = "u" + ks;
      emit_convT_wgrad(m, BW, un, prev, cprev, c);
      ADD_OP(BW, "convT_dgrad:" + un, 2.0 * 4 * cprev * c * nel(ib) / ib.c, eb * (2 * nel(ib) + nel(ug)), {
        if (dt) return k_convT_bf16_dgrad(ctx, CBF(m->Dv(un)), ug.ld, m->P(un + "/kernel"), CBF(m->Av(prev)), WBF(m->Dv(prev)), ib.n, ib.h, ib.w, cprev, c, WBF(static_cast<void*>(m->wsf(m->off_wt))), s);
        const auto so = m->sign_off.find(prev);
        const auto pb = m->wprep_b.find(un);
        const void* img = pb == m->wprep_b.end() ? nullptr : m->wsf(pb->second);
        if (so != m->sign_off.end()) return k_convT_h2_dgrad(ctx, m->D(un), ug.ld, m->P(un + "/kernel"), m->wsf(so->second), m->D(prev), ib.n, ib.h, ib.w, cprev, c, s, 1, img);
        if (img) return k_convT_h2_dgrad(ctx, m->D(un), ug.ld, m->P(un + "/kernel"), m->A(prev), m->D(prev), ib.n, ib.h, ib.w, cprev, c, s, 0, img);
        return unet_convT2x2_bwd_data(ctx, m->D(un), ug.ld, m->P(un + "/kernel"), m->A(prev), m->D(prev), ib.n, ib.h, ib.w, cprev, c, algo, s);
      });
      if (k == 7) bucket("u7/kernel", "out/bias");
      if (k == 6) bucket("u6/kernel", "c6b/bias");
    }
    conv_bwd("c5b", "c5a", 512, 512, true, true);
    conv_bwd("c5a", "p4", 256, 512, true, false, "", ctx->opt_enc_bn_fused != 0);
    if (!ctx->opt_enc_bn_fused) bucket("c5a/kernel", "c5b/bias");
    for (int k = 4; k >= 1; --k) {
      int c = ENC[k - 1]; std::string ks = std::to_string(k);
      const Buf xb = m->act.at("bn" + ks), gb = m->grad.at("bn" + ks);
      const std::string bnn = "bn" + ks, pn = "p" + ks;
      const size_t so = m->bn_bsum_off.at(bnn);
      if (ctx->opt_enc_bn_fused) {
        const std::string dn = "bn" + std::to_string(10 - k), cb = "c" + ks + "b";
        const size_t sod = m->bn_bsum_off.at(dn), bod = m->bnp_off.at(dn), bo = m->bnp_off.at(bnn);
        const Buf cbuf = m->act.at(cb), cg = m->grad.at(cb);
        const int64_t pixels = (int64_t)xb.n * xb.h * xb.w;
        const bool sums_done = m->pool_sums_fused.count(pn) != 0;
        ADD_OP(BW, sums_done ? "pool_bwd_skip_term:" + pn : "pool_bwd_sums:" + pn, 0, sums_done ? 0.0 : eb * 0.5 * nel(xb), {
          int32_t r = sums_done ? UNET_OK : dt ? unet_maxpool2x2_dropout_bwd_sums_bf16(ctx, CBF(m->Av(pn)), CBF(m->Dv(pn)), m->P(bnn + "/gamma"), m->P(bnn + "/beta"), m->wsd(m->off_bn_bsums) + so, xb.n, xb.h,
                                                                 xb.w, xb.c, m->drop_rate, m->drop_seed + (uint64_t)k * 0x9E3779B97F4A7C15ull, s)
                         : unet_maxpool2x2_dropout_bwd_sums(ctx, m->A(pn), m->D(pn), m->P(bnn + "/gamma"), m->P(bnn + "/beta"), m->wsd(m->off_bn_bsums) + so, xb.n, xb.h, xb.w, xb.c,
                                                            m->drop_rate, m->drop_seed + (uint64_t)k * 0x9E3779B97F4A7C15ull, s);
          if (r) return r;
          if (sums_done)
            return k_enc_tail_finish(ctx, m->wsd(m->off_bn_bsums) + so, m->wsd(m->off_bn_bsums) + sod + 3 * (size_t)c, m->wsf(bod) + 7 * (size_t)c, m->P(dn + "/gamma") + c,
                                     m->P(bnn + "/gamma"), m->G(bnn + "/gamma"), m->G(bnn + "/beta"), c, 1.0 / gcount, s);
          r = unet_bn_bwd_skip_term(ctx, m->wsd(m->off_bn_bsums) + so, m->wsd(m->off_bn_bsums) + sod + 3 * (size_t)c, m->wsf(bod) + 7 * (size_t)c, m->P(dn + "/gamma") + c,
                                    m->P(bnn + "/gamma"), c, 1.0 / gcount, s);
          if (r) return r;
          return unet_bn_bwd_param_grads(ctx, m->wsd(m->off_bn_bsums) + so, m->G(bnn + "/gamma"), m->G(bnn + "/beta"), c, s);
        });
        SY.push_back({(int)BW.size() - 1, 2, true, m->off_bn_bsums * 4 + so * 8, 2 * (int64_t)c});
        const size_t syi = SY.size() - 1;
        flush_def();
        if (k == 4) bucket("c5a/kernel", "c5b/bias");
        if (k == 2) { bucket("c3a/kernel", "bn4/beta"); enc_split = true; }
        SY[syi].use_op = (int)BW.size();
        const bool tail = m->enc_tail_dgrad.count(bnn) != 0;
        const std::string dca = "c" + std::to_string(10 - k) + "a";
        ADD_OP(BW, "bn_pool_bwd_apply:" + bnn, tail ? 2.0 * 9 * c * c * (double)pixels * unet_conv3x3_exec_ratio(algo, xb.h, xb.w, c, 2 * c) : 0.0, eb * 3.25 * nel(xb) + (tail ? 4.0 * 9.0 * c * c : 0.0), {
          if (tail)
            return k_conv3x3_h2_dgrad_enc_tail(ctx, m->D(dca), m->wsf(m->wprep_b.at(dca)), m->wsf(m->fold_c_off.at(dca)), m->A(cb), cbuf.ld, m->wsf(bo), m->wsd(m->off_bn_bsums) + so,
                                               (double)pixels * gcount, m->wsf(m->skip_k1_off.at(bnn)), m->D(pn), m->D(cb), xb.n, xb.h, xb.w, xb.c, m->drop_rate,
                                               m->drop_seed + (uint64_t)k * 0x9E3779B97F4A7C15ull, s);
          if (dt) return unet_bn_maxpool_bwd_apply_bf16(ctx, CBF(m->Av(cb)), cbuf.ld, m->wsf(bo), m->wsd(m->off_bn_bsums) + so, (double)pixels * gcount, CBF(m->Dv(bnn)), gb.ld, CBF(m->Dv(pn)),
                                                        WBF(m->Dv(cb)), cg.ld, xb.n, xb.h, xb.w, xb.c, m->drop_rate, m->drop_seed + (uint64_t)k * 0x9E3779B97F4A7C15ull, s);
          const auto k1o = m->skip_k1_off.find(bnn);
          return k_bn_maxpool_bwd_apply_k1(ctx, m->A(cb), cbuf.ld, m->wsf(bo), m->wsd(m->off_bn_bsums) + so, (double)pixels * gcount, m->D(bnn), gb.ld,
                                           k1o == m->skip_k1_off.end() ? nullptr : m->wsf(k1o->second), m->D(pn), m->D(cb), cg.ld,
                                           xb.n, xb.h, xb.w, xb.c, m->drop_rate, m->drop_seed + (uint64_t)k * 0x9E3779B97F4A7C15ull, s);
        });
      } else {
      ADD_OP(BW, "pool_bwd_bnstats:" + pn, 0, eb * 3.25 * nel(xb), {
        if (dt) return unet_maxpool2x2_dropout_bwd_bnstats_bf16(ctx, CBF(m->Av(bnn)), xb.ld, CBF(m->Dv(pn)), WBF(m->Dv(bnn)), gb.ld, m->P(bnn + "/gamma"), m->P(bnn + "/beta"),
                                                                m->wsd(m->off_bn_bsums) + so, xb.n, xb.h, xb.w, xb.c, m->drop_rate,
                                                                m->drop_seed + (uint64_t)k * 0x9E3779B97F4A7C15ull, s);
        return unet_maxpool2x2_dropout_bwd_bnstats(ctx, m->A(bnn), xb.ld, m->D(pn), m->D(bnn), gb.ld, m->P(bnn + "/gamma"), m->P(bnn + "/beta"),
                                                   m->wsd(m->off_bn_bsums) + so, xb.n, xb.h, xb.w, xb.c, m->drop_rate,
                                                   m->drop_seed + (uint64_t)k * 0x9E3779B97F4A7C15ull, s);
      });
      emit_bn_bwd(m, BW, SY, bnn, bnn, "c" + ks + "b", "c" + ks + "b", c, MASK_RELU, 0.0f, 0, true);
// ... 517 lines not shown
    UNET_FAIL(m->ctx, UNET_E_ARG, "model_set_loss: loss %d (alpha %g, beta %g) is not one of this graph's", loss, alpha, beta);
  if (m->arch == UNET_ARCH_CLASSIFIER) return UNET_OK;
  if ((loss == UNET_LOSS_WEIGHTED_BCE_DICE) == m->weighted()) { m->loss = sel; return UNET_OK; }
  unet_model* t = new unet_model();
  t->ctx = m->ctx; t->arch = m->arch; t->in_ch = m->in_ch; t->N = m->N; t->H = m->H; t->W = m->W; t->world = m->world; t->algo = m->algo; t->dt = m->dt; t->loss = sel;
  build_model(t);
  const size_t need = (m->grads ? t->ws_floats_train : t->ws_floats_infer) * sizeof(float);
  delete t;
  if (m->ws && m->ws_bytes < need)
    UNET_FAIL(m->ctx, UNET_E_STATE, "model_set_loss: the bound workspace (%zu bytes) is too small for loss %d (%zu bytes): bind a larger one first", m->ws_bytes, loss, need);
  unet_model keep = std::move(*m);
  *m = unet_model();
  m->ctx = keep.ctx; m->arch = keep.arch; m->in_ch = keep.in_ch; m->N = keep.N; m->H = keep.H; m->W = keep.W; m->world = keep.world; m->algo = keep.algo; m->dt = keep.dt;
  m->loss = sel;
  build_model(m);
  m->params = keep.params; m->grads = keep.grads; m->adam_m = keep.adam_m; m->adam_v = keep.adam_v; m->state = keep.state; m->ws = keep.ws; m->ws_bytes = keep.ws_bytes;
  m->x = keep.x; m->yt = keep.yt; m->pout = keep.pout; m->loss_out2 = keep.loss_out2; m->drop_rate = keep.drop_rate; m->drop_seed = keep.drop_seed;
  m->cw0 = keep.cw0; m->cw1 = keep.cw1;
  if (m->ws) resolve_sync(m);
  return UNET_OK;
}

int32_t unet_model_num_ops(const unet_model* m, int32_t prog) { return (!m || prog < 0 || prog > 2) ? UNET_E_ARG : (int32_t)m->prog[prog].size(); }

int32_t unet_model_sync_points(const unet_model* m, int32_t prog, unet_sync_point* out, int32_t cap) {
  if (!m || prog < 0 || prog > 2) return UNET_E_ARG;
  int n = (int)m->sync[prog].size();
  if (out) for (int i = 0; i < n && i < cap; ++i) out[i] = m->sync[prog][i];
  return n;
}

int32_t unet_model_run(unet_model* m, int32_t prog, int32_t begin, int32_t end, void* stream) {
  if (!m || prog < 0 || prog > 2) return UNET_E_ARG;
  unet_ctx* ctx = m->ctx;
  auto& P = m->prog[prog];
  if (begin < 0 || end > (int)P.size() || begin > end) UNET_FAIL(ctx, UNET_E_ARG, "model_run: bad op range [%d,%d) of %zu", begin, end, P.size());
  if (!m->ws || !m->params) UNET_FAIL(ctx, UNET_E_STATE, "model_run: buffers not bound");
  if (prog == UNET_PROG_BWD && !m->grads) UNET_FAIL(ctx, UNET_E_STATE, "model_run: backward needs a grads buffer");
  if (!m->x) UNET_FAIL(ctx, UNET_E_STATE, "model_run: input not set");
  hipStream_t s = as_stream(stream);
  hipEvent_t e0 = nullptr, e1 = nullptr;
  if (ctx->profiling) { UNET_HIP(ctx, hipEventCreate(&e0)); UNET_HIP(ctx, hipEventCreate(&e1)); }
  if (begin == 0 && prog != UNET_PROG_BWD) { ctx->stats_req_c = 0; ctx->stats_in_slots = nullptr; ctx->stats_in_slots_c = 0; ctx->signs_req = nullptr; ctx->k_slices_ok = 0; }
  for (int i = begin; i < end; ++i) {
    if (ctx->profiling) UNET_HIP(ctx, hipEventRecord(e0, s));
    const int32_t r = P[i].run(s);
    if (r) { ctx->err = P[i].name + ": " + ctx->err; if (ctx->profiling) { (void)hipEventDestroy(e0); (void)hipEventDestroy(e1); } return r; }
    if (ctx->profiling) {
      UNET_HIP(ctx, hipEventRecord(e1, s));
      UNET_HIP(ctx, hipEventSynchronize(e1));
      float ms = 0; UNET_HIP(ctx, hipEventElapsedTime(&ms, e0, e1));
      P[i].ms += ms; P[i].calls += 1;
    }
  }
  if (ctx->profiling) { (void)hipEventDestroy(e0); (void)hipEventDestroy(e1); }
  return UNET_OK;
}

const float* unet_model_loss_ptr(const unet_model* m) { return (m && m->ws) ? m->wsf(m->off_loss_out) : nullptr; }

int32_t unet_model_tap(const unet_model* m, const char* name, int32_t grad, const void** ptr, int32_t* ld, int32_t* n, int32_t* h,
                       int32_t* w, int32_t* c) {
  if (!m || !name || !m->ws) return UNET_E_ARG;
  auto& mp = grad ? m->grad : m->act;
  auto it = mp.find(name);
  if (it == mp.end()) return UNET_E_ARG;
  const Buf& b = it->second;
  const auto fb = m->folded_bn.find(name);
  if (grad && fb != m->folded_bn.end()) {
    const std::string nm = name;
    std::string conv = nm.rfind("bn", 0) == 0 ? "c" + nm.substr(2) + "a" : nm.substr(0, nm.size() - 3) + "b";
    if (m->arch == UNET_ARCH_CLASSIFIER) conv = "c" + nm.substr(2, 1) + "b";
    if (m->fold_c_off.count(conv)) return UNET_E_STATE;
  }
  const std::string nm_ = name;
  if (!grad && m->c9b_virtual && nm_ == "c9b") {
    const Buf& xb = m->act.at("c9a");
    int32_t r = k_conv3x3_h2_fwd(m->ctx, m->A("c9a"), m->wsf(m->wprep_f.at("c9b")), m->P("c9b/bias"), nullptr, MASK_NONE, const_cast<float*>(m->A("c9b")), xb.n, xb.h, xb.w, xb.c, b.c, ACT_RELU,
                                 0.0f, 0, nullptr);
    if (r) return r;
    if (hipStreamSynchronize(nullptr) != hipSuccess) return UNET_E_HIP;
  }
  if (grad && m->enc_tail_dgrad.count(nm_)) return UNET_E_STATE;
  if (grad && m->head_bwd_fused && nm_ == "c9b") return UNET_E_STATE;
  if (!grad && m->skip_raw && nm_.size() == 3 && nm_[0] == 'b' && nm_[2] >= '1' && nm_[2] <= '4') {
    const std::string cb = std::string("c") + nm_[2] + "b";
    const Buf& xb = m->act.at(cb);
    int32_t r = unet_bn_apply(m->ctx, m->A(cb), xb.ld, m->wsf(m->bnp_off.at(name)), const_cast<float*>(m->A(name)), b.ld, (int64_t)b.n * b.h * b.w, b.c, nullptr);
    if (r) return r;
    if (hipStreamSynchronize(nullptr) != hipSuccess) return UNET_E_HIP;
  }
  if (!grad && fb != m->folded_bn.end()) {
    const Buf& xb = m->act.at(fb->second.first);
    const float* bnp_ = m->skip_raw && m->bn_comp_off.count(name) ? m->wsf(m->bn_comp_off.at(name)) : m->wsf(m->bnp_off.at(name));
    int32_t r = m->dt ? unet_bn_apply_bf16(m->ctx, static_cast<const unet_bf16*>(m->Av(fb->second.first)), xb.ld, m->wsf(m->bnp_off.at(name)), static_cast<unet_bf16*>(m->Av(name)), b.ld,
                                           (int64_t)b.n * b.h * b.w, fb->second.second, nullptr)
                      : unet_bn_apply(m->ctx, m->A(fb->second.first), xb.ld, bnp_, const_cast<float*>(m->A(name)), b.ld, (int64_t)b.n * b.h * b.w, fb->second.second, nullptr);
    if (r) return r;
    if (hipStreamSynchronize(nullptr) != hipSuccess) return UNET_E_HIP;
  }
  if (ptr) *ptr = m->bufptr(b);
  if (ld) *ld = b.ld; if (n) *n = b.n; if (h) *h = b.h; if (w) *w = b.w; if (c) *c = b.c;
  return UNET_OK;
}

int32_t unet_model_tap_elem_bytes(const unet_model* m, const char* name, int32_t grad) {
  if (!m || !name) return UNET_E_ARG;
  auto& mp = grad ? m->grad : m->act;
  auto it = mp.find(name);
  return it == mp.end() ? UNET_E_ARG : m->elem_bytes(it->second);
}

int32_t unet_model_op_info(const unet_model* m, int32_t prog, int32_t op, const char** name, double* flops, double* bytes, double* ms,
                           int64_t* calls) {
  if (!m || prog < 0 || prog > 2 || op < 0 || op >= (int)m->prog[prog].size()) return UNET_E_ARG;
  const Op& o = m->prog[prog][op];
  if (name) *name = o.name.c_str();
  if (flops) *flops = o.flops; if (bytes) *bytes = o.bytes; if (ms) *ms = o.ms; if (calls) *calls = o.calls;
  return UNET_OK;
}

int32_t unet_model_reset_timers(unet_model* m) {
  if (!m) return UNET_E_ARG;
  for (auto& P : m->prog) for (auto& o : P) { o.ms = 0; o.calls = 0; }
  return UNET_OK;
}

}
```

Measured before the change: 1080 images/sec.

## Fuse first-layer weight gradient into c1b data-gradient pp kernel

Folds the c1a weight gradient (cin=1, cout=32) into the c1b data-gradient conv_pp kernel. The computed dx tile, still in LDS, is multiplied against a staged input window with fp32 MFMAs, and each block writes per-block partials that a short reduce kernel then sums. This drops the separate c1a wgrad pass, which had to re-read the full-resolution dy gradient for c1a, and stops writing c1a's gradient at all (it is recomputed only on demand for inspection). The cost is extra LDS use, per-tile input loads and MFMA work inside an already tuned pipelined kernel, which may lower occupancy or slow its schedule.

Measured after the change: 1087 images/sec, median of 6. No clear change (+0.7%).

```diff
diff --git a/include/unet_hip.h b/include/unet_hip.h
--- a/include/unet_hip.h
+++ b/include/unet_hip.h
@@ -25,7 +25,7 @@
 int32_t unet_ctx_set_profiling(unet_ctx* ctx, int32_t on);
 enum { UNET_OPT_RELU_BITS = 1, UNET_OPT_BN_FOLD = 2, UNET_OPT_ENC_BN_FUSED = 3, UNET_OPT_BN_CONCAT_ANALYTIC = 4, UNET_OPT_BN_FUSE_STATS = 5, UNET_OPT_DETERMINISTIC = 6,
        UNET_OPT_HEAD_FUSED = 7, UNET_OPT_SKIP_RAW = 8, UNET_OPT_POOL_SUMS_FUSED = 9, UNET_OPT_HEAD_BWD_FUSED = 10, UNET_OPT_CONV_PP = 13, UNET_OPT_ENC_TAIL_DGRAD = 14,
-       UNET_OPT_WGRAD_EARLY_SPLIT = 15 };
+       UNET_OPT_WGRAD_EARLY_SPLIT = 15, UNET_OPT_C1A_WGRAD_FUSED = 16 };
 int32_t unet_ctx_set_option(unet_ctx* ctx, int32_t option, int32_t value);
 int32_t unet_ctx_get_option(unet_ctx* ctx, int32_t option);
 
@@ -64,6 +64,9 @@
 int32_t unet_conv3x3_bnfold_bwd_data_enc_tail(unet_ctx*, const float* dy, const float* w, const float* bnp, const double* bn_bwd_sums, double count, const float* x, int32_t ldx,
                                               const float* enc_bnp, const double* enc_sums, double enc_count, const float* skip_k1, const float* dy_pooled, float rate,
                                               uint64_t seed, float* dx, float* wt_ws, float* coef, int32_t n, int32_t h, int32_t wd, int32_t c, int32_t algo, void* stream);
+int32_t unet_conv3x3_bwd_data_c1_wgrad_supported(unet_ctx*, int32_t n, int32_t h, int32_t wd);
+int32_t unet_conv3x3_bwd_data_c1_wgrad(unet_ctx*, const float* dy, const float* w, const void* bits, const float* x, float* dw, float* db, float* wt_ws, void* ws, size_t ws_bytes,
+                                       int32_t n, int32_t h, int32_t wd, void* stream);
 size_t unet_conv3x3_bwd_weights_ws_bytes(int32_t n, int32_t h, int32_t wd, int32_t cin, int32_t cout);
 int32_t unet_conv3x3_bwd_weights(unet_ctx*, const float* x, const float* dy, float* dw, float* db,
                                  void* ws, size_t ws_bytes, int32_t n, int32_t h, int32_t wd,
diff --git a/one-stop-for-covid-19-infection-and-lung-segmentation-plus-classification_amd/_lib.py b/one-stop-for-covid-19-infection-and-lung-segmentation-plus-classification_amd/_lib.py
--- a/one-stop-for-covid-19-infection-and-lung-segmentation-plus-classification_amd/_lib.py
+++ b/one-stop-for-covid-19-infection-and-lung-segmentation-plus-classification_amd/_lib.py
@@ -9,7 +9,7 @@
 COMM_HANDLE_BYTES, COMM_MAX_WORLD, COMM_MAX_DOUBLES = 64, 8, 2048
 
 ALGO_AUTO, ALGO_NAIVE, ALGO_MFMA = 0, 1, 2
-OPTIONS = {"relu_bits": 1, "bn_fold": 2, "enc_bn_fused": 3, "bn_concat_analytic": 4, "bn_fuse_stats": 5, "deterministic": 6, "head_fused": 7, "skip_raw": 8, "pool_sums_fused": 9, "head_bwd_fused": 10, "conv_pp": 13, "enc_tail_dgrad": 14, "wgrad_early_split": 15}
+OPTIONS = {"relu_bits": 1, "bn_fold": 2, "enc_bn_fused": 3, "bn_concat_analytic": 4, "bn_fuse_stats": 5, "deterministic": 6, "head_fused": 7, "skip_raw": 8, "pool_sums_fused": 9, "head_bwd_fused": 10, "conv_pp": 13, "enc_tail_dgrad": 14, "wgrad_early_split": 15, "c1a_wgrad_fused": 16}
 ARCH_UNET, ARCH_UNETPP, ARCH_CLASSIFIER = 0, 1, 2
 LOSSES = {"bce_dice_loss": 0, "binary_crossentropy": 1, "dice_loss": 2, "tversky_loss": 3, "weighted_bce_dice_loss": 4}
 DTYPE_F32, DTYPE_BF16 = 0, 1
@@ -154,6 +154,8 @@
     "unet_cluster_route": (i32, [vp, vp, i32, i64, i32, i32, i32, i64, vp, vp, i32, vp, i32, vp, vp, vp, vp, sz, vp]),
     "unet_conv3x3_head_supported": (i32, [vp, i32, i32, i32, i32]),
     "unet_conv3x3_head_fwd": (i32, [vp, vp, vp, vp, vp, vp, vp, vp, vp, vp, vp, i32, i32, i32, i32, vp, vp]),
+    "unet_conv3x3_bwd_data_c1_wgrad_supported": (i32, [vp, i32, i32, i32]),
+    "unet_conv3x3_bwd_data_c1_wgrad": (i32, [vp, vp, vp, vp, vp, vp, vp, vp, vp, sz, i32, i32, i32, vp]),
     "unet_conv3x3_bwd_data_pool_sums_supported": (i32, [vp, i32, i32, i32, i32]),
     "unet_conv3x3_bwd_data_pool_sums": (i32, [vp, vp, vp, vp, vp, vp, f32, vp, vp, vp, i32, i32, i32, i32, i32, vp]),
     "unet_head_dy": (i32, [vp, vp, vp, vp, f64, vp, vp, vp, vp, vp, vp, vp, i32, i32, i32, vp]),
diff --git a/one-stop-for-covid-19-infection-and-lung-segmentation-plus-classification_amd/csrc/common.h b/one-stop-for-covid-19-infection-and-lung-segmentation-plus-classification_amd/csrc/common.h
--- a/one-stop-for-covid-19-infection-and-lung-segmentation-plus-classification_amd/csrc/common.h
+++ b/one-stop-for-covid-19-infection-and-lung-segmentation-plus-classification_amd/csrc/common.h
@@ -29,6 +29,7 @@
   int opt_head_fused = 1;
   int opt_head_bwd_fused = 1;
   int opt_enc_tail_dgrad = 1;
+  int opt_c1a_wgrad_fused = 1;
   int opt_wgrad_early_split = 0;
   int opt_conv_pp = 1;
   int opt_deterministic = 0;
@@ -263,7 +264,11 @@
 bool h2_conv3x3_selected(int algo, int K, int M);
 bool pp_conv3x3_selected(const unet_ctx* ctx, int K, int M, int n, int h, int wd, const float* mask, int mask_mode, int act, float rate, int ldy);
 int32_t k_conv3x3_pp_fwd(unet_ctx*, const float* x, const void* wimg, const float* bias, const float* mask, int mask_mode, float* y, int ldy, int n, int h, int wd, int K, int M,
-                         int act, hipStream_t s, bool vdy = false);
+                         int act, hipStream_t s, bool vdy = false, const float* c1x = nullptr, float* c1part = nullptr);
+bool pp_c1a_wgrad_fused_selected(const unet_ctx* ctx, int algo, int n, int h, int wd, int cin, int cout, bool sign_bits, size_t ws_bytes);
+int pp_c1w_partials(const unet_ctx* ctx);
+int32_t k_conv3x3_pp_dgrad_c1w(unet_ctx*, const float* dy, const void* wimg, const float* signs, const float* x1, void* ws, size_t ws_bytes, int n, int h, int wd, hipStream_t s);
+int32_t k_c1_wgrad_reduce(unet_ctx*, void* ws, size_t ws_bytes, int nparts, float* dw, float* db, int cout, hipStream_t s);
 size_t h2_wimg_bytes(int K, int M);
 int32_t k_h2_weights(unet_ctx*, const float* w, void* img, int cin, int cout, int flip, hipStream_t s, const float* cs = nullptr);
 int32_t k_h2_weights_multi(unet_ctx*, const float* const* w, void* const* img, const int* cin, const int* cout, const int* flip, int count, hipStream_t s);
diff --git a/one-stop-for-covid-19-infection-and-lung-segmentation-plus-classification_amd/csrc/kernels_conv_naive.hip b/one-stop-for-covid-19-infection-and-lung-segmentation-plus-classification_amd/csrc/kernels_conv_naive.hip
--- a/one-stop-for-covid-19-infection-and-lung-segmentation-plus-classification_amd/csrc/kernels_conv_naive.hip
+++ b/one-stop-for-covid-19-infection-and-lung-segmentation-plus-classification_amd/csrc/kernels_conv_naive.hip
@@ -450,6 +450,14 @@
   hipLaunchKernelGGL(reduce_c1_kernel, dim3((10 * cout + 127) / 128, 1), dim3(128), 0, s, part2, dw, db, ngroups, ngroups, cout, 1);
   UNET_CHECK_LAUNCH(ctx, "conv3x3_c1_wgrad"); return UNET_OK;
 }
+int32_t k_c1_wgrad_reduce(unet_ctx* ctx, void* ws, size_t ws_bytes, int nparts, float* dw, float* db, int cout, hipStream_t s) {
+  if (!ws || ws_bytes < c1_wgrad_ws_bytes(cout) || nparts < 1 || nparts > C1_BLOCKS) UNET_FAIL(ctx, UNET_E_ARG, "c1_wgrad_reduce: workspace too small or %d partials", nparts);
+  float* part = static_cast<float*>(ws); float* part2 = part + (size_t)C1_BLOCKS * 10 * cout;
+  const int ngroups = (nparts + 31) / 32;
+  hipLaunchKernelGGL(reduce_c1_kernel, dim3((10 * cout + 127) / 128, ngroups), dim3(128), 0, s, part, part2, nullptr, nparts, 32, cout, 0);
+  hipLaunchKernelGGL(reduce_c1_kernel, dim3((10 * cout + 127) / 128, 1), dim3(128), 0, s, part2, dw, db, ngroups, ngroups, cout, 1);
+  UNET_CHECK_LAUNCH(ctx, "c1_wgrad_reduce"); return UNET_OK;
+}
 int32_t k_conv3x3_c1_wgrad(unet_ctx* ctx, const float* x, const float* dy, float* dw, float* db, void* ws, size_t ws_bytes, int n, int h, int wd, int cout,
                            hipStream_t s) { return c1_wgrad_impl(ctx, x, dy, dw, db, ws, ws_bytes, n, h, wd, cout, s); }
 int32_t k_conv3x3_c1_wgrad_bf16(unet_ctx* ctx, const float* x, const unet_bf16* dy, float* dw, float* db, void* ws, size_t ws_bytes, int n, int h, int wd,
diff --git a/one-stop-for-covid-19-infection-and-lung-segmentation-plus-classification_amd/csrc/kernels_conv_pp.hip b/one-stop-for-covid-19-infection-and-lung-segmentation-plus-classification_amd/csrc/kernels_conv_pp.hip
--- a/one-stop-for-covid-19-infection-and-lung-segmentation-plus-classification_amd/csrc/kernels_conv_pp.hip
+++ b/one-stop-for-covid-19-infection-and-lung-segmentation-plus-classification_amd/csrc/kernels_conv_pp.hip
@@ -32,11 +32,12 @@
 __device__ __forceinline__ f16x8 pp_frag(const char* p) { return *reinterpret_cast<const f16x8*>(p); }
 __device__ __forceinline__ int pp_cell(int p, int c) { return p * 128 + ((c ^ (p & 7)) << 4); }
 
-template <int KC, bool BITS, bool VDY>
+template <int KC, bool BITS, bool VDY, bool C1W = false>
 __global__ __launch_bounds__(512, 2) void conv_pp_kernel(const float* __restrict__ x, const unet_bf16* __restrict__ wimg_hdr, const float* __restrict__ bias,
                                                          const float* __restrict__ mask, float* __restrict__ y, int ldy, int N, int H, int W, int act, int mask_mode,
                                                          int tiles_x, int tiles_y, int total_tiles, double* __restrict__ stats, int stats_c,
-                                                         unsigned long long* __restrict__ signs, int xs) {
+                                                         unsigned long long* __restrict__ signs, int xs, const float* __restrict__ c1x, float* __restrict__ c1part) {
+  static_assert(!C1W || (BITS && !VDY && KC == 2), "the fused first-layer weight gradient rides in the one-bit-mask data gradient of 32 -> 32 channels");
   constexpr int RW = 2, TH = 8, PWD = 34, NPIX = (TH + 2) * PWD, K = 16 * KC, M = 32;
   constexpr int HS = NPIX * 16;
   constexpr int PLANE = 2 * HS, CHUNK = 2 * PLANE + 32;
@@ -55,6 +56,8 @@
   float* const s_bias = reinterpret_cast<float*>(smem + W_ALL + 2 * IN_HALF + 4 * 4096) + 8;
   float* const s_stat = s_bias + 32;
   float* const s_tab = s_stat + 8 * 2 * 32;
+  constexpr int XWIN = (TH + 2) * PWD, XWIN_LD = 352;
+  float* const s_x1 = s_tab + 16 * 32 + half * XWIN_LD;
 
   const int per = gridDim.x >> 3, xcd = blockIdx.x & 7, j = blockIdx.x >> 3;
   const int tpx = (total_tiles + 7) >> 3;
@@ -76,6 +79,21 @@
   const __amdgpu_buffer_rsrc_t rs_y = make_rsrc(y, (((long long)N * H * W - 1) * ldy + M) * 4);
   const int st_lane = ((lane >> 3) * ldy + (lane & 7) * 4) * 4;
 
+  const __amdgpu_buffer_rsrc_t rs_x1 = make_rsrc(C1W ? c1x - (W + 1) : nullptr, C1W ? ((long long)N * H * W + W + 1) * 4 : 0);
+  int xrel[2];
+  float xreg[2] = {0.f, 0.f};
+#pragma unroll
+  for (int k = 0; k < 2; ++k) {
+    const int idx = tid + k * 256, r = idx / PWD, col = idx - r * PWD;
+    xrel[k] = idx < XWIN ? (r * W + col) * 4 : UNET_OOB;
+  }
+  const int c1m = lane & 15, c1k = lane >> 4;
+  const bool c1_tap = c1m < 9;
+  const float c1_fill = c1m == 9 ? 1.f : 0.f;
+  const int c1_aoff = c1_tap ? ((wave * RW + c1m / 3) * PWD + c1m % 3 + c1k) * 4 : 0;
+  const int c1_boff = c1k * 128 + ((((c1m >> 2) ^ c1k)) << 4) + (c1m & 3) * 4;
+  unet_f32x4 c1d[2] = {{0.f, 0.f, 0.f, 0.f}, {0.f, 0.f, 0.f, 0.f}};
+  float c1a = 0.f, c1b[2] = {0.f, 0.f};
   unet_u32x4 pregA[PL];
   struct pos { int n, y0, x0; };
   auto tile_pos = [&](int t) __attribute__((always_inline)) {
@@ -150,6 +168,25 @@
     const int r = sl < 9 ? 0 : 1, q = sl - r * 9;
     const int py = py0 + wave * RW + r;
     if (py >= H) return;
+    if (C1W) {
+      if (q == 0) {
+#pragma unroll
+        for (int qq = 0; qq < 4; ++qq)
+          *reinterpret_cast<float4*>(s_out + pp_cell(l31, hi * 4 + qq)) = make_float4(vprev[r][qq * 4], vprev[r][qq * 4 + 1], vprev[r][qq * 4 + 2], vprev[r][qq * 4 + 3]);
+      }
+      const float a = c1_tap ? c1a : c1_fill;
+      const float b0 = c1b[0], b1 = c1b[1];
+      if (q < 8) {
+        c1a = *reinterpret_cast<const float*>(reinterpret_cast<const char*>(s_x1) + c1_aoff + r * PWD * 4 + q * 16);
+#pragma unroll
+        for (int nt = 0; nt < 2; ++nt) c1b[nt] = *reinterpret_cast<const float*>(s_out + c1_boff + q * 512 + ((nt ^ (q & 1)) << 6));
+      }
+      if (q >= 1) {
+        c1d[0] = __builtin_amdgcn_mfma_f32_16x16x4f32(a, b0, c1d[0], 0, 0, 0);
+        c1d[1] = __builtin_amdgcn_mfma_f32_16x16x4f32(a, b1, c1d[1], 0, 0, 0);
+      }
+      return;
+    }
     if (q == 0) {
 #pragma unroll
       for (int qq = 0; qq < 4; ++qq)
@@ -296,6 +333,10 @@
     __builtin_amdgcn_s_barrier();
     PP_STAMP(2);
     if (BITS && have_prev) output_values();
+    if (C1W && have_prev) {
+      s_x1[tid] = xreg[0];
+      if (tid + 256 < XWIN) s_x1[tid + 256] = xreg[1];
+    }
     if (have_cur) {
       const float4 m4 = *reinterpret_cast<const float4*>(s_amax);
       const float mx = fmaxf(fmaxf(m4.x, m4.y), fmaxf(m4.z, m4.w));
@@ -334,6 +375,15 @@
     }
     __builtin_amdgcn_sched_barrier(0);
     if (have_next && (PP_EXP & 2) == 0) issue_loads(p_next, preg);
+    if (C1W && have_cur) {
+      const int soff = ((p_cur.n * H + p_cur.y0) * W + p_cur.x0) * 4;
+#pragma unroll
+      for (int k = 0; k < 2; ++k) {
+        const int idx = tid + k * 256, r = idx / PWD, col = idx - r * PWD;
+        const bool ok = (unsigned)(p_cur.y0 - 1 + r) < (unsigned)H && (unsigned)(p_cur.x0 - 1 + col) < (unsigned)W;
+        xreg[k] = buf_ld1(rs_x1, ok ? xrel[k] : UNET_OOB, soff);
+      }
+    }
     __builtin_amdgcn_sched_barrier(0);
     PP_STAMP(4);
     if (!BITS && have_prev) output_values();
@@ -356,6 +406,23 @@
   for (int it = 0; it <= iters; ++it) body(it, pregA);
   if (!half) { __builtin_amdgcn_s_barrier(); __builtin_amdgcn_s_barrier(); }
 
+  if (C1W) {
+    float* const red = reinterpret_cast<float*>(smem + W_ALL);
+    __syncthreads();
+#pragma unroll
+    for (int nt = 0; nt < 2; ++nt)
+#pragma unroll
+      for (int v = 0; v < 4; ++v)
+        if (c1k * 4 + v < 10) red[(wave8 * 10 + c1k * 4 + v) * 32 + nt * 16 + c1m] = c1d[nt][v];
+    __syncthreads();
+    if (threadIdx.x < 320) {
+      float t = 0.f;
+#pragma unroll
+      for (int wv = 0; wv < 8; ++wv) t += red[wv * 320 + threadIdx.x];
+      c1part[(size_t)blockIdx.x * 320 + threadIdx.x] = t;
+    }
+  }
+
   if (stats) {
     float sv[8] = {st1.x, st1.y, st1.z, st1.w, st2.x, st2.y, st2.z, st2.w};
 #pragma unroll
@@ -391,8 +458,10 @@
   return true;
 }
 
+int pp_c1w_partials(const unet_ctx* ctx) { return ctx->num_cu & ~7; }
+
 int32_t k_conv3x3_pp_fwd(unet_ctx* ctx, const float* x, const void* wimg, const float* bias, const float* mask, int mask_mode, float* y, int ldy, int n, int h, int wd, int K, int M,
-                         int act, hipStream_t s, bool vdy) {
+                         int act, hipStream_t s, bool vdy, const float* c1x, float* c1part) {
   if (K != 32 || M != 32) UNET_FAIL(ctx, UNET_E_SHAPE, "conv pp: K=%d M=%d", K, M);
   constexpr int KC = 2;
   ctx->k_slices_ok = 0;
@@ -413,15 +482,29 @@
     if (act == ACT_RELU && (mask_mode == MASK_NONE || mask_mode == MASK_BIAS_TAB) && !(wd & 7)) { signs = q; ctx->signs_done = q; }
   }
   constexpr int NPIX = 340, CHUNK = 4 * NPIX * 16 + 32;
-  constexpr size_t smem = (size_t)KC * 9 * 2048 + 2 * (size_t)KC * CHUNK + 4 * 4096 + 32 + 128 + 8 * 2 * 32 * 4 + 16 * 32 * 4;
+  const size_t smem = (size_t)KC * 9 * 2048 + 2 * (size_t)KC * CHUNK + 4 * 4096 + 32 + 128 + 8 * 2 * 32 * 4 + 16 * 32 * 4 + (c1x ? 2 * 352 * 4 : 0);
+  if (c1x && (!c1part || vdy || mask_mode != MASK_RELU_BITS || bias || act != ACT_NONE || stats || signs)) UNET_FAIL(ctx, UNET_E_ARG, "conv pp with the first layer's weight gradient: a plain one-bit-mask data-gradient launch only");
   if (vdy && (stats || signs || bias || act != ACT_NONE || mask_mode == MASK_BIAS_TAB)) UNET_FAIL(ctx, UNET_E_ARG, "conv pp behind the head's {dz, mask} stream: a plain data-gradient launch only");
-  auto kern = vdy ? (mask_mode == MASK_RELU_BITS ? conv_pp_kernel<KC, true, true> : conv_pp_kernel<KC, false, true>)
+  auto kern = c1x ? conv_pp_kernel<KC, true, false, true> : vdy ? (mask_mode == MASK_RELU_BITS ? conv_pp_kernel<KC, true, true> : conv_pp_kernel<KC, false, true>)
                   : (mask_mode == MASK_RELU_BITS ? conv_pp_kernel<KC, true, false> : conv_pp_kernel<KC, false, false>);
   UNET_BIG_LDS(ctx, kern, smem, "conv_pp");
   unet_note_kernel(ctx, reinterpret_cast<const void*>(kern));
   const unsigned grid = (unsigned)(ctx->num_cu & ~7);
   hipLaunchKernelGGL(kern, dim3(grid), dim3(512), smem, s, x, static_cast<const unet_bf16*>(wimg), bias, mask, y, ldy, n, h, wd, act, mask_mode, tiles_x, tiles_y, (int)total, stats,
-                     stats_c, signs, ctx->opt_deterministic ? 1 : 0);
+                     stats_c, signs, ctx->opt_deterministic ? 1 : 0, c1x, c1part);
   UNET_CHECK_LAUNCH(ctx, "conv_pp");
   return UNET_OK;
 }
+
+bool pp_c1a_wgrad_fused_selected(const unet_ctx* ctx, int algo, int n, int h, int wd, int cin, int cout, bool sign_bits, size_t ws_bytes) {
+  if (!ctx || !ctx->opt_c1a_wgrad_fused || cin != 1 || cout != 32 || !sign_bits || !h2_conv3x3_selected(algo, 32, 32)) return false;
+  if ((long long)h * wd * 32 * 4 >= (1LL << 30)) return false;
+  if (ws_bytes < c1_wgrad_ws_bytes(32) || (size_t)pp_c1w_partials(ctx) + 32 > c1_wgrad_ws_bytes(32) / (10 * 32 * sizeof(float))) return false;
+  return pp_conv3x3_selected(ctx, 32, 32, n, h, wd, reinterpret_cast<const float*>(ctx), MASK_RELU_BITS, ACT_NONE, 0.0f, 32);
+}
+
+int32_t k_conv3x3_pp_dgrad_c1w(unet_ctx* ctx, const float* dy, const void* wimg, const float* signs, const float* x1, void* ws, size_t ws_bytes, int n, int h, int wd, hipStream_t s) {
+  if (!dy || !wimg || !signs || !x1 || !ws) UNET_FAIL(ctx, UNET_E_ARG, "conv pp with the first layer's weight gradient: null argument");
+  if (!pp_c1a_wgrad_fused_selected(ctx, UNET_ALGO_AUTO, n, h, wd, 1, 32, true, ws_bytes)) UNET_FAIL(ctx, UNET_E_SHAPE, "conv pp with the first layer's weight gradient: n=%d h=%d wd=%d not taken", n, h, wd);
+  return k_conv3x3_pp_fwd(ctx, dy, wimg, nullptr, signs, MASK_RELU_BITS, nullptr, 32, n, h, wd, 32, 32, ACT_NONE, s, false, x1, static_cast<float*>(ws));
+}
diff --git a/one-stop-for-covid-19-infection-and-lung-segmentation-plus-classification_amd/csrc/model.hip b/one-stop-for-covid-19-infection-and-lung-segmentation-plus-classification_amd/csrc/model.hip
--- a/one-stop-for-covid-19-infection-and-lung-segmentation-plus-classification_amd/csrc/model.hip
+++ b/one-stop-for-covid-19-infection-and-lung-segmentation-plus-classification_amd/csrc/model.hip
@@ -60,6 +60,7 @@
     case UNET_OPT_CONV_PP: return &ctx->opt_conv_pp;
     case UNET_OPT_ENC_TAIL_DGRAD: return &ctx->opt_enc_tail_dgrad;
     case UNET_OPT_WGRAD_EARLY_SPLIT: return &ctx->opt_wgrad_early_split;
+    case UNET_OPT_C1A_WGRAD_FUSED: return &ctx->opt_c1a_wgrad_fused;
     default: return nullptr;
   }
 }
@@ -276,6 +277,21 @@
                                          as_stream(stream), wt_ws, 1);
   ctx->k_slices_ok = 0;
   return r;
+}
+
+int32_t unet_conv3x3_bwd_data_c1_wgrad_supported(unet_ctx* ctx, int32_t n, int32_t h, int32_t wd) {
+  return ctx && n >= 1 && h >= 1 && wd >= 1 && pp_c1a_wgrad_fused_selected(ctx, UNET_ALGO_AUTO, n, h, wd, 1, 32, true, c1_wgrad_ws_bytes(32)) ? 1 : 0;
+}
+int32_t unet_conv3x3_bwd_data_c1_wgrad(unet_ctx* ctx, const float* dy, const float* w, const void* bits, const float* x, float* dw, float* db, float* wt_ws, void* ws, size_t ws_bytes,
+                                       int32_t n, int32_t h, int32_t wd, void* stream) {
+  if (!ctx || !dy || !w || !bits || !x || !dw || !db || !wt_ws || !ws || n < 1 || h < 1 || wd < 1) UNET_FAIL(ctx, UNET_E_ARG, "conv3x3_bwd_data_c1_wgrad: bad args");
+  if (!pp_c1a_wgrad_fused_selected(ctx, UNET_ALGO_AUTO, n, h, wd, 1, 32, true, ws_bytes))
+    UNET_FAIL(ctx, UNET_E_SHAPE, "conv3x3_bwd_data_c1_wgrad: not taken for n=%d h=%d w=%d (unet_conv3x3_bwd_data_c1_wgrad_supported)", n, h, wd);
+  int32_t r = k_h2_weights(ctx, w, wt_ws, 32, 32, 1, as_stream(stream));
+  if (r) return r;
+  r = k_conv3x3_pp_dgrad_c1w(ctx, dy, wt_ws, static_cast<const float*>(bits), x, ws, ws_bytes, n, h, wd, as_stream(stream));
+  if (r) return r;
+  return k_c1_wgrad_reduce(ctx, ws, ws_bytes, pp_c1w_partials(ctx), dw, db, 32, as_stream(stream));
 }
 
 int32_t unet_conv3x3_bwd_data_pool_sums_supported(unet_ctx* ctx, int32_t algo, int32_t wd, int32_t cin, int32_t cout) { return ctx && h2_pool_sums_selected(ctx, algo, wd, cout, cin) ? 1 : 0; }
@@ -503,6 +519,7 @@
   std::map<std::string, size_t> fold_off, fold_g_off, fold_c_off;
   std::map<std::string, std::pair<std::string, int>> folded_bn;
   std::map<std::string, size_t> skip_k1_off;
+  bool c1a_wgrad_fused = false;
   std::set<std::string> enc_tail_dgrad;
   std::vector<Op> prog[3];
   std::vector<unet_sync_point> sync[3];
@@ -954,6 +971,13 @@
   unet_ctx* ctx = m->ctx; const int dt = m->dt, algo = m->algo; const double eb = dt ? 2.0 : 4.0;
   const Buf ob = m->act.at(name);
   const double px = (double)ob.n * ob.h * ob.w;
+  if (in.empty() && m->c1a_wgrad_fused) {
+    const double parts = (double)pp_c1w_partials(ctx);
+    ADD_OP(BW, "conv3x3_wgrad:" + name, 0, 4.0 * 10 * cout * (parts + 2.0 * ((parts + 31) / 32) + 1), {
+      return k_c1_wgrad_reduce(ctx, m->wsf(m->off_wgrad_ws), m->wgrad_ws_bytes, pp_c1w_partials(ctx), m->G(name + "/kernel"), m->G(name + "/bias"), cout, s);
+    });
+    return;
+  }
   ADD_OP(BW, "conv3x3_wgrad:" + name, 2.0 * 9 * cin * cout * px, eb * px * (cin + cout) + 4.0 * 9.0 * cin * cout, {
     if (dt) {
       if (in.empty()) return first_conv_wgrad_bf16(ctx, m, name, ob, cout, s);
@@ -1281,6 +1305,12 @@
       } else
       if (want_dx) {
         const bool bits = mask_in && m->sign_off.count(in) != 0;
+        if (name == "c1b" && m->c1a_wgrad_fused) {
+          ADD_OP(BW, "conv3x3_dgrad:" + name, 2.0 * 9 * cin * cout * px + 2.0 * 16 * cin * px / unet_conv3x3_exec_ratio(algo, ob.h, ob.w, cout, cin),
+                 eb * px * (cout + cin / 32.0 + 340.0 / 256.0) + 4.0 * 10 * cin * pp_c1w_partials(ctx) + 4.0 * 9.0 * cin * cout, {
+            return k_conv3x3_pp_dgrad_c1w(ctx, m->D(name), m->wsf(m->wprep_b.at(name)), m->wsf(m->sign_off.at(in)), m->x, m->wsf(m->off_wgrad_ws), m->wgrad_ws_bytes, ob.n, ob.h, ob.w, s);
+          });
+        } else
         ADD_OP(BW, "conv3x3_dgrad:" + name, 2.0 * 9 * cin * cout * px, (hstream ? 8.0 * px + eb * px * (cin + (mask_in ? (bits ? cin / 32.0 : cin) : 0)) : eb * px * (cout + cin + (mask_in ? (bits ? cin / 32.0 : cin) : 0))) + 4.0 * 9.0 * cin * cout, {
           if (dt) return k_conv3x3_bf16_fwd(ctx, CBF(m->Dv(name)), m->P(name + "/kernel"), nullptr, mask_in ? CBF(m->Av(in)) : nullptr, mask_in ? MASK_RELU : MASK_NONE, WBF(m->Dv(in)), ob.n, ob.h,
                                             ob.w, cout, cin, ACT_NONE, 0.0f, 0, WBF(static_cast<void*>(m->wsf(m->off_wt))), 1, s, CBF(static_cast<void*>(m->wsf(m->wprep_b.at(name)))));
@@ -1306,6 +1336,11 @@
             h2_enc_tail_dgrad_selected(ctx, algo, xb.n, xb.h, xb.w, xb.c, ctx->opt_enc_tail_dgrad == 2))
           m->enc_tail_dgrad.insert(bnn);
       }
+    {
+      const Buf b1 = m->act.at("c1a");
+      m->c1a_wgrad_fused = !dt && m->in_ch == 1 && b1.c == 32 && m->sign_off.count("c1a") && m->wprep_b.count("c1b") &&
+                           pp_c1a_wgrad_fused_selected(ctx, algo, b1.n, b1.h, b1.w, m->in_ch, b1.c, true, m->wgrad_ws_bytes);
+    }
     bool enc_split = false;
     const int dec[4] = {256, 128, 64, 32};
     for (int k = 9; k >= 6; --k) {
@@ -1989,6 +2024,13 @@
     if (hipStreamSynchronize(nullptr) != hipSuccess) return UNET_E_HIP;
   }
   if (grad && m->enc_tail_dgrad.count(nm_)) return UNET_E_STATE;
+  if (grad && m->c1a_wgrad_fused && nm_ == "c1a") {
+    const Buf& gb = m->act.at("c1b");
+    int32_t r = k_conv3x3_h2_fwd(m->ctx, m->D("c1b"), m->wsf(m->wprep_b.at("c1b")), nullptr, m->wsf(m->sign_off.at("c1a")), MASK_RELU_BITS, m->D("c1a"), gb.n, gb.h, gb.w, gb.c, b.c, ACT_NONE,
+                                 0.0f, 0, nullptr);
+    if (r) return r;
+    if (hipStreamSynchronize(nullptr) != hipSuccess) return UNET_E_HIP;
+  }
   if (grad && m->head_bwd_fused && nm_ == "c9b") return UNET_E_STATE;
   if (!grad && m->skip_raw && nm_.size() == 3 && nm_[0] == 'b' && nm_[2] >= '1' && nm_[2] <= '4') {
     const std::string cb = std::string("c") + nm_[2] + "b";
```
